# choderalab/pymbar

Measured on AMD Instinct MI355X. Metric: mbar_adaptive_iterations_per_sec, higher is better.
Workload: dtype f64

## Files before the change

### include/mbar_hip.h

```cpp
#ifndef MBAR_HIP_H
#define MBAR_HIP_H

#include <stdint.h>

#ifdef __cplusplus
extern "C" {
#endif

typedef struct mbar_ctx mbar_ctx;

#define MBAR_OK 0
#define MBAR_ERR_ARG (-1)
#define MBAR_ERR_HIP (-2)
#define MBAR_ERR_NODEVICE (-3)
#define MBAR_ERR_STATE (-4)
#define MBAR_ERR_COMM (-5)
#define MBAR_ERR_NUMERIC (-6)

#define MBAR_EVAL_GRAM 1u
#define MBAR_EVAL_USE_OFFSET 2u

#define MBAR_TIMER_LSE 0
#define MBAR_TIMER_GRAM 1
#define MBAR_TIMER_REDUCE 2
#define MBAR_TIMER_OTHER 3
#define MBAR_TIMER_FUSED 4
#define MBAR_TIMER_NEWTON 5
#define MBAR_TIMER_COMM 6
#define MBAR_TIMER_COUNT 7

int mbar_version(void);
const char* mbar_last_error(const mbar_ctx* ctx);
int mbar_device_count(int* count);
int mbar_device_info(int device, char* name, int name_len, int* compute_units, int64_t* total_mem_bytes);

int mbar_ctx_create(mbar_ctx** out, int device, int64_t K, int64_t N_local);
void mbar_ctx_destroy(mbar_ctx* ctx);
int mbar_ctx_synchronize(mbar_ctx* ctx);
int mbar_cache_trim(void);
int mbar_host_digest(const void* data, int64_t nbytes, int threads, uint64_t* out2);
int mbar_host_newton_direction(const double* H, const double* g, int m, int threads, double* x);
int mbar_device_synchronize(int device);
int mbar_ctx_set_option(mbar_ctx* ctx, const char* key, int64_t value);

int mbar_ctx_upload_u(mbar_ctx* ctx, const double* u_host, int64_t ld_host, int64_t col0_host,
                      int64_t ncols, int64_t col0_dev);
int mbar_ctx_download_u(mbar_ctx* ctx, double* out, int64_t ld_out);
int mbar_ctx_upload_rows(mbar_ctx* ctx, int64_t row0, int64_t nrows, const double* rows_host, int64_t ld_host);
int mbar_ctx_copy_rows(mbar_ctx* dst, int64_t dst_row0, mbar_ctx* src, int64_t src_row0, int64_t nrows);
int mbar_ctx_row_sub(mbar_ctx* ctx, int64_t row, const double* v_host);
int mbar_ctx_rows_sub(mbar_ctx* ctx, int64_t dst_row0, int64_t src_row0, int64_t nrows, const double* v_host);
int mbar_ctx_rows_rsub(mbar_ctx* ctx, int64_t dst_row0, int64_t src_row0, int64_t nrows);
int mbar_ctx_rows_logshift(mbar_ctx* ctx, int64_t row0, int64_t nrows, double* shift_out);
int mbar_ctx_vec_logshift(mbar_ctx* ctx, const double* A, double* shift_out);
int mbar_ctx_fill_masked_rows(mbar_ctx* ctx, int64_t row0, int64_t nrows, const double* v_host, const int32_t* label_host);
int mbar_ctx_generate_harmonic(mbar_ctx* ctx, uint64_t seed, const double* O_k, const double* K_k,
                               const int64_t* N_k_global, int64_t n_global0);
int mbar_ctx_set_Nk(mbar_ctx* ctx, const double* N_k);

int mbar_ctx_set_sample_weights(mbar_ctx* ctx, const double* c_n);

int mbar_ctx_draw_bootstrap_weights(mbar_ctx* ctx, uint64_t seed, int64_t replicate, const int64_t* cumN, int64_t K_states,
                                    const int64_t* order, int64_t n_global0);
int mbar_ctx_set_bootstrap_layout(mbar_ctx* ctx, const int64_t* cumN, int64_t K_states, const int64_t* order);
int mbar_bootstrap_draws(uint64_t seed, int64_t replicate, const int64_t* cumN, int64_t K_states, const int64_t* order,
                         int64_t* rints_out);

int mbar_ctx_weights_from_vec(mbar_ctx* ctx, double power);

int mbar_comm_unique_id(void* id128);
int mbar_ctx_comm_init(mbar_ctx* ctx, const void* id128, int rank, int nranks);
typedef int (*mbar_allreduce_fn)(double* buf, int64_t count, int op, void* user);
int mbar_ctx_set_host_allreduce(mbar_ctx* ctx, mbar_allreduce_fn fn, void* user, int rank, int nranks);
int mbar_ctx_comm_destroy(mbar_ctx* ctx);

typedef struct mbar_loopback mbar_loopback;
int mbar_loopback_create(mbar_loopback** out, int nranks);
void mbar_loopback_destroy(mbar_loopback* group);
int mbar_ctx_set_loopback(mbar_ctx* ctx, mbar_loopback* group, int rank);

int mbar_eval(mbar_ctx* ctx, const double* f, int nf, unsigned flags, double* psum,
              double* sumlogden, double* gram);
int mbar_ctx_set_objective_offset(mbar_ctx* ctx, const double* f0);
int mbar_lognum(mbar_ctx* ctx, const double* f, double* lognum);
int mbar_logden(mbar_ctx* ctx, const double* f, double* out_n);
int mbar_logw(mbar_ctx* ctx, const double* f, double* out_kn, int64_t ld_out);
int mbar_w(mbar_ctx* ctx, const double* f, double* out_kn, int64_t ld_out);
int mbar_gram_w(mbar_ctx* ctx, const double* f, double* gramW, double* wsum);

int mbar_ctx_create_ext(mbar_ctx** out, mbar_ctx* base, int64_t K_rows);
int mbar_ctx_rows_sub_from(mbar_ctx* dst, int64_t dst_row0, mbar_ctx* src, int64_t src_row0, int64_t nrows, const double* v_host);
int mbar_ctx_rows_rsub_from(mbar_ctx* dst, int64_t dst_row0, mbar_ctx* src, int64_t src_row0, int64_t nrows);
int mbar_ctx_rows_obs_from(mbar_ctx* dst, int64_t dst_row0, mbar_ctx* base, int64_t state_row0, int64_t obs_row0, int64_t nrows,
                           double* shift_out, const double* min_in, double* min_out);
int mbar_lognum_ext(mbar_ctx* ext, mbar_ctx* base, const double* f_base, double* lognum_ext);
int mbar_gram_w_ext(mbar_ctx* ext, mbar_ctx* base, const double* f_base, const double* f_ext, const double* gram_base, double* gramW,
                    double* wsum);

typedef struct mbar_solve_result {
    int64_t iterations;
    int64_t nr_iter;
    int64_t sci_iter;
    int32_t success;
    int32_t gram_sweeps;
    double max_delta;
    double gnorm;
    double wall_ms;
    int32_t warm_starts;
    int32_t builds;
    int32_t light_sweeps;
    int32_t fused_unit;
} mbar_solve_result;

int mbar_solve_adaptive(mbar_ctx* ctx, double* f_inout, double tol, int64_t maxiter,
                        int64_t min_sc_iter, double gamma, int check_convergence,
                        double* history, int64_t history_rows, mbar_solve_result* result);
int mbar_ctx_last_solve_psum(mbar_ctx* ctx, double* psum);
int mbar_solve_sci(mbar_ctx* ctx, double* f_inout, double tol, int64_t maxiter, int check_convergence,
                   mbar_solve_result* result);

int mbar_ctx_timing(mbar_ctx* ctx, int which, double* total_ms, int64_t* launches);
int mbar_ctx_timing_reset(mbar_ctx* ctx);
int mbar_mfma_f64_peak(mbar_ctx* ctx, double* tflops);

typedef struct mbar_kde mbar_kde;
#define MBAR_KDE_GAUSSIAN 0
#define MBAR_KDE_TOPHAT 1
#define MBAR_KDE_EPANECHNIKOV 2
#define MBAR_KDE_EXPONENTIAL 3
#define MBAR_KDE_LINEAR 4
#define MBAR_KDE_COSINE 5
int mbar_kde_create(mbar_kde** out, int device, int kernel, int d, int64_t N, const double* x, double bandwidth);
void mbar_kde_destroy(mbar_kde* kde);
int mbar_kde_set_weights(mbar_kde* kde, int64_t C, const double* v);
int mbar_kde_eval(mbar_kde* kde, int64_t M, const double* q, double* out);
int mbar_kde_log_norm(int kernel, int d, double bandwidth, double* out);

typedef struct mbar_acf mbar_acf;
int mbar_acf_create(mbar_acf** out, int device, int64_t T, const double* a, const double* b, int64_t K, const int64_t* seg,
                    double shift_a, double shift_b);
void mbar_acf_destroy(mbar_acf* acf);
int mbar_acf_suffix_g(mbar_acf* acf, int64_t nskip, int fast, int64_t mintime, int fft, double* g, int64_t* stop, int32_t* status);
int mbar_acf_multiple_g(mbar_acf* acf, int fast, int64_t mintime, double* g, int64_t* stop, int32_t* status, int64_t ct_cap,
                        double* ct);
int mbar_acf_schedule_length(int fast, int64_t tmax, int64_t* out);
int mbar_acf_lag_sums(mbar_acf* acf, int64_t nlags, const int64_t* lags, int64_t norig, const int64_t* origins, int segments,
                      double* xab, double* xba);

#define MBAR_BAR_CHUNK 4096
typedef struct mbar_bar_state {
    double DeltaF, DeltaF_old, DeltaF_initial, UpperB, LowerB, FUpperB, FLowerB, FNew, relative_change, relative_tolerance;
    double req[2];
    double moments[4];
    int64_t method, iterated, maximum_iterations, iteration, phase, status, nreq, nzero, want_moments, moments_pending;
} mbar_bar_state;
typedef struct mbar_bar mbar_bar;
int mbar_bar_create(mbar_bar** out, int device, int64_t P, const int64_t* n_f, const double* w_f, const int64_t* n_r,
                    const double* w_r);
void mbar_bar_destroy(mbar_bar* bar);
int mbar_bar_zero(mbar_bar* bar, const double* deltaf, double* out);
int mbar_bar_solve(mbar_bar* bar, mbar_bar_state* states, int64_t* passes);
int mbar_bar_moments(mbar_bar* bar, double* out);
int mbar_bar_step_host(mbar_bar_state* state, const double* F);

typedef struct mbar_bspline mbar_bspline;
int mbar_bspline_create(mbar_bspline** out, int device, int64_t N, const double* x);
void mbar_bspline_destroy(mbar_bspline* bs);
int mbar_bspline_set_groups(mbar_bspline* bs, int G, const int* g);
int mbar_bspline_set_weights(mbar_bspline* bs, int64_t C, const double* v);
int mbar_bspline_moments(mbar_bspline* bs, int k, int nbasis, const double* t, double* out);
int mbar_bspline_kernel_ms(mbar_bspline* bs, double* ms);

#define MBAR_BATCH_MAX_K 64
#define MBAR_BATCH_CHUNK 256
typedef struct mbar_batch_state {
    double f[MBAR_BATCH_MAX_K];
    double req[2][MBAR_BATCH_MAX_K];
    double lognum[MBAR_BATCH_MAX_K];
    double psum[MBAR_BATCH_MAX_K];
    double Nk[MBAR_BATCH_MAX_K];
    double x[MBAR_BATCH_MAX_K];
    double tol, gamma, max_delta, max_diff, gnorm_sci, gnorm_nr;
    int64_t K, maxiter, min_sc_iter, iterations, nr_iter, sci_iter, choices;
    int64_t phase, status, success, nreq, gram_req, gram_w, newton_bad;
} mbar_batch_state;
typedef struct mbar_batch mbar_batch;
int mbar_batch_create(mbar_batch** out, int device, int64_t P, const int64_t* K, const int64_t* N, const double* const* u);
void mbar_batch_destroy(mbar_batch* b);
int mbar_batch_solve(mbar_batch* b, mbar_batch_state* states, int64_t* passes);
int mbar_batch_gram_w(mbar_batch* b, const double* f, const int32_t* mask, double* gram, double* wsum);
int mbar_batch_step_host(mbar_batch_state* state, const double* lognum, const double* gram);

int mbar_batch_set_replicas(mbar_batch* b, int64_t R, const int64_t* base, const int64_t* Nk);
int mbar_batch_replica_set_weights(mbar_batch* b, int64_t slot, const double* c_n);
int mbar_batch_replicas_draw(mbar_batch* b, int64_t first, int64_t count, const uint64_t* seed, const int64_t* replicate);
int mbar_batch_replicas_solve(mbar_batch* b, mbar_batch_state* states, int64_t* passes);
int mbar_batch_replicas_gram_w(mbar_batch* b, const double* f, const int32_t* mask, double* gram, double* wsum);

#ifdef __cplusplus
}
#endif
#endif
```

### pymbar_amd/_lib.py

```python
import ctypes as C
import os

HERE = os.path.dirname(os.path.abspath(__file__))
LIB_PATH = os.environ.get("MBAR_HIP_LIBRARY") or os.path.join(HERE, "csrc", "libmbar_hip.so")

MBAR_OK = 0
EVAL_GRAM = 1
EVAL_USE_OFFSET = 2
TIMER_LSE, TIMER_GRAM, TIMER_REDUCE, TIMER_OTHER, TIMER_FUSED, TIMER_NEWTON, TIMER_COMM = 0, 1, 2, 3, 4, 5, 6


class BackendUnavailable(RuntimeError):
    """libmbar_hip.so is missing / not loadable, or there is no gfx950 device."""


class MbarHipError(RuntimeError):

    def __init__(self, code, message):
        super().__init__(f"libmbar_hip error {code}: {message}")
        self.code = code


class BarState(C.Structure):
    _fields_ = [(n, C.c_double) for n in ("DeltaF", "DeltaF_old", "DeltaF_initial", "UpperB", "LowerB", "FUpperB", "FLowerB", "FNew",
                                          "relative_change", "relative_tolerance")] + [
        ("req", C.c_double * 2), ("moments", C.c_double * 4)] + [
        (n, C.c_int64) for n in ("method", "iterated", "maximum_iterations", "iteration", "phase", "status", "nreq", "nzero",
                                 "want_moments", "moments_pending")]


MBAR_BATCH_MAX_K = 64
MBAR_BATCH_CHUNK = 256


class BatchState(C.Structure):
    _fields_ = [(n, C.c_double * MBAR_BATCH_MAX_K) for n in ("f",)] + [("req", (C.c_double * MBAR_BATCH_MAX_K) * 2)] + [
        (n, C.c_double * MBAR_BATCH_MAX_K) for n in ("lognum", "psum", "Nk", "x")] + [
        (n, C.c_double) for n in ("tol", "gamma", "max_delta", "max_diff", "gnorm_sci", "gnorm_nr")] + [
        (n, C.c_int64) for n in ("K", "maxiter", "min_sc_iter", "iterations", "nr_iter", "sci_iter", "choices", "phase", "status",
                                 "success", "nreq", "gram_req", "gram_w", "newton_bad")]


class SolveResult(C.Structure):
    _fields_ = [
        ("iterations", C.c_int64),
        ("nr_iter", C.c_int64),
        ("sci_iter", C.c_int64),
        ("success", C.c_int32),
        ("gram_sweeps", C.c_int32),
        ("max_delta", C.c_double),
        ("gnorm", C.c_double),
        ("wall_ms", C.c_double),
        ("warm_starts", C.c_int32),
        ("builds", C.c_int32),
        ("light_sweeps", C.c_int32),
        ("fused_unit", C.c_int32),
    ]


ALLREDUCE_FN = C.CFUNCTYPE(C.c_int, C.POINTER(C.c_double), C.c_int64, C.c_int, C.c_void_p)

_dp = C.POINTER(C.c_double)
_ip = C.POINTER(C.c_int64)
_ctx = C.c_void_p

SIGNATURES = {
    "mbar_version": (C.c_int, []),
    "mbar_last_error": (C.c_char_p, [_ctx]),
    "mbar_device_count": (C.c_int, [C.POINTER(C.c_int)]),
    "mbar_device_info": (C.c_int, [C.c_int, C.c_char_p, C.c_int, C.POINTER(C.c_int), _ip]),
    "mbar_ctx_create": (C.c_int, [C.POINTER(_ctx), C.c_int, C.c_int64, C.c_int64]),
    "mbar_ctx_destroy": (None, [_ctx]),
    "mbar_ctx_synchronize": (C.c_int, [_ctx]),
    "mbar_device_synchronize": (C.c_int, [C.c_int]),
    "mbar_cache_trim": (C.c_int, []),
    "mbar_host_digest": (C.c_int, [C.c_void_p, C.c_int64, C.c_int, C.POINTER(C.c_uint64)]),
    "mbar_host_newton_direction": (C.c_int, [_dp, _dp, C.c_int, C.c_int, _dp]),
    "mbar_ctx_set_option": (C.c_int, [_ctx, C.c_char_p, C.c_int64]),
    "mbar_ctx_upload_u": (C.c_int, [_ctx, _dp, C.c_int64, C.c_int64, C.c_int64, C.c_int64]),
    "mbar_ctx_download_u": (C.c_int, [_ctx, _dp, C.c_int64]),
    "mbar_ctx_upload_rows": (C.c_int, [_ctx, C.c_int64, C.c_int64, _dp, C.c_int64]),
    "mbar_ctx_copy_rows": (C.c_int, [_ctx, C.c_int64, _ctx, C.c_int64, C.c_int64]),
    "mbar_ctx_row_sub": (C.c_int, [_ctx, C.c_int64, _dp]),
    "mbar_ctx_rows_sub": (C.c_int, [_ctx, C.c_int64, C.c_int64, C.c_int64, _dp]),
    "mbar_ctx_rows_rsub": (C.c_int, [_ctx, C.c_int64, C.c_int64, C.c_int64]),
    "mbar_ctx_rows_logshift": (C.c_int, [_ctx, C.c_int64, C.c_int64, _dp]),
    "mbar_ctx_vec_logshift": (C.c_int, [_ctx, _dp, _dp]),
    "mbar_ctx_fill_masked_rows": (C.c_int, [_ctx, C.c_int64, C.c_int64, _dp, C.POINTER(C.c_int32)]),
    "mbar_ctx_generate_harmonic": (C.c_int, [_ctx, C.c_uint64, _dp, _dp, _ip, C.c_int64]),
    "mbar_ctx_set_Nk": (C.c_int, [_ctx, _dp]),
    "mbar_ctx_set_sample_weights": (C.c_int, [_ctx, _dp]),
    "mbar_ctx_weights_from_vec": (C.c_int, [_ctx, C.c_double]),
    "mbar_ctx_draw_bootstrap_weights": (C.c_int, [_ctx, C.c_uint64, C.c_int64, _ip, C.c_int64, _ip, C.c_int64]),
    "mbar_ctx_set_bootstrap_layout": (C.c_int, [_ctx, _ip, C.c_int64, _ip]),
    "mbar_bootstrap_draws": (C.c_int, [C.c_uint64, C.c_int64, _ip, C.c_int64, _ip, _ip]),
    "mbar_comm_unique_id": (C.c_int, [C.c_void_p]),
    "mbar_ctx_comm_init": (C.c_int, [_ctx, C.c_void_p, C.c_int, C.c_int]),
    "mbar_ctx_set_host_allreduce": (C.c_int, [_ctx, ALLREDUCE_FN, C.c_void_p, C.c_int, C.c_int]),
    "mbar_ctx_comm_destroy": (C.c_int, [_ctx]),
    "mbar_loopback_create": (C.c_int, [C.POINTER(C.c_void_p), C.c_int]),
    "mbar_loopback_destroy": (None, [C.c_void_p]),
    "mbar_ctx_set_loopback": (C.c_int, [_ctx, C.c_void_p, C.c_int]),
    "mbar_eval": (C.c_int, [_ctx, _dp, C.c_int, C.c_uint, _dp, _dp, _dp]),
    "mbar_ctx_set_objective_offset": (C.c_int, [_ctx, _dp]),
    "mbar_lognum": (C.c_int, [_ctx, _dp, _dp]),
    "mbar_logden": (C.c_int, [_ctx, _dp, _dp]),
    "mbar_logw": (C.c_int, [_ctx, _dp, _dp, C.c_int64]),
    "mbar_w": (C.c_int, [_ctx, _dp, _dp, C.c_int64]),
    "mbar_gram_w": (C.c_int, [_ctx, _dp, _dp, _dp]),
    "mbar_ctx_create_ext": (C.c_int, [C.POINTER(_ctx), _ctx, C.c_int64]),
    "mbar_ctx_rows_sub_from": (C.c_int, [_ctx, C.c_int64, _ctx, C.c_int64, C.c_int64, _dp]),
    "mbar_ctx_rows_rsub_from": (C.c_int, [_ctx, C.c_int64, _ctx, C.c_int64, C.c_int64]),
    "mbar_ctx_rows_obs_from": (C.c_int, [_ctx, C.c_int64, _ctx, C.c_int64, C.c_int64, C.c_int64, _dp, _dp, _dp]),
    "mbar_lognum_ext": (C.c_int, [_ctx, _ctx, _dp, _dp]),
    "mbar_gram_w_ext": (C.c_int, [_ctx, _ctx, _dp, _dp, _dp, _dp, _dp]),
    "mbar_solve_adaptive": (C.c_int, [_ctx, _dp, C.c_double, C.c_int64, C.c_int64, C.c_double, C.c_int,
                                      _dp, C.c_int64, C.POINTER(SolveResult)]),
    "mbar_ctx_last_solve_psum": (C.c_int, [_ctx, _dp]),
    "mbar_solve_sci": (C.c_int, [_ctx, _dp, C.c_double, C.c_int64, C.c_int, C.POINTER(SolveResult)]),
    "mbar_ctx_timing": (C.c_int, [_ctx, C.c_int, _dp, _ip]),
    "mbar_ctx_timing_reset": (C.c_int, [_ctx]),
    "mbar_mfma_f64_peak": (C.c_int, [_ctx, _dp]),
    "mbar_kde_create": (C.c_int, [C.POINTER(C.c_void_p), C.c_int, C.c_int, C.c_int, C.c_int64, _dp, C.c_double]),
    "mbar_kde_destroy": (None, [C.c_void_p]),
    "mbar_kde_set_weights": (C.c_int, [C.c_void_p, C.c_int64, _dp]),
    "mbar_kde_eval": (C.c_int, [C.c_void_p, C.c_int64, _dp, _dp]),
    "mbar_kde_log_norm": (C.c_int, [C.c_int, C.c_int, C.c_double, _dp]),
    "mbar_acf_create": (C.c_int, [C.POINTER(C.c_void_p), C.c_int, C.c_int64, _dp, _dp, C.c_int64, _ip, C.c_double, C.c_double]),
    "mbar_acf_destroy": (None, [C.c_void_p]),
    "mbar_acf_suffix_g": (C.c_int, [C.c_void_p, C.c_int64, C.c_int, C.c_int64, C.c_int, _dp, _ip, C.POINTER(C.c_int32)]),
    "mbar_acf_multiple_g": (C.c_int, [C.c_void_p, C.c_int, C.c_int64, _dp, _ip, C.POINTER(C.c_int32), C.c_int64, _dp]),
    "mbar_acf_schedule_length": (C.c_int, [C.c_int, C.c_int64, _ip]),
    "mbar_acf_lag_sums": (C.c_int, [C.c_void_p, C.c_int64, _ip, C.c_int64, _ip, C.c_int, _dp, _dp]),
    "mbar_bar_create": (C.c_int, [C.POINTER(C.c_void_p), C.c_int, C.c_int64, _ip, _dp, _ip, _dp]),
    "mbar_bar_destroy": (None, [C.c_void_p]),
    "mbar_bar_zero": (C.c_int, [C.c_void_p, _dp, _dp]),
    "mbar_bar_solve": (C.c_int, [C.c_void_p, C.POINTER(BarState), _ip]),
    "mbar_bar_moments": (C.c_int, [C.c_void_p, _dp]),
    "mbar_bar_step_host": (C.c_int, [C.POINTER(BarState), _dp]),
    "mbar_bspline_create": (C.c_int, [C.POINTER(C.c_void_p), C.c_int, C.c_int64, _dp]),
    "mbar_bspline_destroy": (None, [C.c_void_p]),
    "mbar_bspline_set_groups": (C.c_int, [C.c_void_p, C.c_int, C.POINTER(C.c_int32)]),
    "mbar_bspline_set_weights": (C.c_int, [C.c_void_p, C.c_int64, _dp]),
    "mbar_bspline_moments": (C.c_int, [C.c_void_p, C.c_int, C.c_int, _dp, _dp]),
    "mbar_bspline_kernel_ms": (C.c_int, [C.c_void_p, _dp]),
    "mbar_batch_create": (C.c_int, [C.POINTER(C.c_void_p), C.c_int, C.c_int64, _ip, _ip, C.POINTER(_dp)]),
    "mbar_batch_destroy": (None, [C.c_void_p]),
    "mbar_batch_solve": (C.c_int, [C.c_void_p, C.POINTER(BatchState), _ip]),
    "mbar_batch_gram_w": (C.c_int, [C.c_void_p, _dp, C.POINTER(C.c_int32), _dp, _dp]),
    "mbar_batch_step_host": (C.c_int, [C.POINTER(BatchState), _dp, _dp]),
    "mbar_batch_set_replicas": (C.c_int, [C.c_void_p, C.c_int64, _ip, _ip]),
    "mbar_batch_replica_set_weights": (C.c_int, [C.c_void_p, C.c_int64, _dp]),
    "mbar_batch_replicas_draw": (C.c_int, [C.c_void_p, C.c_int64, C.c_int64, C.POINTER(C.c_uint64), _ip]),
    "mbar_batch_replicas_solve": (C.c_int, [C.c_void_p, C.POINTER(BatchState), _ip]),
    "mbar_batch_replicas_gram_w": (C.c_int, [C.c_void_p, _dp, C.POINTER(C.c_int32), _dp, _dp]),
}

_lib = None


def load_library():
    global _lib
    if _lib is not None:
        return _lib
    if not os.path.exists(LIB_PATH):
        raise BackendUnavailable(
            f"{LIB_PATH} not found: build it with `python -c 'import __graft_entry__ as g; g.build()'` "
            "(hipcc --offload-arch=gfx950).  pymbar_amd has no CPU fallback.")
    try:
        lib = C.CDLL(LIB_PATH)
    except OSError as exc:
        raise BackendUnavailable(f"cannot load {LIB_PATH}: {exc}") from exc
    for name, (restype, argtypes) in SIGNATURES.items():
        fn = getattr(lib, name)
        fn.restype = restype
        fn.argtypes = argtypes
    _lib = lib
    return lib


def last_error(ctx=None):
    msg = load_library().mbar_last_error(ctx)
    return msg.decode("utf-8", "replace") if msg else ""


def check(code, ctx=None):
    if code != MBAR_OK:
        raise MbarHipError(code, last_error(ctx))


def host_digest(a, threads=0):
    out = (C.c_uint64 * 2)()
    check(load_library().mbar_host_digest(C.c_void_p(a.ctypes.data), a.nbytes, int(threads), out))
    return bytes(out)


def bootstrap_draws(seed, replicate, cumN, order=None):
    import numpy as np

    cumN = np.ascontiguousarray(cumN, dtype=np.int64)
    total = int(cumN[-1])
    out = np.zeros(total, dtype=np.int64)
    ip = C.POINTER(C.c_int64)
    optr = None
    if order is not None:
        order = np.ascontiguousarray(order, dtype=np.int64)
        optr = order.ctypes.data_as(ip)
    check(load_library().mbar_bootstrap_draws(C.c_uint64(int(seed)), int(replicate), cumN.ctypes.data_as(ip), len(cumN) - 1, optr,
                                              out.ctypes.data_as(ip)))
    return out


def host_newton_direction(H, g, threads=0):
    import numpy as np

    H = np.ascontiguousarray(H, dtype=np.float64)
    g = np.ascontiguousarray(g, dtype=np.float64)
    m = g.shape[0]
    if H.shape != (m, m):
        raise ValueError("H must be (m, m) for g of length m")
    x = np.empty(m, dtype=np.float64)
    check(load_library().mbar_host_newton_direction(H.ctypes.data_as(_dp), g.ctypes.data_as(_dp), m, int(threads), x.ctypes.data_as(_dp)))
    return x


def trim_device_cache():
    check(load_library().mbar_cache_trim())


def device_count():
    lib = load_library()
    n = C.c_int(0)
    rc = lib.mbar_device_count(C.byref(n))
    return n.value if rc == MBAR_OK else 0


def require_device():
    if device_count() < 1:
        raise BackendUnavailable(
            "no HIP device visible: pymbar_amd computes only on an MI355X (gfx950) through "
            "libmbar_hip.so and has no CPU fallback")


def default_device(device=None):
    if device is None:
        device = int(os.environ.get("LOCAL_RANK", "0")) % max(1, device_count())
    return int(device)

# ... 27 lines not shown
```

### pymbar_amd/csrc/mbar_capi.cpp

```cpp
#include "mbar_ctx.h"

using namespace mbar;
using namespace mbar::host;

namespace mbar {
namespace host {

int fail(mbar_ctx* c, int code, const std::string& msg) {
    if (c) c->error = msg;
    g_last_error = msg;
    return code;
}
hipEvent_t get_event(mbar_ctx* c) {
    if (!c->pool.empty()) {
        hipEvent_t e = c->pool.back();
        c->pool.pop_back();
        return e;
    }
    hipEvent_t e;
    if (hipEventCreate(&e) != hipSuccess) return nullptr;
    return e;
}
void flush_timers(mbar_ctx* c) {
    for (auto& tp : c->pending) {
// ... 496 lines not shown
        HIPCHK(c, hipMemcpyAsync(c->hred, c->red, total * sizeof(double), hipMemcpyDeviceToHost, c->stream));
    }
    rc = sync_stream(c);
    if (rc) return rc;
    if (!ratio.empty())
        for (int64_t k = 0; k < rows; ++k) c->hred[(size_t)rows + k] *= ratio[(size_t)k];
    if (psum)
        for (int i = 0; i < nf; ++i)
            for (int64_t k = 0; k < c->K; ++k) psum[(size_t)i * c->K + k] = c->hred[(size_t)i * rows + k];
    if (sumlogden)
        for (int i = 0; i < nf; ++i) sumlogden[i] = c->hred[n_ps + i];
    if (want_gram && gram) {
        std::fill(gram, gram + (size_t)c->K * c->K, 0.0);
        unpack_gram(plan, c->hred + off_gram, c->K, gram);
    }
    if (c->opt_check_finite) {
        for (size_t i = 0; i < n_ps + n_obj; ++i)
            if (!std::isfinite(c->hred[i])) {
                c->error = "non-finite partial sum in evaluation pass";
                break;
            }
    }
    if (nf == 1 && ld0 == c->logden[0]) {
        c->ld0_f.assign(f, f + c->K);
        c->ld0_valid = true;
    }
    return MBAR_OK;
}


}
}


extern "C" {

int mbar_version(void) { return 101; }

const char* mbar_last_error(const mbar_ctx* ctx) { return ctx ? ctx->error.c_str() : g_last_error.c_str(); }

int mbar_device_count(int* count) {
    if (!count) return fail(nullptr, MBAR_ERR_ARG, "count is NULL");
    int n = 0;
    hipError_t e = hipGetDeviceCount(&n);
    if (e != hipSuccess) {
        *count = 0;
        return fail(nullptr, MBAR_ERR_NODEVICE, std::string("hipGetDeviceCount: ") + hipGetErrorString(e));
    }
    *count = n;
    return MBAR_OK;
}

int mbar_device_info(int device, char* name, int name_len, int* compute_units, int64_t* total_mem_bytes) {
    hipDeviceProp_t p;
    hipError_t e = hipGetDeviceProperties(&p, device);
    if (e != hipSuccess) return fail(nullptr, MBAR_ERR_NODEVICE, std::string("hipGetDeviceProperties: ") + hipGetErrorString(e));
    if (name && name_len > 0) {
        std::snprintf(name, (size_t)name_len, "%s (%s)", p.name[0] ? p.name : "AMD Instinct MI355X", p.gcnArchName);
    }
    if (compute_units) *compute_units = p.multiProcessorCount;
    if (total_mem_bytes) *total_mem_bytes = (int64_t)p.totalGlobalMem;
    return MBAR_OK;
}

int mbar_ctx_create(mbar_ctx** out, int device, int64_t K, int64_t N_local) {
    if (!out) return fail(nullptr, MBAR_ERR_ARG, "out is NULL");
    *out = nullptr;
    if (K < 1 || N_local < 0) return fail(nullptr, MBAR_ERR_ARG, "K must be >= 1 and N_local >= 0");
    DevInfo di;
    int rc = open_device(device, &di);
    if (rc) return rc;
    mbar_ctx* c = new mbar_ctx();
    g_live_contexts.fetch_add(1);
    c->device = device;
    c->num_cu = di.num_cu;
    c->K = K;
    c->Kp = padded_K(K);
    c->N = N_local;
    c->ld = c->Kp <= 32 ? (N_local + 63) / 64 * 64 : (N_local + TS - 1) / TS * TS;
    if (c->ld == 0) c->ld = c->Kp <= 32 ? 64 : TS;
#define CRT(expr)                                                                                   \
    do {                                                                                            \
        hipError_t _e = (expr);                                                                     \
        if (_e != hipSuccess) {                                                                     \
            int rc_ = fail(nullptr, MBAR_ERR_HIP, std::string(#expr) + ": " + hipGetErrorString(_e)); \
            mbar_ctx_destroy(c);                                                                    \
            return rc_;                                                                             \
        }                                                                                           \
    } while (0)
    {
        std::lock_guard<std::mutex> lock(g_dev_mu);
        auto& pool = g_stream_pool[device];
        if (!pool.empty()) {
            c->stream = pool.back();
            pool.pop_back();
        }
    }
    if (!c->stream) CRT(hipStreamCreateWithFlags(&c->stream, hipStreamNonBlocking));
    const size_t ubytes = (size_t)c->Kp * c->ld * sizeof(double);
    CRT(cache_malloc((void**)&c->u, ubytes));
    CRT(launch_zero(c->stream, c->u, ubytes));
    CRT(cache_malloc((void**)&c->logden[0], (size_t)3 * c->ld * sizeof(double)));
    CRT(launch_zero(c->stream, c->logden[0], (size_t)3 * c->ld * sizeof(double)));
    c->logden[1] = c->logden[0] + c->ld;
    c->logden[2] = c->logden[0] + 2 * c->ld;
    CRT(cache_malloc((void**)&c->cw, (size_t)c->ld * sizeof(double)));
    CRT(launch_zero(c->stream, c->cw, (size_t)c->ld * sizeof(double)));
    if (c->N > 0) CRT(launch_fill(c->stream, c->cw, 1.0, c->N));
    CRT(cache_malloc((void**)&c->small, small_doubles(c->Kp) * sizeof(double)));
    CRT(cache_host_malloc((void**)&c->hstage, (size_t)4 * c->Kp * sizeof(double)));
    CRT(hipMemsetAsync(c->small, 0, small_doubles(c->Kp) * sizeof(double), c->stream));
    CRT(hipStreamSynchronize(c->stream));
#undef CRT
    c->Nk.assign(K, 0.0);
    c->lnNk.assign(K, 0.0);
    *out = c;
    return MBAR_OK;
}

void mbar_ctx_destroy(mbar_ctx* c) {
    if (!c) return;
    (void)hipSetDevice(c->device);
    if (c->stream) (void)hipStreamSynchronize(c->stream);
    flush_timers(c);
    for (auto e : c->pool) (void)hipEventDestroy(e);
    if (c->comm && g_rccl.CommDestroy) g_rccl.CommDestroy(c->comm);
    if (c->u_alloc) (void)cache_free(c->u_alloc);
    else if (c->u) (void)cache_free(c->u);
    if (c->logden[0]) (void)cache_free(c->logden[0]);
    if (c->ad) (void)cache_free(c->ad);
    if (c->P) (void)cache_free(c->P);
    if (c->pm_vec) (void)cache_free(c->pm_vec);
    if (c->pm_ld0) (void)cache_free(c->pm_ld0);
    if (c->part_g) (void)cache_free(c->part_g);
    if (c->cwsq) (void)cache_free(c->cwsq);
    if (c->chol) (void)cache_free(c->chol);
    if (c->ad_ints) (void)cache_free(c->ad_ints);
    if (c->h_ctl) (void)cache_host_free(c->h_ctl);
    if (c->ad_graph) (void)hipGraphExecDestroy(c->ad_graph);
    if (c->dn) (void)cache_free(c->dn);
    if (c->cw) (void)cache_free(c->cw);
    if (c->lden_eff) (void)cache_free(c->lden_eff);
    if (c->small) (void)cache_free(c->small);
    if (c->part) (void)cache_free(c->part);
    if (c->scratch) (void)cache_free(c->scratch);
    if (c->red) (void)cache_free(c->red);
    if (c->hred) (void)cache_host_free(c->hred);
    if (c->lognum_part) (void)cache_free(c->lognum_part);
    if (c->f_hist) (void)cache_free(c->f_hist);
    if (c->hstage) (void)cache_host_free(c->hstage);
    if (c->vec_tmp) (void)cache_free(c->vec_tmp);
    if (c->boot_idx) (void)cache_free(c->boot_idx);
    if (c->stamps) (void)hipFree(c->stamps);
    if (c->sci_graph) (void)hipGraphExecDestroy(c->sci_graph);
    if (c->stream) {
        std::lock_guard<std::mutex> lock(g_dev_mu);
        auto& pool = g_stream_pool[c->device];
        if (pool.size() < 8)
            pool.push_back(c->stream);
        else
            (void)hipStreamDestroy(c->stream);
    }
    delete c;
    if (g_live_contexts.fetch_sub(1) == 1) g_mem.trim_to(g_mem.idle_limit());
}

int mbar_ctx_synchronize(mbar_ctx* c) {
    if (!c) return fail(nullptr, MBAR_ERR_ARG, "ctx is NULL");
    HIPCHK(c, hipSetDevice(c->device));
    return sync_stream(c);
}

int mbar_device_synchronize(int device) {
    hipError_t e = hipSetDevice(device);
    if (e == hipSuccess) e = hipDeviceSynchronize();
    if (e != hipSuccess) return fail(nullptr, MBAR_ERR_HIP, std::string("hipDeviceSynchronize: ") + hipGetErrorString(e));
    return MBAR_OK;
}

int mbar_ctx_set_option(mbar_ctx* c, const char* key, int64_t value) {
    if (!c || !key) return fail(c, MBAR_ERR_ARG, "NULL argument");
    const std::string k(key);
    if (k == "grid_blocks") c->opt_grid = value;
    else if (k == "force_generic") c->opt_force_generic = value;
    else if (k == "small_k_kernel") c->opt_small = value;
    else if (k == "wide_k_kernel") c->opt_wide = value;
    else if (k == "check_finite") c->opt_check_finite = value;
    else if (k == "timing") c->opt_timing = value;
    else if (k == "graph") c->opt_graph = value;
    else if (k == "sci_batch") c->opt_sci_batch = value < 1 ? 1 : (value > 256 ? 256 : value);
    else if (k == "device_loop") c->opt_device_loop = value;
    else if (k == "pmode") c->opt_pmode = value;
    else if (k == "fused") c->opt_fused = value;
    else if (k == "gram_quad") c->opt_quad = value;
    else if (k == "device_loop_wide") c->opt_device_loop_wide = value;
    else if (k == "pcache") c->opt_pcache = value;
    else if (k == "merge_select") c->opt_merge_select = value;
    else if (k == "light_last") c->opt_light_last = value;
    else if (k == "fused_general") {
        c->opt_fused_general = value ? 1 : 0;
        (void)drop_graphs(c);
    }
    else if (k == "debug_download_p") c->opt_debug_download_p = value;
    else if (k == "direct_results") c->opt_direct_results = value;
    else if (k == "sci_merged") c->opt_sci_merged = value;
    else if (k == "host_pmode") c->opt_host_pmode = value;
    else if (k == "rect_waves") c->opt_rect_waves = value == 8 ? 8 : 4;
    else if (k == "newton_ldlt") {
        c->opt_newton_ldlt = value ? 1 : 0;
        (void)drop_graphs(c);
    }
    else if (k == "sci_pingpong") {
        c->opt_sci_pingpong = value;
        (void)drop_graphs(c);
    }
    else if (k == "small_balanced") {
        c->opt_small_balanced = value;
        (void)drop_graphs(c);
    }
    else if (k == "wide_pmode") c->opt_wide_pmode = value;
    else if (k == "quad_trim") {
        c->opt_quad_trim = value;
        c->P_valid = false;
    }
    else if (k == "adapt_batch") c->opt_adapt_batch = value < 1 ? 1 : (value > 64 ? 64 : value);
    else return fail(c, MBAR_ERR_ARG, "unknown option: " + k);
    return MBAR_OK;
}

int mbar_ctx_upload_u(mbar_ctx* c, const double* u_host, int64_t ld_host, int64_t col0_host, int64_t ncols,
                      int64_t col0_dev) {
    if (!c || !u_host) return fail(c, MBAR_ERR_ARG, "NULL argument");
    if (ncols < 0 || col0_dev < 0 || col0_dev + ncols > c->N || col0_host < 0 || col0_host + ncols > ld_host)
        return fail(c, MBAR_ERR_ARG, "column range out of bounds");
    if (ncols == 0) return MBAR_OK;
    HIPCHK(c, hipSetDevice(c->device));
    HIPCHK(c, hipMemcpy2DAsync(c->u + col0_dev, (size_t)c->ld * sizeof(double), u_host + col0_host,
                               (size_t)ld_host * sizeof(double), (size_t)ncols * sizeof(double), (size_t)c->K,
                               hipMemcpyHostToDevice, c->stream));
    c->u_checked = false;
    c->P_valid = false;
    c->last_psum.clear();
    return sync_stream(c);
}

int mbar_ctx_upload_rows(mbar_ctx* c, int64_t row0, int64_t nrows, const double* rows_host, int64_t ld_host) {
    if (!c || !rows_host) return fail(c, MBAR_ERR_ARG, "NULL argument");
    if (row0 < 0 || nrows < 0 || row0 + nrows > c->K || ld_host < c->N) return fail(c, MBAR_ERR_ARG, "row range out of bounds");
    if (nrows == 0) return MBAR_OK;
    HIPCHK(c, hipSetDevice(c->device));
    HIPCHK(c, hipMemcpy2DAsync(c->u + row0 * c->ld, (size_t)c->ld * sizeof(double), rows_host,
                               (size_t)ld_host * sizeof(double), (size_t)c->N * sizeof(double), (size_t)nrows,
                               hipMemcpyHostToDevice, c->stream));
    c->u_checked = false;
    c->P_valid = false;
    c->last_psum.clear();
    return sync_stream(c);
}

int mbar_ctx_copy_rows(mbar_ctx* dst, int64_t dst_row0, mbar_ctx* src, int64_t src_row0, int64_t nrows) {
    if (!dst || !src) return fail(dst, MBAR_ERR_ARG, "NULL argument");
    if (dst->device != src->device || dst->N != src->N) return fail(dst, MBAR_ERR_ARG, "contexts must share device and N_local");
    if (nrows < 0 || dst_row0 < 0 || src_row0 < 0 || dst_row0 + nrows > dst->K || src_row0 + nrows > src->K)
        return fail(dst, MBAR_ERR_ARG, "row range out of bounds");
    if (nrows == 0) return MBAR_OK;
    HIPCHK(dst, hipSetDevice(dst->device));
    HIPCHK(dst, hipStreamSynchronize(src->stream));
    if (dst->ld == src->ld)
        HIPCHK(dst, hipMemcpyAsync(dst->u + dst_row0 * dst->ld, src->u + src_row0 * src->ld, (size_t)nrows * dst->ld * sizeof(double),
                                   hipMemcpyDeviceToDevice, dst->stream));
    else
        HIPCHK(dst, hipMemcpy2DAsync(dst->u + dst_row0 * dst->ld, (size_t)dst->ld * sizeof(double), src->u + src_row0 * src->ld,
                                     (size_t)src->ld * sizeof(double), (size_t)dst->N * sizeof(double), (size_t)nrows,
                                     hipMemcpyDeviceToDevice, dst->stream));
    dst->u_checked = false;
    dst->P_valid = false;
    dst->last_psum.clear();
    return sync_stream(dst);
}

int mbar_ctx_row_sub(mbar_ctx* c, int64_t row, const double* v_host) {
    if (!c) return fail(c, MBAR_ERR_ARG, "NULL argument");
    if (row < 0 || row >= c->K) return fail(c, MBAR_ERR_ARG, "row out of range");
    if (!v_host && !c->vec_tmp) return fail(c, MBAR_ERR_STATE, "mbar_ctx_row_sub: no vector has been uploaded yet");
    HIPCHK(c, hipSetDevice(c->device));
    if (!c->vec_tmp) HIPCHK(c, cache_malloc((void**)&c->vec_tmp, (size_t)c->ld * sizeof(double)));
    double* tmp = c->vec_tmp;
    if (v_host) c->vec_holds_logshift = false;
    if (v_host)
        HIPCHK(c, hipMemcpyAsync(tmp, v_host, (size_t)c->N * sizeof(double), hipMemcpyHostToDevice, c->stream));
    HIPCHK(c, launch_row_sub(c->stream, c->u + row * c->ld, tmp, c->N));
    c->u_checked = false;
    c->P_valid = false;
    c->last_psum.clear();
    return sync_stream(c);
}

int mbar_ctx_rows_sub(mbar_ctx* c, int64_t dst_row0, int64_t src_row0, int64_t nrows, const double* v_host) {
    if (!c) return fail(c, MBAR_ERR_ARG, "NULL argument");
    if (nrows < 0 || dst_row0 < 0 || src_row0 < 0 || dst_row0 + nrows > c->K || src_row0 + nrows > c->K)
        return fail(c, MBAR_ERR_ARG, "row range out of bounds");
    if (dst_row0 != src_row0 && dst_row0 < src_row0 + nrows && src_row0 < dst_row0 + nrows)
        return fail(c, MBAR_ERR_ARG, "mbar_ctx_rows_sub: the row ranges overlap");
    if (!v_host && !c->vec_tmp) return fail(c, MBAR_ERR_STATE, "mbar_ctx_rows_sub: no vector has been uploaded yet");
    if (nrows == 0) return MBAR_OK;
    HIPCHK(c, hipSetDevice(c->device));
    if (!c->vec_tmp) HIPCHK(c, cache_malloc((void**)&c->vec_tmp, (size_t)c->ld * sizeof(double)));
    if (v_host) c->vec_holds_logshift = false;
    if (v_host)
        HIPCHK(c, hipMemcpyAsync(c->vec_tmp, v_host, (size_t)c->N * sizeof(double), hipMemcpyHostToDevice, c->stream));
    HIPCHK(c, launch_rows_sub(c->stream, c->u + dst_row0 * c->ld, c->u + src_row0 * c->ld, c->ld, nrows, c->vec_tmp, c->N));
    c->u_checked = false;
    c->P_valid = false;
    c->last_psum.clear();
    return sync_stream(c);
}

int mbar_ctx_rows_rsub(mbar_ctx* c, int64_t dst_row0, int64_t src_row0, int64_t nrows) {
    if (!c) return fail(c, MBAR_ERR_ARG, "NULL argument");
    if (nrows < 0 || dst_row0 < 0 || src_row0 < 0 || dst_row0 + nrows > c->K || src_row0 + nrows > c->K)
        return fail(c, MBAR_ERR_ARG, "row range out of bounds");
    if (dst_row0 < src_row0 + nrows && src_row0 < dst_row0 + nrows) return fail(c, MBAR_ERR_ARG, "mbar_ctx_rows_rsub: the row ranges overlap");
    if (nrows == 0) return MBAR_OK;
    HIPCHK(c, hipSetDevice(c->device));
    HIPCHK(c, launch_rows_rsub(c->stream, c->u + dst_row0 * c->ld, c->u + src_row0 * c->ld, c->ld, nrows, c->N));
    c->u_checked = false;
    c->P_valid = false;
    c->last_psum.clear();
    return sync_stream(c);
}

static int logshift_rows(mbar_ctx* c, double* base, int64_t nrows, double* shift_host) {
    int rc = ensure(c, &c->scratch, &c->scratch_doubles, (size_t)nrows * 257);
    if (rc) return rc;
    double* shift_dev = c->scratch + (size_t)nrows * 256;
    HIPCHK(c, launch_rows_logshift(c->stream, base, c->ld, nrows, c->N, c->scratch, shift_dev));
    HIPCHK(c, hipMemcpyAsync(shift_host, shift_dev, (size_t)nrows * sizeof(double), hipMemcpyDeviceToHost, c->stream));
    return sync_stream(c);
}

int mbar_ctx_rows_logshift(mbar_ctx* c, int64_t row0, int64_t nrows, double* shift_out) {
    if (!c || !shift_out) return fail(c, MBAR_ERR_ARG, "NULL argument");
    if (row0 < 0 || nrows < 0 || row0 + nrows > c->K) return fail(c, MBAR_ERR_ARG, "row range out of bounds");
    if (nrows == 0) return MBAR_OK;
    if (c->nranks > 1) return fail(c, MBAR_ERR_STATE, "mbar_ctx_rows_logshift: the minimum is taken over this context's samples only");
    HIPCHK(c, hipSetDevice(c->device));
    c->u_checked = false;
    c->P_valid = false;
    c->last_psum.clear();
    return logshift_rows(c, c->u + row0 * c->ld, nrows, shift_out);
}

int mbar_ctx_vec_logshift(mbar_ctx* c, const double* A_host, double* shift_out) {
    if (!c || !A_host || !shift_out) return fail(c, MBAR_ERR_ARG, "NULL argument");
    if (c->nranks > 1) return fail(c, MBAR_ERR_STATE, "mbar_ctx_vec_logshift: the minimum is taken over this context's samples only");
    HIPCHK(c, hipSetDevice(c->device));
    if (!c->vec_tmp) HIPCHK(c, cache_malloc((void**)&c->vec_tmp, (size_t)c->ld * sizeof(double)));
    HIPCHK(c, hipMemcpyAsync(c->vec_tmp, A_host, (size_t)c->N * sizeof(double), hipMemcpyHostToDevice, c->stream));
    c->vec_holds_logshift = false;
    const int lrc = logshift_rows(c, c->vec_tmp, 1, shift_out);
    c->vec_holds_logshift = lrc == MBAR_OK;
    return lrc;
}

int mbar_ctx_fill_masked_rows(mbar_ctx* c, int64_t row0, int64_t nrows, const double* v_host, const int32_t* label_host) {
    if (!c || !v_host || !label_host) return fail(c, MBAR_ERR_ARG, "NULL argument");
    if (row0 < 0 || nrows < 0 || row0 + nrows > c->K) return fail(c, MBAR_ERR_ARG, "row range out of bounds");
    if (nrows == 0) return MBAR_OK;
    HIPCHK(c, hipSetDevice(c->device));
    if (!c->vec_tmp) HIPCHK(c, cache_malloc((void**)&c->vec_tmp, (size_t)c->ld * sizeof(double)));
    int* dlabel = nullptr;
    HIPCHK(c, cache_malloc((void**)&dlabel, (size_t)c->N * sizeof(int)));
    c->vec_holds_logshift = false;
    hipError_t e = hipMemcpyAsync(c->vec_tmp, v_host, (size_t)c->N * sizeof(double), hipMemcpyHostToDevice, c->stream);
    if (e == hipSuccess) e = hipMemcpyAsync(dlabel, label_host, (size_t)c->N * sizeof(int), hipMemcpyHostToDevice, c->stream);
    if (e == hipSuccess) e = launch_fill_masked_rows(c->stream, c->u + row0 * c->ld, c->ld, c->N, nrows, c->vec_tmp, dlabel);
    if (e == hipSuccess) e = hipStreamSynchronize(c->stream);
    (void)cache_free(dlabel);
    if (e != hipSuccess) return fail(c, MBAR_ERR_HIP, std::string("mbar_ctx_fill_masked_rows: ") + hipGetErrorString(e));
// ... 743 lines not shown
```

### pymbar_amd/csrc/mbar_ctx.h

```cpp
#pragma once
#include "../../include/mbar_hip.h"
#include "mbar_internal.h"

#include <dlfcn.h>
#include <sched.h>
#include <unistd.h>
#include <rccl/rccl.h>

#include <algorithm>
#include <chrono>
#include <condition_variable>
#include <cmath>
#include <cstdio>
#include <cstdlib>
#include <cstring>
#include <functional>
#include <limits>
#include <map>
#include <memory>
#include <mutex>
#include <string>
#include <atomic>
#include <thread>
#include <unordered_map>
// ... 110 lines not shown
        *out = q;
        return hipSuccess;
    }
    hipError_t release(void* q) {
        if (!q) return hipSuccess;
        std::lock_guard<std::mutex> lock(mu);
        auto it = live.find(q);
        if (it == live.end()) return hipErrorInvalidValue;
        const size_t sz = it->second.first;
        const int d = it->second.second;
        Pool& p = d < 0 ? pinned : dev[d];
        if (p.cached + sz <= p.limit && sz <= p.limit / 2) {
            p.free_blocks.emplace(sz, q);
            p.cached += sz;
            return hipSuccess;
        }
        live.erase(it);
        return d < 0 ? hipHostFree(q) : hipFree(q);
    }
    void trim_to(size_t keep_bytes) {
        std::lock_guard<std::mutex> lock(mu);
        for (auto& dp : dev) {
            Pool& p = dp.second;
            while (p.cached > keep_bytes && !p.free_blocks.empty()) {
                auto it = std::prev(p.free_blocks.end());
                live.erase(it->second);
                (void)hipSetDevice(dp.first);
                (void)hipFree(it->second);
                p.cached -= it->first;
                p.free_blocks.erase(it);
            }
        }
    }
    size_t idle_limit() {
        if (const char* e = std::getenv("MBAR_CACHE_IDLE_MB")) return (size_t)std::strtoull(e, nullptr, 10) << 20;
        return (size_t)1024 << 20;
    }
    void trim() {
        std::lock_guard<std::mutex> lock(mu);
        for (auto& dp : dev) {
            for (auto& kv : dp.second.free_blocks) {
                live.erase(kv.second);
                (void)hipSetDevice(dp.first);
                (void)hipFree(kv.second);
            }
            dp.second.free_blocks.clear();
            dp.second.cached = 0;
        }
        for (auto& kv : pinned.free_blocks) {
            live.erase(kv.second);
            (void)hipHostFree(kv.second);
        }
        pinned.free_blocks.clear();
        pinned.cached = 0;
    }
};
extern MemCache g_mem;
extern std::atomic<int> g_live_contexts;
struct DevInfo {
    int num_cu = 256;
    std::string arch;
};
extern std::mutex g_dev_mu;
extern std::map<int, DevInfo> g_dev_info;
extern std::map<int, std::vector<hipStream_t>> g_stream_pool;
inline hipError_t cache_malloc(void** p, size_t bytes) { return g_mem.alloc(p, bytes, false); }
inline hipError_t cache_free(void* p) { return g_mem.release(p); }
inline hipError_t cache_host_malloc(void** p, size_t bytes) { return g_mem.alloc(p, bytes, true); }
inline hipError_t cache_host_free(void* p) { return g_mem.release(p); }

struct TimerPair {
    hipEvent_t a, b;
    int which;
};


}
}
using mbar::host::TimerPair;

struct mbar_loopback {
    int nranks = 0, device = -1;
    std::mutex mu;
    std::condition_variable cv;
    int arrived = 0;
    uint64_t gen = 0;
    bool broken = false;
    std::vector<const double*> src;
    std::vector<int64_t> cnt;
    std::vector<int> op;
    std::vector<hipEvent_t> ready, done;
    std::vector<double*> tmp;
    std::vector<size_t> tmp_doubles;
    std::vector<int> attached;
};

struct mbar_ctx {
    int device = 0;
    int num_cu = 256;
    hipStream_t stream = nullptr;
    int64_t K = 0, Kp = 0, N = 0, ld = 0;
    bool have_Nk = false;
    bool u_checked = false, u_poison = false;
    std::vector<double> ld0_f;
    bool ld0_valid = false;
    bool u_posinf = true;
    std::vector<double> Nk, lnNk;
    std::vector<int> sampled;
    double* u = nullptr;
    double* u_alloc = nullptr;
    mbar_ctx* ext_base = nullptr;
    double* logden[3] = {nullptr, nullptr, nullptr};
    double* dn = nullptr;
    double* cw = nullptr;
    double* lden_eff = nullptr;
    bool weighted = false;
    double* small = nullptr;
    double* part = nullptr;
    size_t part_doubles = 0;
    double* scratch = nullptr;
    size_t scratch_doubles = 0;
    double* red = nullptr;
    size_t red_doubles = 0;
    double* hred = nullptr;
    double* hstage = nullptr;
    double* lognum_part = nullptr;
    size_t lognum_part_doubles = 0;
    double* f_hist = nullptr;
    double* vec_tmp = nullptr;
    int64_t* boot_idx = nullptr;
    size_t boot_idx_words = 0;
    uint64_t boot_layout_digest[2] = {0, 0};
    int64_t boot_states = 0, boot_total = 0;
    bool boot_has_order = false;
    bool vec_holds_logshift = false;
    hipGraphExec_t sci_graph = nullptr;
    int64_t sci_graph_batch = 0, sci_graph_sig = 0;
    double sci_graph_tol = 0.0;
    double* ad = nullptr;
    int64_t ad_hist_cap = 0;
    int* ad_ints = nullptr;
    int* h_ctl = nullptr;
    hipGraphExec_t ad_graph = nullptr;
    int64_t ad_graph_batch = 0, ad_graph_sig = 0;
    double* P = nullptr;
    bool P_failed = false;
    double* pm_vec = nullptr;
    double* pm_ld0 = nullptr;
    double* part_g = nullptr;
    size_t part_g_doubles = 0;
    double* cwsq = nullptr;
    double* chol = nullptr;
    long long* stamps = nullptr;
    std::vector<double> last_psum;
    bool P_valid = false;
    std::vector<double> P_a0;
    int64_t opt_grid = 0, opt_force_generic = 0, opt_check_finite = 1, opt_sci_batch = 16, opt_timing = 0, opt_graph = 1, opt_small = 1, opt_wide = 1;
    int64_t opt_device_loop = 1, opt_adapt_batch = 8, opt_pmode = 1, opt_fused = 1, opt_quad = 1, opt_device_loop_wide = 1, opt_pcache = 1, opt_merge_select = 1, opt_sci_merged = 1, opt_wide_pmode = 1, opt_quad_trim = 1, opt_light_last = 1, opt_direct_results = 1, opt_debug_download_p = 0, opt_fused_general = 0;
    int64_t opt_small_balanced = 1, opt_sci_pingpong = 1, opt_host_pmode = 2, opt_rect_waves = 8, opt_newton_ldlt = 1;

    ncclComm_t comm = nullptr;
    mbar_loopback* loop = nullptr;
    mbar_allreduce_fn host_reduce = nullptr;
    void* host_reduce_user = nullptr;
    int rank = 0, nranks = 1;
    std::vector<TimerPair> pending;
    std::vector<hipEvent_t> pool;
    double t_ms[MBAR_TIMER_COUNT] = {0, 0, 0, 0, 0};
    int64_t t_n[MBAR_TIMER_COUNT] = {0, 0, 0, 0, 0};
    std::string error;
};


namespace mbar {
namespace host {

int fail(mbar_ctx* c, int code, const std::string& msg);
#define HIPCHK(ctx, expr)                                                                        \
    do {                                                                                         \
        hipError_t _e = (expr);                                                                  \
        if (_e != hipSuccess)                                                                    \
            return fail(ctx, MBAR_ERR_HIP, std::string(#expr) + ": " + hipGetErrorString(_e));   \
    } while (0)
inline int bad_arg(const std::string& msg) { return fail(nullptr, MBAR_ERR_ARG, msg); }


template <typename T>
struct DevBuf {
    T* p = nullptr;
    size_t n = 0;
    DevBuf() = default;
    DevBuf(const DevBuf&) = delete;
    DevBuf& operator=(const DevBuf&) = delete;
    DevBuf(DevBuf&& o) noexcept : p(o.p), n(o.n) {
        o.p = nullptr;
        o.n = 0;
    }
    DevBuf& operator=(DevBuf&& o) noexcept {
        std::swap(p, o.p);
        std::swap(n, o.n);
        return *this;
    }
    ~DevBuf() { reset(); }
    operator T*() const { return p; }
    void reset() {
        if (p) (void)cache_free(p);
        p = nullptr;
        n = 0;
    }
    auto grow(size_t want) -> hipError_t {
        if (n >= want) return hipSuccess;
        if (p) {
            hipError_t e = cache_free(p);
            if (e != hipSuccess) return e;
        }
        p = nullptr;
        n = 0;
        hipError_t e = cache_malloc((void**)&p, want * sizeof(T));
        if (e == hipSuccess) n = want;
        return e;
    }
};

int open_device(int device, DevInfo* out);

struct Handle {
    int device = 0;
    hipStream_t stream = nullptr;
    Handle() { g_live_contexts.fetch_add(1); }
    Handle(const Handle&) = delete;
    Handle& operator=(const Handle&) = delete;
    ~Handle() {
        if (stream) (void)hipStreamDestroy(stream);
        if (g_live_contexts.fetch_sub(1) == 1) g_mem.trim_to(g_mem.idle_limit());
    }
};

template <class H>
void destroy_handle(H* h) {
    if (!h) return;
    (void)hipSetDevice(h->device);
    if (h->stream) (void)hipStreamSynchronize(h->stream);
    delete h;
}

template <class H, class Init>
int create_handle(H** out, int device, Init&& init) {
    DevInfo di;
    int rc = open_device(device, &di);
    if (rc) return rc;
    H* h = new H();
    h->device = device;
    hipError_t e = hipStreamCreateWithFlags(&h->stream, hipStreamNonBlocking);
    rc = e == hipSuccess ? init(h, di)
                         : fail(nullptr, MBAR_ERR_HIP, std::string("hipStreamCreateWithFlags: ") + hipGetErrorString(e));
    if (rc != MBAR_OK) {
        const std::string msg = g_last_error;
        destroy_handle(h);
        return fail(nullptr, rc, msg);
    }
    *out = h;
    return MBAR_OK;
}

struct ColumnPasses {
    std::vector<int> widths;
    std::vector<double> host;
    int64_t rows = 0, C = 0;
    DevBuf<double> dev;
    int64_t pass = -1;
    int cb = 0;
    explicit ColumnPasses(std::vector<int> w) : widths(std::move(w)) {}
    int width(int64_t cols) const {
        for (int w : widths)
            if (w >= cols) return w;
        return widths.back();
    }
    double* reset(int64_t rows_, int64_t C_, const double* v = nullptr) {
        rows = rows_;
        C = C_;
        if (v) host.assign(v, v + rows * C);
        else host.resize((size_t)rows * C);
        pass = -1;
        return host.data();
    }
    bool holds(int64_t c0, int width_) const { return pass == c0 && cb == width_; }
    int upload(int64_t c0, int cv, int w, int64_t pitch);
};


hipEvent_t get_event(mbar_ctx* c);
struct ScopedTimer {
    mbar_ctx* c;
    TimerPair tp;
    bool on;
    ScopedTimer(mbar_ctx* c_, int which) : c(c_), on(false) {
        tp.a = tp.b = nullptr;
        if (!c->opt_timing) return;
        tp.a = get_event(c);
        tp.b = get_event(c);
        tp.which = which;
        if (tp.a && tp.b) {
            on = hipEventRecord(tp.a, c->stream) == hipSuccess;
        }
    }
    ~ScopedTimer() {
        if (on) {
            (void)hipEventRecord(tp.b, c->stream);
            c->pending.push_back(tp);
        }
    }
// ... 74 lines not shown
```

### pymbar_amd/csrc/mbar_device.h

```cpp
#ifndef MBAR_DEVICE_H
#define MBAR_DEVICE_H
#include "mbar_internal.h"

#include <hip/hip_ext.h>
#include <math.h>
#include <type_traits>

namespace mbar {

typedef double v4d __attribute__((ext_vector_type(4)));

template <int CTRL>
__device__ __forceinline__ double dpp_move(double x) {
    int lo = __double2loint(x), hi = __double2hiint(x);
    lo = __builtin_amdgcn_update_dpp(0, lo, CTRL, 0xF, 0xF, true);
    hi = __builtin_amdgcn_update_dpp(0, hi, CTRL, 0xF, 0xF, true);
    return __hiloint2double(hi, lo);
}
__device__ __forceinline__ double row16_max(double x) {
    x = fmax(x, dpp_move<0xB1>(x));
    x = fmax(x, dpp_move<0x4E>(x));
    x = fmax(x, dpp_move<0x141>(x));
    x = fmax(x, dpp_move<0x140>(x));
    return x;
// ... 373 lines not shown
                                              double (&s0)[NF]) {
    double x0[NB];
    lse_load1<NB>(cbuf, rd0, a, x0);
    lse_math1<NB, NF>(x0, c, acc, w0, m2_0, s0);
}
template <int NB, int NF>
__device__ __forceinline__ void lse_group_pair(const char* cbuf, const char* wslot, int rd_base,
                                               const int (&pos)[GROUPS], int g, const double (&a)[NB],
                                               const double (&c)[NB], double (&acc)[NF][NB], int ks, int ns,
                                               double& mm, double (&ss)[NF]) {
    double m2a, m2b, sa[NF], sb[NF];
    const double va = *reinterpret_cast<const double*>(wslot + (4 * g + ns) * 8);
    const double vb = *reinterpret_cast<const double*>(wslot + (4 * (g + 1) + ns) * 8);
    if constexpr (NB <= 8) {
        lse_two_groups<NB, NF>(cbuf, rd_base + pos[g], rd_base + pos[g + 1], a, c, acc, va, vb, m2a, m2b, sa, sb);
    } else {
        lse_one_group<NB, NF>(cbuf, rd_base + pos[g], a, c, acc, va, m2a, sa);
        lse_one_group<NB, NF>(cbuf, rd_base + pos[g + 1], a, c, acc, vb, m2b, sb);
    }
    if ((ks & 3) == g) {
        mm = m2a;
#pragma unroll
        for (int f = 0; f < NF; ++f) ss[f] = sa[f];
    }
    if ((ks & 3) == g + 1) {
        mm = m2b;
#pragma unroll
        for (int f = 0; f < NF; ++f) ss[f] = sb[f];
    }
}

template <bool WIDE>
struct StageOffsetsT {
    typedef typename std::conditional<WIDE, uint64_t, uint32_t>::type off_t;
    off_t off[2];
};
typedef StageOffsetsT<false> StageOffsets;
template <bool WIDE = false>
__device__ __forceinline__ StageOffsetsT<WIDE> make_stage_offsets(int64_t ld, int lane) {
    StageOffsetsT<WIDE> so;
    const int r = lane >> 3, pos = 2 * (lane & 7);
#pragma unroll
    for (int par = 0; par < 2; ++par) {
        const int smp = (pos - ((r & 6) | (par << 3))) & 15;
        so.off[par] = (typename StageOffsetsT<WIDE>::off_t)(((int64_t)r * ld + smp) * 8);
    }
    return so;
}
#ifndef MBAR_DMA_AUX
#define MBAR_DMA_AUX 0
#endif
template <bool DMA>
__device__ __forceinline__ void stage_piece(const double* __restrict__ ubase , uint64_t voff,
                                            char* dst , int lane) {
    const char* src = reinterpret_cast<const char*>(ubase) + voff;
    if constexpr (DMA) {
        __builtin_amdgcn_global_load_lds((const __attribute__((address_space(1))) void*)src,
                                         (__attribute__((address_space(3))) void*)dst, 16, 0, MBAR_DMA_AUX);
    } else {
        *reinterpret_cast<double2*>(dst + lane * 16) = *reinterpret_cast<const double2*>(src);
    }
}
template <bool DMA>
__device__ __forceinline__ void stage_piece(const double* __restrict__ ubase , uint32_t voff,
                                            char* dst , int lane) {
    uint64_t ub = reinterpret_cast<uint64_t>(ubase);
    asm("" : "+s"(ub));
    asm("" : "+v"(voff));
    const char* src = reinterpret_cast<const char*>(ub) + voff;
    if constexpr (DMA) {
        __builtin_amdgcn_global_load_lds((const __attribute__((address_space(1))) void*)src,
                                         (__attribute__((address_space(3))) void*)dst, 16, 0, MBAR_DMA_AUX);
    } else {
        *reinterpret_cast<double2*>(dst + lane * 16) = *reinterpret_cast<const double2*>(src);
    }
}
template <int ROWS, bool DMA, int J0, int JSTEP, typename RowMap, typename SO>
__device__ __forceinline__ void stage_tile(const double* __restrict__ u, int64_t ld, int64_t n0, char* dst, int lane,
                                           const SO& so, RowMap rowmap) {
    constexpr int NDMA = ROWS / 8;
#pragma unroll
    for (int j = J0; j < NDMA; j += JSTEP)
        stage_piece<DMA>(u + rowmap(8 * j) * ld + rowmap.cols(j, n0), so.off[j & 1], dst + j * 1024, lane);
}

template <bool DMA>
__device__ __forceinline__ void stage_vec16(const double* __restrict__ v, int64_t n0, char* dst, int lane) {
    if (lane < 8) stage_piece<DMA>(v + n0, (uint32_t)(lane * 16), dst, lane);
}

__device__ __forceinline__ void settle(double& x) { asm volatile("" : "+v"(x)); }

__device__ __forceinline__ double load_untracked(const double* p) {
    double v;
    asm volatile("global_load_dwordx2 %0, %1, off" : "=v"(v) : "v"(p) : "memory");
    return v;
}
template <int N>
__device__ __forceinline__ void wait_vm_for(double& a, double& b, double& c, double& d, double& e, double (&r)[16]) {
    asm volatile("s_waitcnt vmcnt(%21)"
                 : "+v"(a), "+v"(b), "+v"(c), "+v"(d), "+v"(e), "+v"(r[0]), "+v"(r[1]), "+v"(r[2]), "+v"(r[3]), "+v"(r[4]), "+v"(r[5]),
                   "+v"(r[6]), "+v"(r[7]), "+v"(r[8]), "+v"(r[9]), "+v"(r[10]), "+v"(r[11]), "+v"(r[12]), "+v"(r[13]), "+v"(r[14]), "+v"(r[15])
                 : "n"(N)
                 : "memory");
}
__device__ __forceinline__ void lds_barrier() { asm volatile("s_waitcnt lgkmcnt(0)\n\ts_barrier" ::: "memory"); }
template <int N>
__device__ __forceinline__ void wait_vm() {
    asm volatile("s_waitcnt vmcnt(%0)" ::"n"(N) : "memory");
}

struct RowIdentity {
    int64_t row0;
    uint32_t live = 0xffffffffu;
    __device__ __forceinline__ int64_t operator()(int tr) const { return row0 + tr; }
    __device__ __forceinline__ int64_t cols(int j, int64_t n0) const { return ((live >> j) & 1u) ? n0 : 0; }
};
struct RowTwoPanels {
    int64_t row_i0, row_j0;
    int split;
    uint32_t live = 0xffffffffu;
    __device__ __forceinline__ int64_t operator()(int tr) const {
        return tr < split ? row_i0 + tr : row_j0 + (tr - split);
    }
    __device__ __forceinline__ int64_t cols(int j, int64_t n0) const { return ((live >> j) & 1u) ? n0 : 0; }
};
template <int NB>
__device__ __forceinline__ uint32_t live_piece_mask(const double (&a)[NB], double dead) {
    uint32_t m = 0;
#pragma unroll
    for (int I = 0; I < NB; ++I) {
        const unsigned long long b = __ballot(a[I] != dead);
        m |= ((b & 0xffull) ? 1u : 0u) << (2 * I);
        m |= ((b & 0xff00ull) ? 1u : 0u) << (2 * I + 1);
    }
    return m;
}

constexpr int lse_waves(int nb) { return nb <= 2 ? 16 : (nb <= 4 ? 8 : (nb <= 8 ? 4 : 2)); }
constexpr int TSS = 64;
constexpr int GRAM_AGPR_BLOCKS = 31;
constexpr double GRAM_NEG_HUGE = -2.9e303, LOGDEN_HUGE = 1e300;
constexpr int FUSED_PSUM1_FROM_GRAM_NB = 8;

static inline int blocks_per_cu_for(size_t lds_bytes) {
    int b = (int)((160 * 1024) / lds_bytes);
    if (b < 1) b = 1;
    if (b > 4) b = 4;
    return b;
}

static inline bool stage_offsets_wide(int64_t ld) { return (uint64_t)ld * 56u + 128u >= (1ull << 32); }

hipError_t launch_fused_quad(hipStream_t s, int nbt, const LaunchGeom& g, const double* P, int64_t ld, int64_t N, const double* cmul,
                             const double* cw, const double* wsq, double* rinv0, double* gp, double* pp, const LoopCtl& lc);

}
#endif
```

### pymbar_amd/csrc/mbar_host.cpp

```cpp
#include "mbar_ctx.h"

using namespace mbar;
using namespace mbar::host;

namespace mbar {
namespace host {

thread_local std::string g_last_error;
MemCache g_mem;
std::atomic<int> g_live_contexts{0};
std::mutex g_dev_mu;
std::map<int, DevInfo> g_dev_info;
std::map<int, std::vector<hipStream_t>> g_stream_pool;

int open_device(int device, DevInfo* out) {
    int n = 0;
    if (hipGetDeviceCount(&n) != hipSuccess || n < 1)
        return fail(nullptr, MBAR_ERR_NODEVICE, "no HIP device visible (libmbar_hip needs an MI355X / gfx950 GPU)");
    if (device < 0 || device >= n) return bad_arg("device index out of range");
    HIPCHK(nullptr, hipSetDevice(device));
    DevInfo di;
    {
        std::lock_guard<std::mutex> lock(g_dev_mu);
        auto it = g_dev_info.find(device);
// ... 381 lines not shown
            rc_[c] = d;
            inv[c - j0] = 1.0 / d;
            for (int i = c + 1; i < j1; ++i) {
                double* ri = L + (size_t)i * S;
                double v = ri[c];
                for (int k = j0; k < c; ++k) v -= ri[k] * rc_[k];
                ri[c] = v * inv[c - j0];
            }
        }
        for (int c = 0; c < j1 - j0; ++c)
            for (int k = c; k < j1 - j0; ++k) Lt[c * B + k] = L[(size_t)(j0 + k) * S + j0 + c];
        return true;
    };
    const bool dbg = std::getenv("MBAR_DEBUG_TIMING") != nullptr;
    double tp_diag = 0, tp_p1 = 0, tp_p2 = 0, tp_wait = 0;
    auto run = [&](int t) {
        const bool tm = dbg && t == 0;
        double q0 = tm ? now_ms() : 0.0, q1;
        auto lap = [&](double& into) { if (tm) { q1 = now_ms(); into += q1 - q0; q0 = q1; } };
        for_my_chunks(t, 0, [&](int i0, int n) {
            for (int i = i0; i < i0 + n; ++i) {
                double* dst = L + (size_t)i * S;
                const size_t len = i == mv ? (size_t)m : (size_t)(i + 1);
                std::memcpy(dst, i == mv ? b.data() : A + (size_t)i * lda, len * sizeof(double));
                std::memset(dst + len, 0, (S - len) * sizeof(double));
            }
        });
        copied.fetch_add(1, std::memory_order_acq_rel);
        spin_until([&]() { return copied.load(std::memory_order_acquire) >= T; });
        lap(tp_wait);
        for (int bi = 0; bi < nblk; ++bi) {
            const int j1 = std::min((bi + 1) * B, m);
            if (t == 0) {
                if (bi > 0)
                    for (int i0 = bi * B; i0 < j1; i0 += 8) phase2_rows(0, i0, std::min(8, j1 - i0), bi - 1);
                lap(tp_p2);
                if (!factor_diag(bi)) {
                    failed.store(1, std::memory_order_release);
                    return;
                }
                diag_ready.store(bi, std::memory_order_release);
                lap(tp_diag);
            }
            const int i_lo = j1 >= m ? mv : j1;
            if (bi > 0) for_my_chunks(t, i_lo, [&](int i0, int n) { phase2_rows(t, i0, n, bi - 1); });
            lap(tp_p2);
            if (t != 0) {
                spin_until([&]() { return diag_ready.load(std::memory_order_acquire) >= bi || failed.load(std::memory_order_acquire); });
                if (failed.load(std::memory_order_acquire)) return;
            }
            for_my_chunks(t, i_lo, [&](int i0, int n) { solve8(L + (size_t)i0 * S, S, n, bi * B, j1 - bi * B, Lt, inv, colbuf[bi & 1], ms, i0); });
            lap(tp_p1);
            arrived.fetch_add(1, std::memory_order_acq_rel);
            spin_until([&]() { return arrived.load(std::memory_order_acquire) >= T * (bi + 1) || failed.load(std::memory_order_acquire); });
            lap(tp_wait);
            if (failed.load(std::memory_order_acquire)) return;
        }
    };
    const double t_begin = dbg ? now_ms() : 0.0;
    g_team.run(T, run);
    const double t_fact = dbg ? now_ms() : 0.0;
    if (failed.load()) return false;
    std::memcpy(b.data(), L + (size_t)mv * S, (size_t)m * sizeof(double));
    for (int i = m - 1; i >= 0; --i) {
        const double* row = L + (size_t)i * S;
        const double xi = b[i] / row[i];
        b[i] = xi;
        for (int k = 0; k < i; ++k) b[k] -= row[k] * xi;
    }
    if (dbg)
        std::fprintf(stderr, "[mbar] blocked Cholesky m=%d, %d threads: factorisation %.3f ms (thread 0: diagonal blocks %.3f, rows against the block %.3f, trailing updates %.3f, copy + waiting %.3f), substitutions %.3f ms\n",
                     m, T, t_fact - t_begin, tp_diag, tp_p1, tp_p2, tp_wait, now_ms() - t_fact);
    for (int i = 0; i < m; ++i)
        if (!std::isfinite(b[i])) return false;
    return true;
}

void jacobi_eigh(std::vector<double> A, int m, std::vector<double>& w, std::vector<double>& V) {
    V.assign((size_t)m * m, 0.0);
    for (int i = 0; i < m; ++i) V[(size_t)i * m + i] = 1.0;
    for (int sweep = 0; sweep < 60; ++sweep) {
        double off = 0.0, diag = 0.0;
        for (int i = 0; i < m; ++i) {
            diag += A[(size_t)i * m + i] * A[(size_t)i * m + i];
            for (int j = i + 1; j < m; ++j) off += A[(size_t)i * m + j] * A[(size_t)i * m + j];
        }
        if (off <= 1e-30 * (diag + 1e-300)) break;
        for (int p = 0; p < m - 1; ++p)
            for (int q = p + 1; q < m; ++q) {
                const double apq = A[(size_t)p * m + q];
                if (apq == 0.0) continue;
                const double app = A[(size_t)p * m + p], aqq = A[(size_t)q * m + q];
                const double theta = (aqq - app) / (2.0 * apq);
                const double t = (theta >= 0 ? 1.0 : -1.0) / (std::fabs(theta) + std::sqrt(theta * theta + 1.0));
                const double cs = 1.0 / std::sqrt(t * t + 1.0), sn = t * cs;
                for (int k = 0; k < m; ++k) {
                    const double akp = A[(size_t)k * m + p], akq = A[(size_t)k * m + q];
                    A[(size_t)k * m + p] = cs * akp - sn * akq;
                    A[(size_t)k * m + q] = sn * akp + cs * akq;
                }
                for (int k = 0; k < m; ++k) {
                    const double apk = A[(size_t)p * m + k], aqk = A[(size_t)q * m + k];
                    A[(size_t)p * m + k] = cs * apk - sn * aqk;
                    A[(size_t)q * m + k] = sn * apk + cs * aqk;
                }
                for (int k = 0; k < m; ++k) {
                    const double vkp = V[(size_t)k * m + p], vkq = V[(size_t)k * m + q];
                    V[(size_t)k * m + p] = cs * vkp - sn * vkq;
                    V[(size_t)k * m + q] = sn * vkp + cs * vkq;
                }
            }
    }
    w.resize(m);
    for (int i = 0; i < m; ++i) w[i] = A[(size_t)i * m + i];
}

void newton_direction(const std::vector<double>& H, const std::vector<double>& g, int m, std::vector<double>& x) {
    x.assign(m, 0.0);
    if (m <= 1) return;
    const int r = m - 1;
    std::vector<double> b(g.begin() + 1, g.end());
    bool ok;
    if (r >= CHOL_BLOCKED_MIN) {
        ok = chol_solve_blocked(H.data() + m + 1, (size_t)m, b, r, host_team_size(r));
    } else {
        std::vector<double> A((size_t)r * r);
        for (int i = 0; i < r; ++i)
            for (int j = 0; j < r; ++j) A[(size_t)i * r + j] = H[(size_t)(i + 1) * m + (j + 1)];
        ok = chol_solve(A, b, r);
    }
    if (ok) {
        for (int i = 0; i < r; ++i) x[i + 1] = b[i];
        return;
    }
    std::vector<double> w, V;
    jacobi_eigh(H, m, w, V);
    double wmax = 0.0;
    for (double v : w) wmax = std::max(wmax, std::fabs(v));
    const double cut = wmax * std::numeric_limits<double>::epsilon() * m;
    std::vector<double> y(m, 0.0);
    for (int e = 0; e < m; ++e) {
        if (std::fabs(w[e]) <= cut) continue;
        double proj = 0.0;
        for (int k = 0; k < m; ++k) proj += V[(size_t)k * m + e] * g[k];
        proj /= w[e];
        for (int k = 0; k < m; ++k) y[k] += V[(size_t)k * m + e] * proj;
    }
    for (int k = 0; k < m; ++k) x[k] = y[k] - y[0];
}



}
}

extern "C" {

int mbar_cache_trim(void) {
    g_mem.trim();
    return MBAR_OK;
}

namespace {
inline uint64_t rotl64(uint64_t x, int r) { return (x << r) | (x >> (64 - r)); }
constexpr uint64_t DG_M0 = 0x9E3779B97F4A7C15ull, DG_M1 = 0xC2B2AE3D27D4EB4Full, DG_M2 = 0x165667B19E3779F9ull,
                   DG_M3 = 0xD6E8FEB86659FD93ull;
constexpr int64_t DG_CHUNK = 1 << 20;

void digest_chunk(const unsigned char* p, int64_t n, uint64_t out[2]) {
    uint64_t a0 = DG_M0 ^ (uint64_t)n, a1 = DG_M1, a2 = DG_M2, a3 = DG_M3;
    int64_t i = 0;
    for (; i + 32 <= n; i += 32) {
        uint64_t w[4];
        std::memcpy(w, p + i, 32);
        a0 = rotl64(a0 ^ w[0], 29) * DG_M1;
        a1 = rotl64(a1 ^ w[1], 29) * DG_M2;
        a2 = rotl64(a2 ^ w[2], 29) * DG_M3;
        a3 = rotl64(a3 ^ w[3], 29) * DG_M0;
    }
    if (i < n) {
        uint64_t w[4] = {0, 0, 0, 0};
        std::memcpy(w, p + i, (size_t)(n - i));
        a0 = rotl64(a0 ^ w[0], 29) * DG_M1;
        a1 = rotl64(a1 ^ w[1], 29) * DG_M2;
        a2 = rotl64(a2 ^ w[2], 29) * DG_M3;
        a3 = rotl64(a3 ^ w[3], 29) * DG_M0;
    }
    out[0] = a0 ^ rotl64(a1, 13) ^ rotl64(a2, 29) ^ rotl64(a3, 47);
    out[1] = a0 * DG_M2 + a1 * DG_M3 + a2 * DG_M0 + a3 * DG_M1;
}
}

int mbar_host_digest(const void* data, int64_t nbytes, int threads, uint64_t* out2) {
    if ((!data && nbytes > 0) || nbytes < 0 || !out2) return fail(nullptr, MBAR_ERR_ARG, "mbar_host_digest: bad argument");
    const unsigned char* p = (const unsigned char*)data;
    const int64_t nchunks = (nbytes + DG_CHUNK - 1) / DG_CHUNK;
    std::vector<uint64_t> part((size_t)nchunks * 2);
    int nt = threads > 0 ? threads : (int)std::thread::hardware_concurrency();
    nt = (int)std::max<int64_t>(1, std::min<int64_t>({(int64_t)nt, (int64_t)64, nchunks / 8}));
    auto work = [&](int t) {
        for (int64_t c = t; c < nchunks; c += nt)
            digest_chunk(p + c * DG_CHUNK, std::min<int64_t>(DG_CHUNK, nbytes - c * DG_CHUNK), &part[(size_t)c * 2]);
    };
    if (nt == 1) {
        work(0);
    } else {
        std::vector<std::thread> pool;
        for (int t = 1; t < nt; ++t) pool.emplace_back(work, t);
        work(0);
        for (auto& th : pool) th.join();
    }
    uint64_t h0 = DG_M3 ^ (uint64_t)nbytes, h1 = DG_M2 + (uint64_t)nbytes;
    for (int64_t c = 0; c < nchunks; ++c) {
        h0 = rotl64(h0 ^ part[(size_t)c * 2], 31) * DG_M0;
        h1 = rotl64(h1 ^ part[(size_t)c * 2 + 1], 27) * DG_M1;
    }
    out2[0] = h0 ^ (h0 >> 32);
    out2[1] = h1 ^ (h1 >> 29);
    return MBAR_OK;
}

int mbar_host_newton_direction(const double* H, const double* g, int m, int threads, double* x) {
    if (!H || !g || !x || m < 1) return fail(nullptr, MBAR_ERR_ARG, "mbar_host_newton_direction: bad argument");
    std::vector<double> Hv(H, H + (size_t)m * m), gv(g, g + m), xv;
    if (threads != 0) {
        const int r = m - 1;
        std::vector<double> A((size_t)r * r), b(r);
        for (int i = 0; i < r; ++i) {
            b[i] = gv[i + 1];
            for (int j = 0; j < r; ++j) A[(size_t)i * r + j] = Hv[(size_t)(i + 1) * m + (j + 1)];
        }
        if (r > 0 && (threads > 0 ? chol_solve_blocked(A.data(), (size_t)r, b, r, threads) : chol_solve(A, b, r))) {
            x[0] = 0.0;
            for (int i = 0; i < r; ++i) x[i + 1] = b[i];
            return MBAR_OK;
        }
    }
    newton_direction(Hv, gv, m, xv);
    std::copy(xv.begin(), xv.end(), x);
    return MBAR_OK;
}

int mbar_bootstrap_draws(uint64_t seed, int64_t replicate, const int64_t* cumN, int64_t K_states, const int64_t* order, int64_t* rints_out) {
    if (!cumN || !rints_out || K_states < 1 || replicate < 0 || cumN[0] != 0) return fail(nullptr, MBAR_ERR_ARG, "mbar_bootstrap_draws: bad argument");
    for (int64_t k = 0; k < K_states; ++k)
        if (cumN[k + 1] < cumN[k]) return fail(nullptr, MBAR_ERR_ARG, "mbar_bootstrap_draws: cumN must not decrease");
    if (order)
        for (int64_t p = 0; p < cumN[K_states]; ++p)
            if (order[p] < 0 || order[p] >= cumN[K_states]) return fail(nullptr, MBAR_ERR_ARG, "mbar_bootstrap_draws: order entry out of range");
    for (int64_t k = 0; k < K_states; ++k) {
        const int64_t start = cumN[k], nk = cumN[k + 1] - start;
        for (int64_t i = 0; i < nk; ++i) {
            const int64_t pos = start + bootstrap_draw(seed, (uint64_t)replicate, (uint64_t)(start + i), (uint64_t)nk);
            const int64_t slot_sample = order ? order[start + i] : start + i;
            rints_out[slot_sample] = order ? order[pos] : pos;
        }
    }
    return MBAR_OK;
}

}
```

### pymbar_amd/csrc/mbar_internal.h

```cpp
#pragma once
#include <hip/hip_runtime.h>
#include <stdint.h>

#include "../../include/mbar_hip.h"

namespace mbar {

constexpr int TS = 16;
constexpr int GROUPS = 4;
constexpr int MAX_FAST_K = 256;
constexpr int PANEL = 64;

inline int64_t padded_K(int64_t K) {
    if (K <= 128) return (K + 15) / 16 * 16;
    return (K + PANEL - 1) / PANEL * PANEL;
}
inline int lse_nb_for(int64_t Kp) {
    static const int nbs[] = {1, 2, 3, 4, 5, 6, 7, 8, 12, 16};
    int need = (int)(Kp / 16);
    for (int nb : nbs) if (nb >= need) return nb;
    return 0;
}

#if defined(__HIPCC__)
#define MBAR_HD __host__ __device__
#else
#define MBAR_HD
#endif
MBAR_HD inline uint64_t bootstrap_mix64(uint64_t z) {
    z = (z ^ (z >> 30)) * 0xBF58476D1CE4E5B9ull;
    z = (z ^ (z >> 27)) * 0x94D049BB133111EBull;
    return z ^ (z >> 31);
}
MBAR_HD inline int64_t bootstrap_draw(uint64_t seed, uint64_t replicate, uint64_t slot, uint64_t n) {
    const uint64_t key = bootstrap_mix64(seed + 0x9E3779B97F4A7C15ull * (replicate + 1));
    const uint64_t z = bootstrap_mix64(bootstrap_mix64(key ^ (slot * 0xD1342543DE82EF95ull)) + slot);
    return (int64_t)(((unsigned __int128)z * (unsigned __int128)n) >> 64);
}

enum : int {
    CTL_SLOT = 0,
    CTL_DONE = 1,
    CTL_ITER = 2,
    CTL_SCI = 3,
    CTL_NR = 4,
    CTL_REASON = 5,
    CTL_NEEDGRAM = 6,
    CTL_GRAMSWEEPS = 7,
    CTL_SPEC = 8,
    CTL_LIGHT = 9,
    CTL_LIGHTS = 10,
    CTL_WORDS = 12
};
struct LoopCtl {
    const int* ctl = nullptr;
    int64_t slot_stride = 0;
    hipEvent_t ev_start = nullptr, ev_stop = nullptr;
    bool unclamped = false;
    bool pmode = false;
    bool cond_needgram = false;
    bool light_only = false;
};

struct LaunchGeom {
    int blocks;
    int waves;
    int nwaves;
    int psum_records;
    int variant;
    size_t lds_bytes;
    int live_blocks = 0;
    int balanced = 0;
};

LaunchGeom lse_geometry(int nb, int nf, int num_cu, int64_t ntiles, int64_t grid_override, int variant);
hipError_t launch_lse(hipStream_t s, int nb, int nf, const LaunchGeom& g,
                      const double* u, int64_t ld, int64_t N, const double* aden ,
                      const double* cw, double* logden0, double* logden1, const double* dn,
                      double* psum_part, double* obj_part, const LoopCtl& lc = LoopCtl());

LaunchGeom gram_geometry(int tile_rows, bool diag, int num_cu, int64_t ntiles, int64_t grid_override);
hipError_t launch_row_sub(hipStream_t s, double* row, const double* v, int64_t n);
hipError_t launch_rows_sub(hipStream_t s, double* dst, const double* src, int64_t ld, int64_t nrows, const double* v, int64_t n);
hipError_t launch_rows_obs(hipStream_t s, double* dst, const double* obs, const double* state, int64_t ld, int64_t nrows, int64_t n,
                           double* part, double* shift_out, bool have_min = false);
hipError_t launch_rows_rsub(hipStream_t s, double* dst, const double* src, int64_t ld, int64_t nrows, int64_t n);
hipError_t launch_rows_logshift(hipStream_t s, double* base, int64_t ld, int64_t nrows, int64_t n, double* part, double* shift_out);
hipError_t launch_fill_masked_rows(hipStream_t s, double* rows, int64_t ld, int64_t n, int64_t nrows, const double* v,
                                   const int* label);
hipError_t launch_gram_diag(hipStream_t s, int nb, const LaunchGeom& g, const double* u,
                            int64_t ld, int64_t N, const double* anum ,
                            const double* logden, int64_t row0, double* gram_part, double* psum_part,
                            const LoopCtl& lc = LoopCtl());
hipError_t launch_gram_thin(hipStream_t s, const LaunchGeom& g, const double* u, int64_t ld, int64_t N, const double* ai,
                            const double* aj, const double* logden, int64_t ri, int64_t rj, double* gp);
hipError_t launch_gram_off(hipStream_t s, int nbj , const LaunchGeom& g, const double* u, int64_t ld,
                           int64_t N, const double* anum_i, const double* anum_j, const double* logden,
                           int64_t row_i0, int64_t row_j0, double* gram_part, bool pmode = false);

LaunchGeom gram_quad_geometry(int nbt, int num_cu, int64_t ntiles, int64_t grid_override);
hipError_t launch_gram_rect(hipStream_t s, int nbi, const LaunchGeom& g, const double* P, int64_t ld, int64_t N, int64_t ri, int64_t rj,
                            const double* rinv, double* gram_part);
hipError_t launch_gram_quad(hipStream_t s, int nbt, const LaunchGeom& g, const double* u, int64_t ld, int64_t N,
                            const double* anum, const double* logden, double* gram_part, const LoopCtl& lc = LoopCtl(),
                            double* Pout = nullptr);
hipError_t launch_gram_quad_split(hipStream_t s, int nbt, const LaunchGeom& g, const double* u, int64_t ld, int64_t N, const double* anum,
                                  const double* logden, double* gram_part, int64_t split_rows, int64_t row_j0);

hipError_t launch_lse_split(hipStream_t s, int num_cu, int nf, const double* u, int64_t ld, int64_t N, int64_t rows, const double* aden,
                            const double* cw, double* logden, double* logden1, const double* dn, double* psum_part, double* obj_part,
                            int* blocks_out, const double* ld_anchor = nullptr );
hipError_t launch_lse_generic(hipStream_t s, int num_cu, const double* u, int64_t ld, int64_t N, int64_t K,
                              const double* aden, const double* cw, double* logden, const double* dn,
                              double* obj_part , int* blocks_out);
hipError_t launch_colsum_generic(hipStream_t s, int num_cu, const double* u, int64_t ld, int64_t N, int64_t K,
                                 const double* anum, const double* cw, const double* logden,
                                 double* psum_part , int* blocks_out);
hipError_t launch_shift_logden(hipStream_t s, const double* logden, const double* cw, double alpha, int64_t N,
                               double* out, const LoopCtl& lc = LoopCtl());

hipError_t launch_reduce(hipStream_t s, const double* part, int64_t nparts, int64_t count,
                         double* scratch, double* out);
hipError_t launch_lognum(hipStream_t s, const double* u, int64_t ld, int64_t N, int64_t K,
                         const double* anum, const double* logden,
                         double* pmax , double* psum , int64_t nchunks);
int64_t lognum_chunks(int64_t N, int64_t K);
hipError_t launch_lognum_merge(hipStream_t s, const double* pmax, const double* psum, int64_t K,
                               int64_t nchunks, double* out_max , double* out_sum );
hipError_t launch_logw(hipStream_t s, const double* u, int64_t ld, int64_t N, int64_t K,
                       const double* f, const double* logden, double* out, int64_t ld_out, bool exponentiate = false);
hipError_t launch_check_u(hipStream_t s, const double* u, int64_t ld, int64_t N, int64_t K, int* flags);
hipError_t launch_generate_harmonic(hipStream_t s, double* u, int64_t ld, int64_t N, int64_t K,
                                    uint64_t seed, const double* O_k, const double* K_k,
                                    const int64_t* cumN , int64_t n_global0);
hipError_t launch_sci_update(hipStream_t s, const double* part, int64_t nparts, int64_t rows, const double* Nk,
                             const double* lnNk, int64_t K, int64_t Kp, int first_state, double tol, double* f,
                             double* aden, double* f_hist, double* delta_out);
struct SciLoopArgs {
    const double* Nk;
    const double* lnNk;
    int K;
    int first;
    double tol;
    double* state;
    double* rec;
    int64_t nrec;
    double* f_hist;
    double* delta_out;
    int parity;
    uint32_t live;
    int balanced;
    int pingpong;
    long long* stamps;
};
hipError_t launch_sci_small(hipStream_t s, int nb, const LaunchGeom& g, const double* u, int64_t ld, int64_t N, const double* cw,
                            const SciLoopArgs& q);
hipError_t launch_bootstrap_counts(hipStream_t s, uint64_t seed, int64_t replicate, const int64_t* cum, int64_t K, int64_t total,
                                   const int64_t* order, int64_t n0, int64_t N, double* cw);
hipError_t launch_weights_from_log(hipStream_t s, const double* v, double p, int64_t n, double* cw, double* cwsq, int* overflow);
hipError_t launch_reduce_level1(hipStream_t s, const double* part, int64_t nparts, int64_t count, double* out,
                                int64_t* nchunks);
hipError_t launch_mfma_peak(hipStream_t s, int blocks, int iters, double* sink);
hipError_t launch_reduce2(hipStream_t s, const double* partA, int64_t countA, const double* partB, int64_t countB,
                          int64_t nparts, double* scratch, double* outA, double* outB);

struct LoopSrc {
    const double* p[8];
    int n;
};
hipError_t launch_loop_reduce(hipStream_t s, const LoopSrc& src, int64_t count, int op , double* out);

struct AdaptArgs {
    const double* gram_red;
    const double* lse_red;
    double* f;
    double* psum;
    double* cand;
    double* ratio;
    double* aden;
    double* anum;
    const double* Nk;
    const double* lnNk;
    const int* sampled;
    int m, K, Kp;
    int* ctl;
    const double* prm;
    double* state;
    double* hist;
    int64_t hist_cap;
    int pmode;
    const double* a0;
    double* ccur;
    int fused;
    double* cgram;
    int light_ok;
    long long* stamps;
    int newton_ldlt;
};
LaunchGeom psweep_geometry(int nb, int num_cu, int64_t ntiles, int64_t grid_override);
hipError_t launch_psweep(hipStream_t s, int nb, int nf, const LaunchGeom& g, const double* P, int64_t ld, int64_t N,
                         const double* cmul, const double* cw, double* rinv0, double* rinv1, double* psum_part,
                         const LoopCtl& lc = LoopCtl());
LaunchGeom fused_geometry(int nb, int num_cu, int64_t ntiles, int64_t grid_override, bool unit = false);
hipError_t launch_fused(hipStream_t s, int nb, const LaunchGeom& g, const double* P, int64_t ld, int64_t N, const double* cmul,
                        const double* cw, const double* wsq, bool unit, double* rinv_base, double* gram_part, double* psum_part,
                        const LoopCtl& lc);
LaunchGeom build_sweep_geometry(int nb, int num_cu, int64_t ntiles, int64_t grid_override);
hipError_t launch_build_sweep(hipStream_t s, int nb, const LaunchGeom& g, const double* u, int64_t ld, int64_t N,
                              const double* aden, const double* cw, double* P, double* rinv_slot, double* psum_part);
LaunchGeom build_gram_geometry(int nb, int num_cu, int64_t ntiles, int64_t grid_override);
hipError_t launch_build_gram(hipStream_t s, int nb, const LaunchGeom& g, const double* u, int64_t ld, int64_t N,
                             const double* aden, const double* wsq, bool general, double* P, double* rinv_slot, double* gram_part);

hipError_t launch_make_p(hipStream_t s, int num_cu, const double* u, int64_t ld, int64_t N, int64_t rows, const double* aden,
                         const double* logden, double* P);
hipError_t launch_fill(hipStream_t s, double* v, double value, int64_t n);
hipError_t launch_zero(hipStream_t s, void* p, size_t bytes);
hipError_t launch_sqrt_vec(hipStream_t s, double* dst, const double* src, int64_t n);
hipError_t launch_rinv_from_logden(hipStream_t s, const double* ld0, const double* ldv, const double* cw, bool weighted, int64_t N,
                                   double* out);
hipError_t launch_rinv_weighted(hipStream_t s, const double* rinv, const double* cw, int64_t N, double* out,
                                const LoopCtl& lc = LoopCtl());
hipError_t launch_newton(hipStream_t s, const AdaptArgs& a);
constexpr size_t NEWTON_CHOL_WORK = (size_t)256 * 256 + 8;
hipError_t launch_newton_chol(hipStream_t s, const AdaptArgs& a, double* work);
hipError_t launch_select(hipStream_t s, const AdaptArgs& a);
hipError_t launch_select_newton(hipStream_t s, const AdaptArgs& a);
hipError_t launch_ctl_resume(hipStream_t s, int* ctl);


enum : int { KDE_GAUSSIAN = 0, KDE_TOPHAT = 1, KDE_EPANECHNIKOV = 2, KDE_EXPONENTIAL = 3, KDE_LINEAR = 4, KDE_COSINE = 5 };
constexpr int KDE_MAX_D = 8;
constexpr int KDE_TILE = 64;
constexpr int KDE_MAX_CB = 32;
struct KdeLaunch {
    int kernel, d, cb;
    const double* X;
    int64_t ldx;
    const double* V;
    const double* Q;
    int64_t ldq, M;
    double coef;
    double h, inv_h, inv_h2;
    int64_t qblocks, nchunks, chunk;
    double* part;
};
size_t kde_lds_bytes(int kernel, int d, int cb);
hipError_t launch_kde(hipStream_t s, const KdeLaunch& a);
hipError_t launch_kde_combine(hipStream_t s, const KdeLaunch& a, int cv, const double* logW, double lognorm, double* out, int* flag);
hipError_t launch_kde_exact(hipStream_t s, const KdeLaunch& a, int64_t N, int64_t npairs, const int64_t* pq, const double* logW,
                            double lognorm, double* out);

constexpr int BSP_MAX_K = 7;
constexpr int BSP_MAX_BASIS = 1024;
constexpr int BSP_MAX_GROUPS = 1024;
constexpr int BSP_MAX_CB = 32;
constexpr int BSP_SLAB_ENTRIES = 768;
struct BsplineLaunch {
    int k, nbasis, cb;
    const double* X;
    const int* G;
    const double* V;
    int64_t N;
    const double* t;
    int64_t nchunks, chunk;
    int cells, tile_cells, ntiles;
    double* part;
};
size_t bspline_lds_bytes(int k, int nbasis, int tile_cells, int cb);
hipError_t launch_bspline(hipStream_t s, const BsplineLaunch& a);
hipError_t launch_bspline_combine(hipStream_t s, const BsplineLaunch& a, double* out);

constexpr int ACF_WG = 256;
constexpr int ACF_R = 8;
constexpr int ACF_TILE = ACF_WG * ACF_R;
constexpr int ACF_MAX_LAGS = 64;
enum : int { ACF_AUTO = 0, ACF_CROSS = 1, ACF_PLAIN = 2 };
enum : int { ACF_RULE_SUFFIX = 0, ACF_RULE_MULTIPLE = 1 };
enum : int { ACF_RUNNING = 0, ACF_STOPPED = 1, ACF_ZERO_VARIANCE = 2, ACF_END = 3 };
struct AcfLaunch {
    int kind, nacc;
    const double2* A;
    const double2* B;
    const int* rem;
    int64_t T, ldx, ntiles;
    int nl;
    int64_t lag[ACF_MAX_LAGS];
    int64_t inc[ACF_MAX_LAGS];
    double den[ACF_MAX_LAGS];
    int64_t kbase;
    int64_t tile_lo, atile_hi;
    double2* tot;
    double2* off;
};
struct AcfRule {
    int mode, fft;
    int64_t nskip, norig;
    int64_t mintime;
    double navg;
    int64_t tend;
    const double2* SA;
    const double2* SB;
    double* g;
    double* sig2;
    double2* dA;
    double2* dB;
    int* status;
    int64_t* stop;
    double* ct;
    int* active;
};
hipError_t launch_acf_tiles(hipStream_t s, const AcfLaunch& a);
hipError_t launch_acf_scan(hipStream_t s, const AcfLaunch& a);
hipError_t launch_acf_store(hipStream_t s, const AcfLaunch& a, int64_t c_lo, int64_t c_hi, const int* oid, double2* out, int64_t ldo);
hipError_t launch_acf_rule(hipStream_t s, const AcfLaunch& a, const AcfRule& r, int64_t c_lo, int64_t c_hi);
hipError_t launch_acf_rule_init(hipStream_t s, const AcfRule& r, int64_t T, int64_t last_change);
hipError_t launch_acf_finish(hipStream_t s, const AcfLaunch& a, const double2* q, int64_t norig, const int64_t* orig, int segments,
                             const double2* SA, const double2* SB, double* xab, double* xba, int64_t j0);
hipError_t launch_acf_fill_int(hipStream_t s, int* p, int64_t n, int v);
hipError_t launch_acf_scatter_oid(hipStream_t s, int* oid, const int64_t* orig, int64_t norig);


enum : int64_t { BAR_RUNNING = 0, BAR_DONE = 1, BAR_NAN_BRACKET = 2, BAR_BOUNDS = 3, BAR_NOT_CONVERGED = 4 };
enum : int64_t { BAR_FALSE_POSITION = 0, BAR_BISECTION = 1, BAR_SELF_CONSISTENT = 2 };
enum : int64_t { BAR_PH_INIT = 0, BAR_PH_BRACKET0 = 1, BAR_PH_WIDEN = 2, BAR_PH_LOOP = 3 };

MBAR_HD inline void bar_finish_loop(mbar_bar_state& s, bool broke) {
    if (!broke) s.iteration = s.maximum_iterations;
    s.nreq = 0;
    s.status = (s.iterated && !(s.iteration < s.maximum_iterations)) ? BAR_NOT_CONVERGED : BAR_DONE;
}

MBAR_HD inline int64_t bar_advance(mbar_bar_state& s, const double* F) {
#pragma clang fp contract(off)
    if (s.status != BAR_RUNNING) return s.status;
    const bool bracketed = s.method != BAR_SELF_CONSISTENT;
    switch (s.phase) {
    case BAR_PH_INIT:
        s.DeltaF_initial = s.DeltaF;
        s.iteration = 0;
        s.nzero = 0;
        if (bracketed) {
            s.req[0] = s.UpperB;
            s.req[1] = s.LowerB;
            s.nreq = 2;
            s.phase = BAR_PH_BRACKET0;
            return s.status;
        }
        break;
    case BAR_PH_BRACKET0:
    case BAR_PH_WIDEN: {
        s.FUpperB = F[0];
        s.FLowerB = F[1];
        s.nzero += 2;
        if (s.phase == BAR_PH_BRACKET0 && (s.FUpperB != s.FUpperB || s.FLowerB != s.FLowerB)) {
            s.DeltaF = 0.0;
            s.nreq = 0;
            s.status = BAR_NAN_BRACKET;
            return s.status;
        }
        if (s.FUpperB * s.FLowerB > 0) {
            const double FAve = (s.UpperB + s.LowerB) / 2;
            const double du = fabs(s.UpperB - FAve), dl = fabs(s.LowerB - FAve);
// ... 306 lines not shown
```

### pymbar_amd/csrc/mbar_k_fused.hip

```cpp
#include "mbar_device.h"

namespace mbar {

template <int NB>
__host__ __device__ constexpr int fused_steps_done(int I) {
    if (I < 0) return 0;
    if (I >= NB - 2) return 2 * NB;
    if (NB < 4) return 2 * (I + 1) < 2 * NB ? 2 * (I + 1) : 2 * NB;
    const int r1 = (NB + 1) / 2 - 1;
    if (I <= r1) return 2 * (I + 1) < NB ? 2 * (I + 1) : NB;
    const int rows = NB - 2 - r1;
    return NB + (NB * (I - r1) + rows - 1) / rows;
}
template <int NB, bool WIDE, bool UNIT>
__global__ void __launch_bounds__(256, 1)
k_fused(const double* __restrict__ P, int64_t ld, int64_t N, int64_t ntiles, const double* __restrict__ cmul,
        const double* __restrict__ cw, const double* __restrict__ wsq, double* __restrict__ rinv0,
        double* __restrict__ rinv1, double* __restrict__ gram_part, double* __restrict__ psum_part,
        const int* __restrict__ ctl, int64_t slot_stride) {
    extern __shared__ __attribute__((aligned(16))) char smem[];
    if (ctl) {
        if (ctl[CTL_DONE] != 0 || ctl[CTL_LIGHT] != 0) return;
        const int s = ctl[CTL_SLOT];
        rinv1 = rinv0 + (int64_t)((s + 2) % 3) * slot_stride;
        rinv0 = rinv0 + (int64_t)((s + 1) % 3) * slot_stride;
    }
    constexpr int ROWS = NB * 16;
    constexpr int NDMA = ROWS / 8 + (UNIT ? 0 : 1);
    constexpr int U_BYTES = ROWS * TS * 8;
    constexpr int TILE_BYTES = U_BYTES + (UNIT ? 0 : 1024);
    constexpr int NBLK = NB * (NB + 1) / 2;
    constexpr bool PINNED = NBLK > GRAM_AGPR_BLOCKS;
    constexpr bool ACC1 = NB < FUSED_PSUM1_FROM_GRAM_NB;
    const int lane = threadIdx.x & 63;
    const int wave = __builtin_amdgcn_readfirstlane(threadIdx.x >> 6);
    const int nwv = blockDim.x >> 6;
    const int ks = lane & 15, ns = lane >> 4;
    char* buf = smem + wave * (2 * TILE_BYTES);
    const int64_t gw = (int64_t)blockIdx.x * nwv + wave;
    const int64_t W = (int64_t)gridDim.x * nwv;
    RowIdentity rows{0};
    const StageOffsetsT<WIDE> so = make_stage_offsets<WIDE>(ld, lane);

    double acc[2][NB];
#pragma unroll
    for (int f = 0; f < 2; ++f)
#pragma unroll
        for (int I = 0; I < NB; ++I) acc[f][I] = 0.0;
    {
        double cany[NB];
#pragma unroll
        for (int I = 0; I < NB; ++I) cany[I] = fabs(cmul[16 * I + ks]) + fabs(cmul[ROWS + 16 * I + ks]);
        if constexpr (NB <= 2) rows.live = live_piece_mask<NB>(cany, 0.0);
    }
    constexpr int NSTEP = ROWS / 4;
    double cb[UNIT ? NSTEP : 1];
    if constexpr (UNIT) {
#pragma unroll
        for (int st = 0; st < NSTEP; ++st) {
            const double cv = cmul[(lane & 1) * ROWS + 4 * st + (lane >> 4)];
            cb[st] = (lane & 3) < 2 ? cv : 0.0;
            asm volatile("" : "+v"(cb[st]));
        }
    } else {
        double* ctab = reinterpret_cast<double*>(smem + nwv * (2 * TILE_BYTES));
        for (int e = threadIdx.x; e < NSTEP * 16; e += blockDim.x) ctab[e] = (e & 3) < 2 ? cmul[(e & 3) * ROWS + (e >> 2)] : 0.0;
        __syncthreads();
    }
    int apos[4];
#pragma unroll
    for (int q = 0; q < 4; ++q) apos[q] = ns * (TS * 8) + (((lane & 15) + (ns & 2) + 4 * q) & 15) * 8;
    v4d G[NBLK];
#pragma unroll
    for (int b = 0; b < NBLK; ++b) G[b] = v4d{0.0, 0.0, 0.0, 0.0};

    const int rd_base = ks * (TS * 8);
    int pos[GROUPS];
#pragma unroll
    for (int g = 0; g < GROUPS; ++g) pos[g] = ((4 * g + ns + (ks & 14)) & 15) * 8;
    const int sq = ns + 4 * ((lane >> 2) & 3);
    const int fq = lane & 3;

    const char* wsrc = reinterpret_cast<const char*>(((lane >> 3) & 1) ? wsq : cw) + (lane & 7) * 16;
    auto stage_w = [&](int64_t tile, char* dst) {
        __builtin_amdgcn_global_load_lds((const __attribute__((address_space(1))) void*)(wsrc + tile * (TS * 8)),
                                         (__attribute__((address_space(3))) void*)(dst + U_BYTES), 16, 0, 0);
    };
    auto stage = [&](int64_t tile, char* dst) {
        stage_tile<ROWS, true, 0, 1>(P, ld, tile * TS, dst, lane, so, rows);
        if constexpr (!UNIT) stage_w(tile, dst);
    };
    auto read_group = [&](const char* tb, int g, double (&x)[NB], double& wg, double& swg) {
        if constexpr (!UNIT) {
            wg = *reinterpret_cast<const double*>(tb + U_BYTES + (4 * g + ns) * 8);
            swg = *reinterpret_cast<const double*>(tb + U_BYTES + TS * 8 + (4 * g + ns) * 8);
        }
#pragma unroll
        for (int I = 0; I < NB; ++I) x[I] = *reinterpret_cast<const double*>(tb + I * (16 * TS * 8) + rd_base + pos[g]);
    };
    uint32_t cop_off = (uint32_t)(nwv * (2 * TILE_BYTES) + (lane >> 4) * 32 + (lane & 3) * 8);
    auto read_step = [&](const char* tb, int st, double& a, double& b) {
        a = *reinterpret_cast<const double*>(tb + st * (4 * TS * 8) + apos[st & 3]);
        if constexpr (UNIT) b = cb[st];
        else b = *reinterpret_cast<const double*>(smem + cop_off + st * 128);
    };
    auto mfma4 = [&](double& d, double a, double b, bool first) {
        if constexpr (PINNED) {
            if (first)
                asm volatile("v_mfma_f64_4x4x4_4b_f64 %0, %1, %2, 0" : "=v"(d) : "v"(a), "v"(b));
            else
                asm volatile("v_mfma_f64_4x4x4_4b_f64 %0, %1, %2, %0" : "+v"(d) : "v"(a), "v"(b));
        } else {
            d = __builtin_amdgcn_mfma_f64_4x4x4f64(a, b, first ? 0.0 : d, 0, 0, 0);
        }
    };
    auto store_rinv = [&](int64_t tile, double& r) {
        const int64_t n = tile * TS + sq;
        double* out = fq ? rinv1 : rinv0;
        if constexpr (UNIT) r = n < N ? r : 0.0;
        if (n < N && fq < 2) out[n] = r;
    };
    int64_t t = gw;
    int cur = 0;
    double rcur = 0.0;
    double uv[2][NB], w[2], sw[2];
    if (t < ntiles) {
        stage(t, buf);
        if (t + W < ntiles) {
            stage(t + W, buf + TILE_BYTES);
            wait_vm<NDMA>();
        } else {
            wait_vm<0>();
        }
        double sa = 0.0, sb = 0.0;
#pragma unroll
        for (int st = 0; st < NSTEP; st += 2) {
            double a0, b0, a1, b1;
            read_step(buf, st, a0, b0);
            read_step(buf, st + 1, a1, b1);
            sa = __builtin_amdgcn_mfma_f64_4x4x4f64(a0, b0, sa, 0, 0, 0);
            sb = __builtin_amdgcn_mfma_f64_4x4x4f64(a1, b1, sb, 0, 0, 0);
        }
        rcur = recip_fast(fmax(sa + sb, 1e-300));
        store_rinv(t, rcur);
        read_group(buf, 0, uv[0], w[0], sw[0]);
    }
    for (; t < ntiles; t += W) {
        char* cbuf = buf + cur * TILE_BYTES;
        char* nbuf = buf + (cur ^ 1) * TILE_BYTES;
        const int64_t tn = t + W, tnn = t + 2 * W;
        const int64_t tstage = tnn < ntiles ? tnn : t;
        if constexpr (!UNIT) asm volatile("" : "+v"(cop_off));
        double sacc[4];
#pragma unroll
        for (int g = 0; g < GROUPS; ++g) {
            const int gc = g & 1, gn = gc ^ 1;
            if (g == 2) wait_vm<1>();
            double r0, r1;
            switch (g) {
                case 0: r0 = row16_bcast<0>(rcur); r1 = row16_bcast<1>(rcur); break;
                case 1: r0 = row16_bcast<4>(rcur); r1 = row16_bcast<5>(rcur); break;
                case 2: r0 = row16_bcast<8>(rcur); r1 = row16_bcast<9>(rcur); break;
                default: r0 = row16_bcast<12>(rcur); r1 = row16_bcast<13>(rcur); break;
            }
            const double q0 = UNIT ? r0 : w[gc] * r0, q1 = UNIT ? r1 : w[gc] * r1;
#pragma unroll
            for (int I = 0; I < NB; ++I) {
                acc[0][I] = fma(uv[gc][I], q0, acc[0][I]);
                if constexpr (ACC1) acc[1][I] = fma(uv[gc][I], q1, acc[1][I]);
                settle(acc[0][I]);
                if constexpr (ACC1) settle(acc[1][I]);
            }
            const double rin = UNIT ? r1 : r1 * sw[gc];
            double p[NB];
#pragma unroll
            for (int I = 0; I < NB; ++I) p[I] = uv[gc][I] * rin;
            constexpr int B1 = NB >= 4 ? NB : 2 * NB;
            double opa[B1], opb[B1];
            auto request_next = [&]() {
                if (g < GROUPS - 1) {
                    read_group(cbuf, g + 1, uv[gn], w[gn], sw[gn]);
                } else {
                    read_group(nbuf, 0, uv[gn], w[gn], sw[gn]);
                }
            };
            auto request_steps = [&]() {
                if (g >= 2) {
#pragma unroll
                    for (int q = 0; q < B1; ++q) read_step(nbuf, (g - 2) * 2 * NB + q, opa[q], opb[q]);
                }
            };
            if constexpr (!PINNED) {
                request_next();
                request_steps();
            }
            auto mfma = [&](int b, double x, double y) {
                if constexpr (PINNED) {
                    if (b < GRAM_AGPR_BLOCKS)
                        asm volatile("v_mfma_f64_16x16x4_f64 %0, %1, %2, %0" : "+a"(G[b]) : "v"(x), "v"(y));
                    else
                        asm volatile("v_mfma_f64_16x16x4_f64 %0, %1, %2, %0" : "+v"(G[b]) : "v"(x), "v"(y));
                } else {
                    G[b] = __builtin_amdgcn_mfma_f64_16x16x4f64(x, y, G[b], 0, 0, 0);
                }
            };
            if constexpr (PINNED) {
                __builtin_amdgcn_sched_barrier(0);
                asm volatile("s_nop 7");
            }
            constexpr int NM = NBLK;
            int b = 0, nm = 0;
#pragma unroll
            for (int I = 0; I < NB; ++I) {
                if (NB == 1 && g >= 2) {
                    mfma4(sacc[2 * (g & 1)], opa[0], opb[0], true);
                    mfma4(sacc[2 * (g & 1) + 1], opa[1], opb[1], true);
                }
#pragma unroll
                for (int J = I; J < NB; ++J) {
                    mfma(b, p[I], p[J]);
                    if constexpr (PINNED) {
                        if (nm == 0 || nm == 1) {
                            __builtin_amdgcn_sched_barrier(0);
                            if (nm == 0) request_next(); else request_steps();
                            __builtin_amdgcn_sched_barrier(0);
                        }
                    }
                    if (g == GROUPS - 1) {
#pragma unroll
                        for (int j = nm * NDMA / NM; j < (nm + 1) * NDMA / NM; ++j) {
                            if constexpr (PINNED) __builtin_amdgcn_sched_barrier(0);
                            if (j < ROWS / 8)
                                stage_piece<true>(P + rows(8 * j) * ld + rows.cols(j, tstage * TS), so.off[j & 1], cbuf + j * 1024, lane);
                            else if constexpr (!UNIT)
                                stage_w(tstage, cbuf);
                            if constexpr (PINNED) __builtin_amdgcn_sched_barrier(0);
                        }
                    }
                    ++b;
                    ++nm;
                }
                if (g >= 2 && NB > 1 && I < NB - 1) {
#pragma unroll
                    for (int q = fused_steps_done<NB>(I - 1); q < fused_steps_done<NB>(I); ++q)
                        mfma4(sacc[q & 3], opa[q % B1], opb[q % B1], g == 2 && q < 4);
                    if (B1 < 2 * NB && fused_steps_done<NB>(I - 1) < B1 && fused_steps_done<NB>(I) >= B1) {
#pragma unroll
                        for (int q = 0; q < B1; ++q) read_step(nbuf, (g - 2) * 2 * NB + B1 + q, opa[q], opb[q]);
                    }
                }
            }
            if constexpr (PINNED) __builtin_amdgcn_sched_barrier(0);
        }
        if constexpr (PINNED)
            asm volatile("s_nop 7\n\ts_nop 7" : "+v"(sacc[0]), "+v"(sacc[1]), "+v"(sacc[2]), "+v"(sacc[3]));
        rcur = recip_fast(fmax((sacc[0] + sacc[1]) + (sacc[2] + sacc[3]), 1e-300));
        store_rinv(tn, rcur);
        cur ^= 1;
    }
    if constexpr (PINNED) asm volatile("s_nop 15\n\ts_nop 15" ::: "memory");
#pragma unroll
    for (int f = 0; f < 2; ++f) {
#pragma unroll
        for (int I = 0; I < NB; ++I) {
            double v = acc[f][I];
            v += __shfl_xor(v, 16);
            v += __shfl_xor(v, 32);
            if (lane < 16) psum_part[(gw * 2 + f) * ROWS + 16 * I + lane] = v;
        }
    }
    {
        int b = 0;
#pragma unroll
        for (int I = 0; I < NB; ++I)
#pragma unroll
            for (int J = I; J < NB; ++J, ++b) {
#pragma unroll
                for (int r = 0; r < 4; ++r) {
#if defined(MBAR_GRAM_STORE_NT)
                    __builtin_nontemporal_store(G[b][r], &gram_part[((gw * NBLK + b) * 4 + r) * 64 + lane]);
#else
                    gram_part[((gw * NBLK + b) * 4 + r) * 64 + lane] = G[b][r];
#endif
                }
            }
    }
}



LaunchGeom fused_geometry(int nb, int num_cu, int64_t ntiles, int64_t grid_override, bool unit) {
    LaunchGeom g;
    g.waves = 4;
    g.variant = 1;
    if (nb > 8) {
        g.variant = 6;
        g.lds_bytes = (size_t)2 * ((size_t)nb * 16 * TS * 8 + 4 * 1024) + 1024;
        int64_t capq = grid_override > 0 ? grid_override : num_cu;
        int64_t wantq = ntiles < 1 ? 1 : ntiles;
        g.blocks = (int)(wantq < capq ? wantq : capq);
        g.nwaves = g.blocks;
        g.psum_records = g.nwaves;
        return g;
    }
    const size_t tile = (size_t)nb * 16 * TS * 8 + 1024;
    const size_t lds_general = (size_t)4 * 2 * tile + (size_t)nb * 512;
    g.lds_bytes = unit ? (size_t)4 * 2 * (tile - 1024) : lds_general;
    int64_t want = (ntiles + 3) / 4;
    int64_t cap = num_cu;
    if (nb <= 5) {
        static const int occ[6] = {1, 4, 4, 3, 2, 2};
        const int by_lds = blocks_per_cu_for(lds_general);
        cap = (int64_t)num_cu * (by_lds < occ[nb] ? by_lds : occ[nb]);
        int64_t by_work = (ntiles + 127) / 128;
        if (by_work < num_cu) by_work = num_cu;
        if (cap > by_work) cap = by_work;
    }
    if (grid_override > 0) cap = grid_override;
    if (want < 1) want = 1;
    g.blocks = (int)(want < cap ? want : cap);
    g.nwaves = g.blocks * 4;
    g.psum_records = g.nwaves;
    return g;
}
template <int NB>
static hipError_t launch_fused_nb(hipStream_t s, const LaunchGeom& g, const double* P, int64_t ld, int64_t N, const double* cmul,
                                  const double* cw, const double* wsq, bool unit, double* rinv0, double* gp, double* pp, const LoopCtl& lc) {
    auto go = [&](auto kern) -> hipError_t {
        if (g.lds_bytes > 64 * 1024) {
            hipError_t e = hipFuncSetAttribute(reinterpret_cast<const void*>(kern),
                                               hipFuncAttributeMaxDynamicSharedMemorySize, (int)g.lds_bytes);
            if (e != hipSuccess) return e;
        }
        const int64_t ntiles = (N + TS - 1) / TS;
        double* r1 = nullptr;
        if (lc.ev_start && lc.ev_stop)
            hipExtLaunchKernelGGL(kern, dim3(g.blocks), dim3(256), g.lds_bytes, s, lc.ev_start, lc.ev_stop, 0, P, ld, N, ntiles, cmul,
                                  cw, wsq, rinv0, r1, gp, pp, lc.ctl, lc.slot_stride);
        else
            hipLaunchKernelGGL(kern, dim3(g.blocks), dim3(256), g.lds_bytes, s, P, ld, N, ntiles, cmul, cw, wsq, rinv0, r1, gp, pp,
                               lc.ctl, lc.slot_stride);
        return hipGetLastError();
    };
    if (unit) return stage_offsets_wide(ld) ? go(k_fused<NB, true, true>) : go(k_fused<NB, false, true>);
    return stage_offsets_wide(ld) ? go(k_fused<NB, true, false>) : go(k_fused<NB, false, false>);
}
hipError_t launch_fused(hipStream_t s, int nb, const LaunchGeom& g, const double* P, int64_t ld, int64_t N, const double* cmul,
                        const double* cw, const double* wsq, bool unit, double* rinv_base, double* gram_part, double* psum_part,
                        const LoopCtl& lc) {
    if (!lc.ctl) return hipErrorInvalidValue;
    if (nb == 12 || nb == 16) return launch_fused_quad(s, nb, g, P, ld, N, cmul, cw, wsq, rinv_base, gram_part, psum_part, lc);
    switch (nb) {
#define MBAR_CASE(NB_) \
    case NB_: return launch_fused_nb<NB_>(s, g, P, ld, N, cmul, cw, wsq, unit, rinv_base, gram_part, psum_part, lc);
        MBAR_CASE(1) MBAR_CASE(2) MBAR_CASE(3) MBAR_CASE(4) MBAR_CASE(5) MBAR_CASE(6) MBAR_CASE(7) MBAR_CASE(8)
#undef MBAR_CASE
        default: return hipErrorInvalidValue;
    }
}

}
```

### pymbar_amd/csrc/mbar_k_pmode.hip

```cpp
#include "mbar_device.h"

namespace mbar {

__global__ void __launch_bounds__(256)
k_rinv_weighted(const double* __restrict__ rinv, const double* __restrict__ cw, int64_t N, double* __restrict__ out,
                const int* __restrict__ ctl, int64_t slot_stride) {
    if (ctl) {
        if (ctl[CTL_DONE] != 0) return;
        rinv += (int64_t)ctl[CTL_SLOT] * slot_stride;
    }
    for (int64_t n = (int64_t)blockIdx.x * blockDim.x + threadIdx.x; n < N; n += (int64_t)gridDim.x * blockDim.x)
        out[n] = rinv[n] * sqrt(cw[n]);
}

__global__ void __launch_bounds__(256)
k_rinv_from_logden(const double* __restrict__ ld0, const double* __restrict__ ldv, const double* __restrict__ cw, int weighted,
                   int64_t N, double* __restrict__ out) {
    for (int64_t n = (int64_t)blockIdx.x * blockDim.x + threadIdx.x; n < N; n += (int64_t)gridDim.x * blockDim.x) {
        double r = exp(ld0[n] - ldv[n]);
        if (weighted) r *= sqrt(cw[n]);
        out[n] = r;
    }
}
hipError_t launch_rinv_from_logden(hipStream_t s, const double* ld0, const double* ldv, const double* cw, bool weighted, int64_t N,
                                   double* out) {
    int64_t bx = (N + 255) / 256;
    if (bx > 2048) bx = 2048;
    if (bx < 1) bx = 1;
    hipLaunchKernelGGL(k_rinv_from_logden, dim3((unsigned)bx), dim3(256), 0, s, ld0, ldv, cw, weighted ? 1 : 0, N, out);
    return hipGetLastError();
}

typedef double v2d __attribute__((ext_vector_type(2)));
__device__ __forceinline__ void store_p16(char* dst, const double2& v) {
#if defined(MBAR_P_STORE_NT)
    __builtin_nontemporal_store(v2d{v.x, v.y}, reinterpret_cast<v2d*>(dst));
#else
    *reinterpret_cast<double2*>(dst) = v;
#endif
}
template <int NB>
__device__ __forceinline__ void build_two_groups(char* cbuf, int rd0, int rd1, const double (&a)[NB], double (&acc)[NB],
                                                 double w0, double w1) {
    double x0[NB], x1[NB];
#pragma unroll
    for (int I = 0; I < NB; ++I) {
        x0[I] = *reinterpret_cast<const double*>(cbuf + I * (16 * TS * 8) + rd0);
        x1[I] = *reinterpret_cast<const double*>(cbuf + I * (16 * TS * 8) + rd1);
    }
    __builtin_amdgcn_sched_barrier(0);
#pragma unroll
    for (int I = 0; I < NB; ++I) {
        x0[I] = a[I] - x0[I];
        x1[I] = a[I] - x1[I];
    }
    double m0 = tree_max<NB>(x0), m1 = tree_max<NB>(x1);
    row16_max2(m0, m1);
    const double m2_0 = m0 * LOG2E_S, m2_1 = m1 * LOG2E_S;
#pragma unroll
    for (int I = 0; I < NB; ++I) {
        x0[I] = fma(x0[I], LOG2E_S, -m2_0);
        x1[I] = fma(x1[I], LOG2E_S, -m2_1);
    }
    exp2s_batch2<NB>(x0, x1);
    double s0 = tree_sum<NB>(x0), s1 = tree_sum<NB>(x1);
    row16_sum2(s0, s1);
    const double ri0 = recip_fast(s0), ri1 = recip_fast(s1);
#pragma unroll
    for (int I = 0; I < NB; ++I) {
        x0[I] *= ri0;
        x1[I] *= ri1;
        acc[I] = fma(x1[I], w1, fma(x0[I], w0, acc[I]));
        *reinterpret_cast<double*>(cbuf + I * (16 * TS * 8) + rd0) = x0[I];
        *reinterpret_cast<double*>(cbuf + I * (16 * TS * 8) + rd1) = x1[I];
    }
}
template <int NB, bool WIDE>
__global__ void __launch_bounds__(64 * lse_waves(NB))
k_build_sweep(const double* __restrict__ u, int64_t ld, int64_t N, int64_t ntiles, const double* __restrict__ aden,
              const double* __restrict__ cw, double* __restrict__ P, double* __restrict__ rinv_slot,
              double* __restrict__ psum_part) {
    extern __shared__ __attribute__((aligned(16))) char smem[];
    constexpr int ROWS = NB * 16;
    constexpr int NDMA = ROWS / 8;
    constexpr int U_BYTES = ROWS * TS * 8;
    constexpr int TILE_BYTES = U_BYTES + TS * 8;
    const int lane = threadIdx.x & 63;
    const int wave = __builtin_amdgcn_readfirstlane(threadIdx.x >> 6);
    const int nwv = blockDim.x >> 6;
    const int ks = lane & 15, ns = lane >> 4;
    exp_table_init(smem);
    __syncthreads();
    char* buf = smem + EXP_TABLE_BYTES + wave * (2 * TILE_BYTES);
    const int64_t gw = (int64_t)blockIdx.x * nwv + wave;
    const int64_t W = (int64_t)gridDim.x * nwv;
    RowIdentity rows{0};
    const StageOffsetsT<WIDE> so = make_stage_offsets<WIDE>(ld, lane);

    double a[NB], acc[NB];
#pragma unroll
    for (int I = 0; I < NB; ++I) {
        a[I] = aden[16 * I + ks];
        acc[I] = 0.0;
    }
#pragma unroll
    for (int I = 0; I < NB; ++I) settle(a[I]);
    rows.live = live_piece_mask<NB>(a, -INFINITY);
    const int rd_base = ks * (TS * 8);
    int pos[GROUPS];
#pragma unroll
    for (int g = 0; g < GROUPS; ++g) pos[g] = rd_base + ((4 * g + ns + (ks & 14)) & 15) * 8;

    int64_t t = gw;
    int cur = 0;
    if (t < ntiles) {
        stage_tile<ROWS, true, 0, 1>(u, ld, t * TS, buf, lane, so, rows);
        stage_vec16<true>(cw, t * TS, buf + U_BYTES, lane);
    }
    for (; t < ntiles; t += W) {
        char* cbuf = buf + cur * TILE_BYTES;
        const char* wslot = cbuf + U_BYTES;
        const int64_t tn = t + W;
        if (tn < ntiles) {
            char* nbuf = buf + (cur ^ 1) * TILE_BYTES;
            stage_tile<ROWS, true, 0, 1>(u, ld, tn * TS, nbuf, lane, so, rows);
            stage_vec16<true>(cw, tn * TS, nbuf + U_BYTES, lane);
            if (t != gw)
                wait_vm<2 * (NDMA + 1)>();
            else
                wait_vm<NDMA + 1>();
        } else {
            wait_vm<0>();
        }
        double w[GROUPS];
#pragma unroll
        for (int g = 0; g < GROUPS; ++g) w[g] = *reinterpret_cast<const double*>(wslot + (4 * g + ns) * 8);
        build_two_groups<NB>(cbuf, pos[0], pos[1], a, acc, w[0], w[1]);
        build_two_groups<NB>(cbuf, pos[2], pos[3], a, acc, w[2], w[3]);
        __builtin_amdgcn_fence(__ATOMIC_RELEASE, "wavefront");
        __builtin_amdgcn_wave_barrier();
#pragma unroll
        for (int j = 0; j < NDMA; ++j) {
            const double2 v = *reinterpret_cast<const double2*>(cbuf + j * 1024 + lane * 16);
            char* dst = reinterpret_cast<char*>(P + (int64_t)(8 * j) * ld + t * TS) + so.off[j & 1];
            store_p16(dst, v);
        }
        {
            const int64_t n = t * TS + lane;
            if (lane < TS && n < N) rinv_slot[n] = 1.0;
        }
        cur ^= 1;
    }
#pragma unroll
    for (int I = 0; I < NB; ++I) {
        double v = acc[I];
        v += __shfl_xor(v, 16);
        v += __shfl_xor(v, 32);
        if (lane < 16) psum_part[gw * ROWS + 16 * I + lane] = v;
    }
}

template <int NB, bool WIDE, bool GENERAL>
__global__ void __launch_bounds__(256, 1)
k_build_gram(const double* __restrict__ u, int64_t ld, int64_t N, int64_t ntiles, const double* __restrict__ aden,
             const double* __restrict__ wsq, double* __restrict__ P, double* __restrict__ rinv_slot, double* __restrict__ gram_part) {
    extern __shared__ __attribute__((aligned(16))) char smem[];
    constexpr int ROWS = NB * 16;
    constexpr int NDMA = ROWS / 8;
    constexpr int U_BYTES = ROWS * TS * 8;
    constexpr int TILE_BYTES = U_BYTES + TS * 8;
    constexpr int NBLK = NB * (NB + 1) / 2;
    constexpr bool PINNED = NBLK > GRAM_AGPR_BLOCKS;
    const int lane = threadIdx.x & 63;
    const int wave = __builtin_amdgcn_readfirstlane(threadIdx.x >> 6);
    const int nwv = blockDim.x >> 6;
    const int ks = lane & 15, ns = lane >> 4;
    exp_table_init(smem);
    __syncthreads();
    char* buf = smem + EXP_TABLE_BYTES + wave * (2 * TILE_BYTES);
    const int64_t gw = (int64_t)blockIdx.x * nwv + wave;
    const int64_t W = (int64_t)gridDim.x * nwv;
    RowIdentity rows{0};
    const StageOffsetsT<WIDE> so = make_stage_offsets<WIDE>(ld, lane);

    double aL[NB];
    {
        double a[NB];
#pragma unroll
        for (int I = 0; I < NB; ++I) a[I] = aden[16 * I + ks];
        if constexpr (NB <= 2) rows.live = live_piece_mask<NB>(a, -INFINITY);
#pragma unroll
        for (int I = 0; I < NB; ++I) aL[I] = a[I] > -INFINITY ? a[I] * LOG2E_S : -1.0e9;
    }
#pragma unroll
    for (int I = 0; I < NB; ++I) settle(aL[I]);
    v4d G[NBLK];
#pragma unroll
    for (int b = 0; b < NBLK; ++b) G[b] = v4d{0.0, 0.0, 0.0, 0.0};
    const int rd_base = ks * (TS * 8);
    int pos[GROUPS];
#pragma unroll
    for (int g = 0; g < GROUPS; ++g) pos[g] = rd_base + ((4 * g + ns + (ks & 14)) & 15) * 8;

    auto stage = [&](int64_t tile, char* dst) {
        stage_tile<ROWS, true, 0, 1>(u, ld, tile * TS, dst, lane, so, rows);
        stage_vec16<true>(wsq, tile * TS, dst + U_BYTES, lane);
    };
    int64_t t = gw;
    int cur = 0;
    if (t < ntiles) stage(t, buf);
    for (; t < ntiles; t += W) {
        char* cbuf = buf + cur * TILE_BYTES;
        const int64_t tn = t + W;
        if (tn < ntiles) {
            stage(tn, buf + (cur ^ 1) * TILE_BYTES);
            if (t != gw)
                wait_vm<2 * (NDMA + 1)>();
            else
                wait_vm<NDMA + 1>();
        } else {
            wait_vm<0>();
        }
        const int nvalid = (int)(N - t * TS < TS ? N - t * TS : TS);
        auto mfma = [&](int b, double xx, double yy) {
            if constexpr (PINNED) {
                if (b < GRAM_AGPR_BLOCKS)
                    asm("v_mfma_f64_16x16x4_f64 %0, %1, %2, %0" : "+a"(G[b]) : "v"(xx), "v"(yy));
                else
                    asm("v_mfma_f64_16x16x4_f64 %0, %1, %2, %0" : "+v"(G[b]) : "v"(xx), "v"(yy));
            } else {
                G[b] = __builtin_amdgcn_mfma_f64_16x16x4f64(xx, yy, G[b], 0, 0, 0);
            }
        };
#pragma unroll
        for (int g = 0; g < GROUPS; g += 2) {
            double x0[NB], x1[NB];
#pragma unroll
            for (int I = 0; I < NB; ++I) {
                x0[I] = *reinterpret_cast<const double*>(cbuf + I * (16 * TS * 8) + pos[g]);
                x1[I] = *reinterpret_cast<const double*>(cbuf + I * (16 * TS * 8) + pos[g + 1]);
            }
            __builtin_amdgcn_sched_barrier(0);
#pragma unroll
            for (int I = 0; I < NB; ++I) {
                x0[I] = fma(x0[I], -LOG2E_S, aL[I]);
                x1[I] = fma(x1[I], -LOG2E_S, aL[I]);
            }
            double m0 = tree_max<NB>(x0), m1 = tree_max<NB>(x1);
            row16_max2(m0, m1);
#pragma unroll
            for (int I = 0; I < NB; ++I) {
                x0[I] = m0 - x0[I];
                x1[I] = m1 - x1[I];
            }
            exp2s_neg_batch2<NB, GENERAL>(x0, x1);
            double s0 = tree_sum<NB>(x0), s1 = tree_sum<NB>(x1);
            row16_sum2(s0, s1);
            double ri0 = recip_fast(s0), ri1 = recip_fast(s1);
            if (4 * g + ns >= nvalid) ri0 = 0.0;
            if (4 * g + 4 + ns >= nvalid) ri1 = 0.0;
            double p0[NB], p1[NB];
            if constexpr (GENERAL) {
                const double sw0 = *reinterpret_cast<const double*>(cbuf + U_BYTES + (4 * g + ns) * 8);
                const double sw1 = *reinterpret_cast<const double*>(cbuf + U_BYTES + (4 * g + 4 + ns) * 8);
#pragma unroll
                for (int I = 0; I < NB; ++I) {
                    x0[I] *= ri0;
                    x1[I] *= ri1;
                    *reinterpret_cast<double*>(cbuf + I * (16 * TS * 8) + pos[g]) = x0[I];
                    *reinterpret_cast<double*>(cbuf + I * (16 * TS * 8) + pos[g + 1]) = x1[I];
                    p0[I] = x0[I] * sw0;
                    p1[I] = x1[I] * sw1;
                }
            } else {
#pragma unroll
                for (int I = 0; I < NB; ++I) {
                    p0[I] = x0[I] * ri0;
                    p1[I] = x1[I] * ri1;
                    *reinterpret_cast<double*>(cbuf + I * (16 * TS * 8) + pos[g]) = p0[I];
                    *reinterpret_cast<double*>(cbuf + I * (16 * TS * 8) + pos[g + 1]) = p1[I];
                }
            }
            if constexpr (PINNED) {
                __builtin_amdgcn_sched_barrier(0);
                asm volatile("s_nop 7");
            }
            {
                int b = 0;
#pragma unroll
                for (int I = 0; I < NB; ++I)
#pragma unroll
                    for (int J = I; J < NB; ++J) mfma(b++, p0[I], p0[J]);
            }
            {
                int b = 0;
#pragma unroll
                for (int I = 0; I < NB; ++I)
#pragma unroll
                    for (int J = I; J < NB; ++J) mfma(b++, p1[I], p1[J]);
            }
            if constexpr (PINNED) __builtin_amdgcn_sched_barrier(0);
        }
        __builtin_amdgcn_fence(__ATOMIC_RELEASE, "wavefront");
        __builtin_amdgcn_wave_barrier();
#pragma unroll
        for (int j = 0; j < NDMA; ++j) {
            const double2 v = *reinterpret_cast<const double2*>(cbuf + j * 1024 + lane * 16);
            char* dst = reinterpret_cast<char*>(P + (int64_t)(8 * j) * ld + t * TS) + so.off[j & 1];
            store_p16(dst, v);
        }
        {
            const int64_t n = t * TS + lane;
            if (lane < TS && n < N) rinv_slot[n] = 1.0;
        }
        cur ^= 1;
    }
    if constexpr (PINNED) asm volatile("s_nop 15\n\ts_nop 15" ::: "memory");
#pragma unroll
    for (int b = 0; b < NBLK; ++b)
#pragma unroll
        for (int r = 0; r < 4; ++r) gram_part[((gw * NBLK + b) * 4 + r) * 64 + lane] = G[b][r];
}

template <int NB, int NF>
__device__ __forceinline__ void psweep_two_groups(const char* cbuf, int rd0, int rd1, const double (&c)[NF][NB],
                                                  double (&acc)[NF][NB], double w0, double w1, double (&r0)[NF],
                                                  double (&r1)[NF]) {
    double x0[NB], x1[NB];
#pragma unroll
    for (int I = 0; I < NB; ++I) {
        x0[I] = *reinterpret_cast<const double*>(cbuf + I * (16 * TS * 8) + rd0);
        x1[I] = *reinterpret_cast<const double*>(cbuf + I * (16 * TS * 8) + rd1);
    }
    __builtin_amdgcn_sched_barrier(0);
#pragma unroll
    for (int f = 0; f < NF; ++f) {
        double s0 = dot_sum<NB>(x0, c[f]), s1 = dot_sum<NB>(x1, c[f]);
        row16_sum2(s0, s1);
        r0[f] = recip_fast(fmax(s0, 1e-300));
        r1[f] = recip_fast(fmax(s1, 1e-300));
        const double q0 = w0 * r0[f], q1 = w1 * r1[f];
#pragma unroll
        for (int I = 0; I < NB; ++I) acc[f][I] = fma(x1[I], q1, fma(x0[I], q0, acc[f][I]));
    }
}

template <int NB, int NF, bool WIDE>
__global__ void __launch_bounds__(64 * lse_waves(NB))
k_psweep(const double* __restrict__ P, int64_t ld, int64_t N, int64_t ntiles, const double* __restrict__ cmul,
         const double* __restrict__ cw, double* __restrict__ rinv0, double* __restrict__ rinv1,
         double* __restrict__ psum_part, const int* __restrict__ ctl, int64_t slot_stride, int light_only) {
    extern __shared__ __attribute__((aligned(16))) char smem[];
    if (ctl) {
        if (ctl[CTL_DONE] != 0) return;
        if (light_only && ctl[CTL_LIGHT] == 0) return;
        const int s = ctl[CTL_SLOT];
        rinv1 = rinv0 + (int64_t)((s + 2) % 3) * slot_stride;
        rinv0 = rinv0 + (int64_t)((s + 1) % 3) * slot_stride;
    }
    constexpr int ROWS = NB * 16;
    constexpr int U_BYTES = ROWS * TS * 8;
    constexpr int TILE_BYTES = U_BYTES + TS * 8;
    const int lane = threadIdx.x & 63;
    const int wave = __builtin_amdgcn_readfirstlane(threadIdx.x >> 6);
    const int nwv = blockDim.x >> 6;
    const int ks = lane & 15, ns = lane >> 4;
    char* buf = smem + wave * (2 * TILE_BYTES);
    const int64_t gw = (int64_t)blockIdx.x * nwv + wave;
    const int64_t W = (int64_t)gridDim.x * nwv;
    RowIdentity rows{0};
    const StageOffsetsT<WIDE> so = make_stage_offsets<WIDE>(ld, lane);

    double c[NF][NB], acc[NF][NB];
#pragma unroll
    for (int f = 0; f < NF; ++f)
#pragma unroll
        for (int I = 0; I < NB; ++I) {
            c[f][I] = cmul[f * ROWS + 16 * I + ks];
            acc[f][I] = 0.0;
        }
#pragma unroll
    for (int f = 0; f < NF; ++f)
#pragma unroll
        for (int I = 0; I < NB; ++I) settle(c[f][I]);
    {
        double cany[NB];
#pragma unroll
        for (int I = 0; I < NB; ++I) cany[I] = NF == 2 ? fabs(c[0][I]) + fabs(c[NF - 1][I]) : c[0][I];
        rows.live = live_piece_mask<NB>(cany, 0.0);
    }
    const int rd_base = ks * (TS * 8);
    int pos[GROUPS];
#pragma unroll
    for (int g = 0; g < GROUPS; ++g) pos[g] = rd_base + ((4 * g + ns + (ks & 14)) & 15) * 8;
    const int gq = ks & 3;
    const int fq = (NF == 2 && (ks & 4)) ? 1 : 0;

    int64_t t = gw;
    int cur = 0;
    if (t < ntiles) {
        stage_tile<ROWS, true, 0, 1>(P, ld, t * TS, buf, lane, so, rows);
        stage_vec16<true>(cw, t * TS, buf + U_BYTES, lane);
    }
    for (; t < ntiles; t += W) {
        char* cbuf = buf + cur * TILE_BYTES;
        const char* wslot = cbuf + U_BYTES;
        const int64_t tn = t + W;
        if (tn < ntiles) {
            char* nbuf = buf + (cur ^ 1) * TILE_BYTES;
            stage_tile<ROWS, true, 0, 2>(P, ld, tn * TS, nbuf, lane, so, rows);
            stage_vec16<true>(cw, tn * TS, nbuf + U_BYTES, lane);
            constexpr int NEVEN = (ROWS / 8 + 1) / 2 + 1;
            if (t != gw)
                wait_vm<NEVEN + 1>();
            else
                wait_vm<NEVEN>();
        } else {
            wait_vm<0>();
        }
        double w[GROUPS];
#pragma unroll
        for (int g = 0; g < GROUPS; ++g) w[g] = *reinterpret_cast<const double*>(wslot + (4 * g + ns) * 8);
        double ra[NF], rb[NF], keep = 0.0;
        psweep_two_groups<NB, NF>(cbuf, pos[0], pos[1], c, acc, w[0], w[1], ra, rb);
        if (gq == 0) keep = ra[fq];
        if (gq == 1) keep = rb[fq];
        __builtin_amdgcn_sched_barrier(0);
        if (tn < ntiles) stage_tile<ROWS, true, 1, 2>(P, ld, tn * TS, buf + (cur ^ 1) * TILE_BYTES, lane, so, rows);
        __builtin_amdgcn_sched_barrier(0);
        psweep_two_groups<NB, NF>(cbuf, pos[2], pos[3], c, acc, w[2], w[3], ra, rb);
        if (gq == 2) keep = ra[fq];
        if (gq == 3) keep = rb[fq];
        {
            const int64_t n = t * TS + 4 * gq + ns;
            double* out = fq ? rinv1 : rinv0;
            if (n < N && ks < 4 * NF) out[n] = keep;
        }
        cur ^= 1;
    }
#pragma unroll
    for (int f = 0; f < NF; ++f) {
#pragma unroll
        for (int I = 0; I < NB; ++I) {
            double v = acc[f][I];
            v += __shfl_xor(v, 16);
            v += __shfl_xor(v, 32);
            if (lane < 16) psum_part[(gw * NF + f) * ROWS + 16 * I + lane] = v;
        }
    }
}



LaunchGeom psweep_geometry(int nb, int num_cu, int64_t ntiles, int64_t grid_override) {
    LaunchGeom g;
    const size_t tile = (size_t)nb * 16 * TS * 8 + TS * 8;
    g.variant = 1;
    g.waves = lse_waves(nb);
    g.lds_bytes = (size_t)g.waves * 2 * tile;
    int64_t want = (ntiles + g.waves - 1) / g.waves;
    int64_t cap = (int64_t)num_cu * blocks_per_cu_for(g.lds_bytes);
    if (grid_override > 0) cap = grid_override;
    if (want < 1) want = 1;
    g.blocks = (int)(want < cap ? want : cap);
    g.nwaves = g.blocks * g.waves;
    g.psum_records = g.nwaves;
    return g;
}

template <int NB>
static hipError_t launch_psweep_nb(hipStream_t s, int nf, const LaunchGeom& g, const double* P, int64_t ld, int64_t N,
                                   const double* cmul, const double* cw, double* rinv0, double* rinv1, double* pp,
                                   const LoopCtl& lc) {
    auto go = [&](auto kern) -> hipError_t {
        if (g.lds_bytes > 64 * 1024) {
            hipError_t e = hipFuncSetAttribute(reinterpret_cast<const void*>(kern),
                                               hipFuncAttributeMaxDynamicSharedMemorySize, (int)g.lds_bytes);
            if (e != hipSuccess) return e;
        }
        const int64_t ntiles = (N + TS - 1) / TS;
        if (lc.ev_start && lc.ev_stop)
            hipExtLaunchKernelGGL(kern, dim3(g.blocks), dim3(g.waves * 64), g.lds_bytes, s, lc.ev_start, lc.ev_stop, 0, P, ld, N,
                                  ntiles, cmul, cw, rinv0, rinv1, pp, lc.ctl, lc.slot_stride, lc.light_only ? 1 : 0);
        else
            hipLaunchKernelGGL(kern, dim3(g.blocks), dim3(g.waves * 64), g.lds_bytes, s, P, ld, N, ntiles, cmul, cw, rinv0,
                               rinv1, pp, lc.ctl, lc.slot_stride, lc.light_only ? 1 : 0);
        return hipGetLastError();
    };
    const bool wide = stage_offsets_wide(ld);
    if (nf == 1) return wide ? go(k_psweep<NB, 1, true>) : go(k_psweep<NB, 1, false>);
    return wide ? go(k_psweep<NB, 2, true>) : go(k_psweep<NB, 2, false>);
}

hipError_t launch_psweep(hipStream_t s, int nb, int nf, const LaunchGeom& g, const double* P, int64_t ld, int64_t N,
                         const double* cmul, const double* cw, double* rinv0, double* rinv1, double* pp, const LoopCtl& lc) {
    switch (nb) {
#define MBAR_CASE(NB_) \
    case NB_: return launch_psweep_nb<NB_>(s, nf, g, P, ld, N, cmul, cw, rinv0, rinv1, pp, lc);
        MBAR_CASE(1) MBAR_CASE(2) MBAR_CASE(3) MBAR_CASE(4) MBAR_CASE(5) MBAR_CASE(6) MBAR_CASE(7) MBAR_CASE(8)
#undef MBAR_CASE
        default: return hipErrorInvalidValue;
    }
}

hipError_t launch_rinv_weighted(hipStream_t s, const double* rinv, const double* cw, int64_t N, double* out,
                                const LoopCtl& lc) {
    int64_t bx = (N + 255) / 256;
    if (bx > 2048) bx = 2048;
    if (bx < 1) bx = 1;
    hipLaunchKernelGGL(k_rinv_weighted, dim3((unsigned)bx), dim3(256), 0, s, rinv, cw, N, out, lc.ctl, lc.slot_stride);
    return hipGetLastError();
}

template <int NB>
static hipError_t launch_build_sweep_nb(hipStream_t s, const LaunchGeom& g, const double* u, int64_t ld, int64_t N,
                                        const double* aden, const double* cw, double* P, double* rinv_slot, double* pp) {
    auto go = [&](auto kern) -> hipError_t {
        if (g.lds_bytes > 64 * 1024) {
            hipError_t e = hipFuncSetAttribute(reinterpret_cast<const void*>(kern),
                                               hipFuncAttributeMaxDynamicSharedMemorySize, (int)g.lds_bytes);
            if (e != hipSuccess) return e;
        }
        const int64_t ntiles = (N + TS - 1) / TS;
        hipLaunchKernelGGL(kern, dim3(g.blocks), dim3(g.waves * 64), g.lds_bytes, s, u, ld, N, ntiles, aden, cw, P, rinv_slot, pp);
        return hipGetLastError();
    };
    return stage_offsets_wide(ld) ? go(k_build_sweep<NB, true>) : go(k_build_sweep<NB, false>);
}
LaunchGeom build_sweep_geometry(int nb, int num_cu, int64_t ntiles, int64_t grid_override) {
    return lse_geometry(nb, 1, num_cu, ntiles, grid_override, 1);
}
hipError_t launch_build_sweep(hipStream_t s, int nb, const LaunchGeom& g, const double* u, int64_t ld, int64_t N,
                              const double* aden, const double* cw, double* P, double* rinv_slot, double* pp) {
    switch (nb) {
#define MBAR_CASE(NB_) \
    case NB_: return launch_build_sweep_nb<NB_>(s, g, u, ld, N, aden, cw, P, rinv_slot, pp);
        MBAR_CASE(1) MBAR_CASE(2) MBAR_CASE(3) MBAR_CASE(4) MBAR_CASE(5) MBAR_CASE(6) MBAR_CASE(7) MBAR_CASE(8)
#undef MBAR_CASE
        default: return hipErrorInvalidValue;
    }
}

LaunchGeom build_gram_geometry(int nb, int num_cu, int64_t ntiles, int64_t grid_override) {
    LaunchGeom g = fused_geometry(nb, num_cu, ntiles, grid_override);
    g.lds_bytes = (size_t)4 * 2 * ((size_t)nb * 16 * TS * 8 + TS * 8) + EXP_TABLE_BYTES;
    return g;
}
template <int NB>
static hipError_t launch_build_gram_nb(hipStream_t s, const LaunchGeom& g, const double* u, int64_t ld, int64_t N,
                                       const double* aden, const double* wsq, bool general, double* P, double* rinv_slot, double* gp) {
    auto go = [&](auto kern) -> hipError_t {
        if (g.lds_bytes > 64 * 1024) {
            hipError_t e = hipFuncSetAttribute(reinterpret_cast<const void*>(kern),
                                               hipFuncAttributeMaxDynamicSharedMemorySize, (int)g.lds_bytes);
            if (e != hipSuccess) return e;
        }
        const int64_t ntiles = (N + TS - 1) / TS;
        hipLaunchKernelGGL(kern, dim3(g.blocks), dim3(256), g.lds_bytes, s, u, ld, N, ntiles, aden, wsq, P, rinv_slot, gp);
        return hipGetLastError();
    };
    if (general) return stage_offsets_wide(ld) ? go(k_build_gram<NB, true, true>) : go(k_build_gram<NB, false, true>);
    return stage_offsets_wide(ld) ? go(k_build_gram<NB, true, false>) : go(k_build_gram<NB, false, false>);
}
hipError_t launch_build_gram(hipStream_t s, int nb, const LaunchGeom& g, const double* u, int64_t ld, int64_t N,
                             const double* aden, const double* wsq, bool general, double* P, double* rinv_slot, double* gram_part) {
    switch (nb) {
#define MBAR_CASE(NB_) \
    case NB_: return launch_build_gram_nb<NB_>(s, g, u, ld, N, aden, wsq, general, P, rinv_slot, gram_part);
        MBAR_CASE(1) MBAR_CASE(2) MBAR_CASE(3) MBAR_CASE(4) MBAR_CASE(5) MBAR_CASE(6) MBAR_CASE(7) MBAR_CASE(8)
#undef MBAR_CASE
        default: return hipErrorInvalidValue;
    }
}

}
```

### pymbar_amd/csrc/mbar_loops.cpp

```cpp
#include "mbar_ctx.h"

using namespace mbar;
using namespace mbar::host;

namespace mbar {
namespace host {

int adaptive_host_loop(mbar_ctx* c, std::vector<double>& f, double tol, int64_t maxiter, int64_t min_sc_iter, double gamma,
                       int check_convergence, double* history, int64_t history_rows, mbar_solve_result& res,
                       std::vector<double>& psum, double& max_delta) {
    const int64_t K = c->K;
    const int m = (int)c->sampled.size();
    const int first = c->sampled[0];
    std::vector<double> f_old(K), cand(2 * (size_t)K), psum2(2 * (size_t)K);
    std::vector<double> H((size_t)m * m), g(m), x;
    std::vector<int> pos((size_t)K, -1);
    for (int i = 0; i < m; ++i) pos[(size_t)c->sampled[i]] = i;
    psum.assign(K, 0.0);
    int cur = 0;
    int rc = eval_core(c, f.data(), 1, 0, c->logden[cur], nullptr, psum.data(), nullptr, nullptr);
    if (rc) return rc;
    bool done = false;
    const GramPlan plan = plan_for(c);
    const bool dbg = std::getenv("MBAR_DEBUG_TIMING") != nullptr;
// ... 185 lines not shown
            res.sci_iter++;
            choice = 0;
        } else {
            std::copy(f_nr, f_nr + K, f.begin());
            std::copy(psum2.begin() + K, psum2.end(), psum.begin());
            cur = sB;
            res.nr_iter++;
            choice = 1;
        }
        const double small = std::min(1e-8, tol);
        max_delta = 0.0;
        double max_diff = 0.0;
        bool nan_seen = false;
        for (int i = 1; i < m; ++i) {
            const int k = c->sampled[i];
            const double div = std::fabs(f[k]) < small ? 1.0 : std::fabs(f[k]);
            const double d1 = std::fabs(f[k] - f_old[k]) / div, d2 = std::fabs(f_sci[k] - f_nr[k]) / div;
            if (std::isnan(d1)) nan_seen = true;
            max_delta = std::max(max_delta, d1);
            max_diff = std::max(max_diff, d2);
        }
        if (nan_seen) max_delta = std::numeric_limits<double>::quiet_NaN();
        res.iterations = it + 1;
        res.gram_sweeps += 1;
        if (history && it < history_rows) {
            history[4 * it + 0] = choice;
            history[4 * it + 1] = std::sqrt(gn_sci);
            history[4 * it + 2] = std::sqrt(gn_nr);
            history[4 * it + 3] = max_delta;
        }
        double stop = (check_convergence && (std::isnan(max_delta) || (max_delta < tol && max_diff < std::sqrt(tol)))) ? 1.0 : 0.0;
        if (check_convergence) {
            rc = agree_with_rank0(c, &stop, 1);
            if (rc) return rc;
        }
        if (stop > 0.5) {
            res.success = 1;
            done = true;
        }
    }
    const int64_t nit = res.iterations - it0;
    if (dbg && nit > 0)
        std::fprintf(stderr, "[mbar] adaptive (host loop): %lld it, per it: passA %.3f ms (of it unpacking %.3f), host solve %.3f ms (of it the factorisation + substitutions %.3f), passB %.3f ms, total %.3f ms\n",
                     (long long)nit, tA / nit, tA_unpack / nit, tH / nit, tH_solve / nit, tB / nit, (now_ms() - t0) / nit);
    return MBAR_OK;
}

bool device_loop_eligible(const mbar_ctx* c) {
    if (!c->opt_device_loop || !use_fast(c)) return false;
    if (c->nranks > 1 && !stream_transport(c)) return false;
    const int64_t ntiles = (c->N + TS - 1) / TS;
    const LaunchGeom gl = lse_geometry((int)(c->Kp / 16), 2, c->num_cu, ntiles, c->opt_grid, lse_variant_for(c));
    if (c->Kp > 128) return c->opt_device_loop_wide && use_quad(c) && gl.variant == 5;
    return gl.variant == 1;
}

inline size_t ad_off_f(const mbar_ctx*) { return 0; }
inline size_t ad_off_psum(const mbar_ctx* c) { return (size_t)c->Kp; }
inline size_t ad_off_cand(const mbar_ctx* c) { return (size_t)2 * c->Kp; }
inline size_t ad_off_ratio(const mbar_ctx* c) { return (size_t)4 * c->Kp; }
inline size_t ad_off_prm(const mbar_ctx* c) { return (size_t)5 * c->Kp; }
inline size_t ad_off_state(const mbar_ctx* c) { return (size_t)5 * c->Kp + 4; }
inline size_t ad_off_hist(const mbar_ctx* c) { return (size_t)5 * c->Kp + 8; }

int ensure_ad(mbar_ctx* c, int64_t hist_rows) {
    const int64_t cap = std::max<int64_t>(1024, std::min<int64_t>(hist_rows, 1 << 20));
    if (!c->ad || c->ad_hist_cap < cap) {
        int rc = drop_graphs(c);
        if (rc) return rc;
        if (c->ad) HIPCHK(c, cache_free(c->ad));
        c->ad = nullptr;
        HIPCHK(c, cache_malloc((void**)&c->ad, (ad_off_hist(c) + (size_t)4 * cap) * sizeof(double)));
        c->ad_hist_cap = cap;
    }
    if (!c->ad_ints) HIPCHK(c, cache_malloc((void**)&c->ad_ints, (size_t)(CTL_WORDS + c->Kp) * sizeof(int)));
    if (!c->h_ctl) HIPCHK(c, cache_host_malloc((void**)&c->h_ctl, (size_t)CTL_WORDS * sizeof(int)));
    return MBAR_OK;
}

int agree_all_ok(mbar_ctx* c, bool& ok) {
    if (c->nranks <= 1) return MBAR_OK;
    double v = ok ? 0.0 : 1.0;
    int rc = allreduce_host(c, &v, 1, 1);
    if (rc) return rc;
    ok = !(v > 0.0);
    return MBAR_OK;
}

int adaptive_device_loop(mbar_ctx* c, std::vector<double>& f, double tol, int64_t maxiter, int64_t min_sc_iter, double gamma,
                         int check_convergence, double* history, int64_t history_rows, mbar_solve_result& res,
                         std::vector<double>& psum, double& max_delta, bool& handed_back) {
    const int64_t K = c->K, Kp = c->Kp;
    const int m = (int)c->sampled.size();
    const int nb = (int)(Kp / 16);
    const int64_t ntiles = (c->N + TS - 1) / TS;
    handed_back = false;
    c->ld0_valid = false;
    psum.assign(K, 0.0);
    const bool wide = Kp > 128;
    bool pmode = c->opt_pmode && !c->P_failed && (!wide || (c->opt_wide_pmode && c->opt_fused));
    int arc = ensure_ad(c, history ? history_rows : 0);
    if (!arc && wide && !c->chol && cache_malloc((void**)&c->chol, NEWTON_CHOL_WORK * sizeof(double)) != hipSuccess)
        arc = fail(c, MBAR_ERR_HIP, "allocation of the Newton workspace failed");
    if (!arc && pmode && !c->P) {
        arc = drop_graphs(c);
        if (!arc) {
            if (cache_malloc((void**)&c->P, (size_t)Kp * c->ld * sizeof(double)) != hipSuccess) {
                (void)hipGetLastError();
                c->P = nullptr;
                c->P_failed = true;
                pmode = false;
            } else if (launch_zero(c->stream, c->P, (size_t)Kp * c->ld * sizeof(double)) != hipSuccess) {
                arc = fail(c, MBAR_ERR_HIP, "zero fill of P failed");
            }
        }
    }
    {
        bool p_ok = pmode;
        int rc = agree_all_ok(c, p_ok);
        if (rc) return rc;
        if (pmode && !p_ok) {
            pmode = false;
            c->error = "resident probability matrix does not fit on every rank: classic sweeps";
        }
    }
    if (!arc && pmode && !c->pm_vec && cache_malloc((void**)&c->pm_vec, (size_t)3 * Kp * sizeof(double)) != hipSuccess)
        arc = fail(c, MBAR_ERR_HIP, "allocation of the P-mode vectors failed");
    const bool fused = pmode && c->opt_fused;
    bool light = fused && check_convergence && c->opt_light_last != 0 &&
                 (c->opt_light_last >= 2 || (nb >= 5 && (double)Kp * (double)c->N >= 5.0e7));
    LaunchGeom gg = wide ? gram_quad_geometry(nb, c->num_cu, ntiles, c->opt_grid)
                         : gram_geometry(nb * 16, true, c->num_cu, ntiles, c->opt_grid);
    const bool unit = !c->weighted && !c->opt_fused_general;
    LaunchGeom gl = fused ? fused_geometry(nb, c->num_cu, ntiles, c->opt_grid, unit)
                    : pmode ? psweep_geometry(nb, c->num_cu, ntiles, c->opt_grid)
                            : lse_geometry(nb, 2, c->num_cu, ntiles, c->opt_grid, lse_variant_for(c));
    if (wide) gg.live_blocks = gl.live_blocks = quad_live_blocks(c);
    if (fused) {
        gg.blocks = gl.blocks;
        gg.nwaves = gl.nwaves;
    }
    LaunchGeom gp = psweep_geometry(wide ? 8 : nb, c->num_cu, ntiles, 0);
    if (light && !wide && gl.nwaves % gp.waves != 0) light = false;
    if (light && !wide) {
        gp.blocks = gl.nwaves / gp.waves;
        gp.nwaves = gp.psum_records = gl.nwaves;
    }
    {
        bool l_ok = light;
        int rcl = agree_all_ok(c, l_ok);
        if (rcl) return rcl;
        light = light && l_ok;
    }
    const LaunchGeom gb = fused ? build_gram_geometry(nb, c->num_cu, ntiles, c->opt_grid)
                                : build_sweep_geometry(nb, c->num_cu, ntiles, c->opt_grid);
    const size_t rec_g = (size_t)nb * (nb + 1) / 2 * 256;
    const size_t rec_l = (size_t)2 * Kp;
    const size_t off_gram = rec_l + 2;
    if (!arc) arc = ensure_red(c, off_gram + rec_g);
    if (!arc)
        arc = ensure(c, &c->part, &c->part_doubles,
                     std::max(std::max((size_t)gg.nwaves * rec_g, (size_t)gl.nwaves * (rec_l + 2)), (size_t)gb.nwaves * Kp));
    if (!arc)
        arc = ensure(c, &c->scratch, &c->scratch_doubles,
                     std::max(((size_t)std::max(gg.nwaves, gl.nwaves) / 32 + 1) * (rec_g + rec_l + 2), ((size_t)gb.nwaves / 32 + 1) * (Kp + rec_g)));
    if (!arc && c->weighted && !c->lden_eff) arc = fail(c, MBAR_ERR_STATE, "weighted context without its logden buffer");
    if (!arc && fused) arc = ensure(c, &c->part_g, &c->part_g_doubles, (size_t)gl.nwaves * rec_g);
    {
        bool ok = arc == MBAR_OK;
        const std::string local_err = c->error;
        int rc = agree_all_ok(c, ok);
        if (rc) return rc;
        if (arc) return arc;
        if (!ok) return fail(c, MBAR_ERR_STATE, "a peer rank could not allocate its solver buffers");
        c->error = local_err;
    }
    int rc = MBAR_OK;
    LoopCtl lc_slot, lc_flat;
    lc_slot.ctl = lc_flat.ctl = c->ad_ints;
    lc_slot.slot_stride = c->ld;
    lc_slot.unclamped = lc_flat.unclamped = c->u_checked && !c->u_posinf;
    lc_slot.pmode = lc_flat.pmode = pmode;
    std::vector<double> an0((size_t)Kp), cm0((size_t)Kp, 0.0);
    build_aden(c, f.data(), an0.data(), Kp);
    bool warm = fused && c->opt_pcache && c->P_valid && (int64_t)c->P_a0.size() == Kp;
    for (int64_t k = 0; warm && k < Kp; ++k) {
        const bool live = !std::isinf(an0[k]), was = !std::isinf(c->P_a0[k]);
        if (live != was) warm = false;
        else if (live) {
            const double d = an0[k] - c->P_a0[k];
            if (!(std::fabs(d) < 200.0)) warm = false;
            cm0[k] = std::exp(d);
        }
    }
    rc = agree_all_ok(c, warm);
    if (rc) return rc;
    if (!pmode) {
        rc = eval_core(c, f.data(), 1, 0, c->logden[0], nullptr, psum.data(), nullptr, nullptr);
        if (rc) return rc;
    } else if (warm) {
        std::vector<int> z((size_t)CTL_WORDS, 0);
        HIPCHK(c, hipMemcpyAsync(c->ad_ints, z.data(), z.size() * sizeof(int), hipMemcpyHostToDevice, c->stream));
        std::copy(cm0.begin(), cm0.end(), c->hstage);
        std::copy(cm0.begin(), cm0.end(), c->hstage + Kp);
        HIPCHK(c, hipMemcpyAsync(d_aden(c), c->hstage, (size_t)2 * Kp * sizeof(double), hipMemcpyHostToDevice, c->stream));
        HIPCHK(c, hipMemsetAsync(c->red, 0, off_gram * sizeof(double), c->stream));
        {
            ScopedTimer t(c, MBAR_TIMER_OTHER);
            HIPCHK(c, launch_fused(c->stream, nb, gl, c->P, c->ld, c->N, d_aden(c), c->cw, c->weighted ? c->cwsq : c->cw, unit,
                                   c->logden[0], c->part_g, c->part, lc_slot));
        }
        HIPCHK(c, launch_reduce2(c->stream, c->part, (int64_t)rec_l, c->part_g, (int64_t)rec_g, gl.nwaves, c->scratch, c->red,
                                 c->red + off_gram));
        rc = allreduce_dev(c, c->red, (int64_t)(off_gram + rec_g), 0);
        if (rc) return rc;
        HIPCHK(c, hipMemcpyAsync(c->hred, c->red, (size_t)Kp * sizeof(double), hipMemcpyDeviceToHost, c->stream));
        rc = sync_stream(c);
        if (rc) return rc;
        for (int64_t k = 0; k < K; ++k) psum[k] = c->hred[k] * cm0[k];
        res.warm_starts += 1;
    } else if (wide) {
        c->P_valid = false;
        rc = eval_core(c, f.data(), 1, 0, c->logden[1], nullptr, psum.data(), nullptr, nullptr);
        if (rc) return rc;
        if (fused && !c->weighted) {
            ScopedTimer t(c, MBAR_TIMER_OTHER);
            HIPCHK(c, launch_gram_quad(c->stream, nb, gg, c->u, c->ld, c->N, d_aden(c), c->logden[1], c->part_g, LoopCtl(), c->P));
            HIPCHK(c, launch_reduce(c->stream, c->part_g, gg.nwaves, (int64_t)rec_g, c->scratch, c->red + off_gram));
            rc = allreduce_dev(c, c->red + off_gram, (int64_t)rec_g, 0);
            if (rc) return rc;
            HIPCHK(c, launch_fill(c->stream, c->logden[0], 1.0, c->ld));
        } else {
            ScopedTimer t(c, MBAR_TIMER_OTHER);
            HIPCHK(c, launch_make_p(c->stream, c->num_cu, c->u, c->ld, c->N, Kp, d_aden(c), c->logden[1], c->P));
            HIPCHK(c, launch_fill(c->stream, c->logden[0], 1.0, c->ld));
        }
        if (fused && c->weighted) {
            const double* lden = c->logden[0];
            if (c->weighted) {
                HIPCHK(c, launch_rinv_weighted(c->stream, c->logden[0], c->cw, c->N, c->lden_eff));
                lden = c->lden_eff;
            }
            LoopCtl lp;
            lp.pmode = true;
            {
                ScopedTimer t(c, MBAR_TIMER_GRAM);
                HIPCHK(c, launch_gram_quad(c->stream, nb, gg, c->P, c->ld, c->N, d_anum(c), lden, c->part_g, lp));
            }
            HIPCHK(c, launch_reduce(c->stream, c->part_g, gg.nwaves, (int64_t)rec_g, c->scratch, c->red + off_gram));
            rc = allreduce_dev(c, c->red + off_gram, (int64_t)rec_g, 0);
            if (rc) return rc;
        }
        rc = sync_stream(c);
        if (rc) return rc;
        c->P_a0 = an0;
        c->P_valid = true;
        res.builds += 1;
    } else {
        c->P_valid = false;
        build_aden(c, f.data(), c->hstage, Kp);
        HIPCHK(c, hipMemcpyAsync(d_aden(c), c->hstage, (size_t)Kp * sizeof(double), hipMemcpyHostToDevice, c->stream));
        HIPCHK(c, hipMemsetAsync(c->red, 0, off_gram * sizeof(double), c->stream));
        {
            ScopedTimer t(c, MBAR_TIMER_OTHER);
            if (fused)
                HIPCHK(c, launch_build_gram(c->stream, nb, gb, c->u, c->ld, c->N, d_aden(c), c->weighted ? c->cwsq : c->cw,
                                            c->weighted || !lc_slot.unclamped, c->P, c->logden[0], c->part_g));
            else
                HIPCHK(c, launch_build_sweep(c->stream, nb, gb, c->u, c->ld, c->N, d_aden(c), c->cw, c->P, c->logden[0], c->part));
        }
        if (fused) {
            HIPCHK(c, launch_reduce(c->stream, c->part_g, gb.nwaves, (int64_t)rec_g, c->scratch, c->red + off_gram));
            rc = allreduce_dev(c, c->red + off_gram, (int64_t)rec_g, 0);
            if (rc) return rc;
            HIPCHK(c, hipMemcpyAsync(c->hred + off_gram, c->red + off_gram, rec_g * sizeof(double), hipMemcpyDeviceToHost, c->stream));
            rc = sync_stream(c);
            if (rc) return rc;
            gram_row_sums(c->hred + off_gram, (int)nb, K, psum.data());
        } else {
            HIPCHK(c, launch_reduce(c->stream, c->part, gb.nwaves, Kp, c->scratch, c->red));
            rc = allreduce_dev(c, c->red, Kp, 0);
            if (rc) return rc;
            HIPCHK(c, hipMemcpyAsync(c->hred, c->red, (size_t)Kp * sizeof(double), hipMemcpyDeviceToHost, c->stream));
            rc = sync_stream(c);
            if (rc) return rc;
            for (int64_t k = 0; k < K; ++k) psum[k] = c->hred[k];
        }
        c->P_a0 = an0;
        c->P_valid = true;
        res.builds += 1;
    }
    double* gram_part = fused ? c->part_g : c->part;

    {
        std::vector<double> h(ad_off_hist(c), 0.0);
        for (int64_t k = 0; k < K; ++k) {
            h[ad_off_f(c) + k] = f[k];
            h[ad_off_psum(c) + k] = psum[k];
        }
        h[ad_off_prm(c) + 0] = gamma;
        h[ad_off_prm(c) + 1] = tol;
        h[ad_off_prm(c) + 2] = (double)std::min<int64_t>(min_sc_iter, 1 << 30);
        h[ad_off_prm(c) + 3] = check_convergence ? 1.0 : 0.0;
        h[ad_off_state(c)] = std::numeric_limits<double>::quiet_NaN();
        std::vector<int> hi((size_t)CTL_WORDS + Kp, 0);
        hi[CTL_NEEDGRAM] = fused ? 0 : 1;
        hi[CTL_GRAMSWEEPS] = 0;
        hi[CTL_SPEC] = 1;
// ... 28 lines not shown
    q.aden = d_aden(c);
    q.anum = d_anum(c);
    q.Nk = d_Nk(c);
    q.lnNk = d_lnNk(c);
    q.sampled = c->ad_ints + CTL_WORDS;
    q.m = m;
    q.K = (int)K;
    q.Kp = (int)Kp;
    q.ctl = c->ad_ints;
    q.prm = c->ad + ad_off_prm(c);
    q.state = c->ad + ad_off_state(c);
    q.hist = c->ad + ad_off_hist(c);
    q.hist_cap = c->ad_hist_cap;
    q.pmode = pmode ? 1 : 0;
    q.a0 = c->pm_vec;
    q.ccur = pmode ? c->pm_vec + Kp : nullptr;
    q.fused = fused ? 1 : 0;
    q.cgram = fused ? c->pm_vec + 2 * Kp : nullptr;
    q.light_ok = light ? 1 : 0;
    q.newton_ldlt = c->opt_newton_ldlt ? 1 : 0;
    if (const char* e = std::getenv("MBAR_NEWTON_LDLT")) q.newton_ldlt = std::atoi(e) != 0 ? 1 : 0;
    q.stamps = nullptr;
    if (std::getenv("MBAR_DEBUG_STAMPS")) {
        if (!c->stamps) HIPCHK(c, hipMalloc((void**)&c->stamps, 65 * 16 * sizeof(long long)));
        HIPCHK(c, hipMemsetAsync(c->stamps, 0, 65 * 16 * sizeof(long long), c->stream));
        q.stamps = c->stamps;
    }

    auto enqueue_gram = [&](bool timed) -> int {
        const double* lden = c->logden[0];
        LoopCtl lca = lc_slot;
        if (fused) HIPCHK(c, launch_ctl_resume(c->stream, c->ad_ints));
        if (c->weighted) {
            if (pmode)
                HIPCHK(c, launch_rinv_weighted(c->stream, c->logden[0], c->cw, c->N, c->lden_eff, lc_slot));
            else
                HIPCHK(c, launch_shift_logden(c->stream, c->logden[0], c->cw, 0.5, c->N, c->lden_eff, lc_slot));
            lden = c->lden_eff;
            lca = lc_flat;
        }
        {
            TimerPair tp{nullptr, nullptr, MBAR_TIMER_GRAM};
            if (timed) { tp.a = get_event(c); tp.b = get_event(c); }
            const bool ext = tp.a && tp.b && c->opt_timing == 2;
            if (ext) { lca.ev_start = tp.a; lca.ev_stop = tp.b; }
            if (tp.a && tp.b && !ext) (void)hipEventRecord(tp.a, c->stream);
            if (wide)
                HIPCHK(c, launch_gram_quad(c->stream, nb, gg, pmode ? c->P : c->u, c->ld, c->N, d_anum(c), lden, gram_part, lca));
            else
                HIPCHK(c, launch_gram_diag(c->stream, nb, gg, pmode ? c->P : c->u, c->ld, c->N, d_anum(c), lden, 0, gram_part,
                                           nullptr, lca));
            if (tp.a && tp.b && !ext) (void)hipEventRecord(tp.b, c->stream);
            if (tp.a && tp.b) c->pending.push_back(tp);
        }
        HIPCHK(c, launch_reduce(c->stream, gram_part, gg.nwaves, (int64_t)rec_g, c->scratch, c->red + off_gram));
        if (stream_transport(c)) {
            int r2 = allreduce_dev(c, c->red + off_gram, (int64_t)rec_g, 0);
            if (r2) return r2;
        }
        return MBAR_OK;
    };
    const bool merged = fused && !wide && c->opt_merge_select;
    bool need_newton = true;
    struct Section {
        mbar_ctx* c;
        TimerPair tp;
        Section(mbar_ctx* c_, bool on, int which) : c(c_) {
            tp.a = tp.b = nullptr;
            tp.which = which;
            if (!on) return;
            tp.a = get_event(c);
            tp.b = get_event(c);
            if (tp.a && tp.b) (void)hipEventRecord(tp.a, c->stream);
        }
        ~Section() {
            if (tp.a && tp.b) {
                (void)hipEventRecord(tp.b, c->stream);
                c->pending.push_back(tp);
            }
        }
    };
    auto enqueue_iteration = [&](bool timed) -> int {
        const bool split = timed && c->opt_timing == 3;
        if (!fused) {
            int r2 = enqueue_gram(timed);
            if (r2) return r2;
        }
        {
            Section sec(c, split && (wide || !merged || need_newton), MBAR_TIMER_NEWTON);
            if (wide)
                HIPCHK(c, launch_newton_chol(c->stream, q, c->chol));
            else if (!merged || need_newton)
                HIPCHK(c, launch_newton(c->stream, q));
        }
        need_newton = false;
        double* psum_part = c->part;
        double* obj_part = c->part + (size_t)gl.nwaves * rec_l;
        {
            TimerPair tp{nullptr, nullptr, fused ? MBAR_TIMER_FUSED : MBAR_TIMER_LSE};
            if (timed) { tp.a = get_event(c); tp.b = get_event(c); }
            const bool ext = tp.a && tp.b && c->opt_timing == 2;
            LoopCtl lcb = lc_slot;
            if (ext) { lcb.ev_start = tp.a; lcb.ev_stop = tp.b; }
            if (tp.a && tp.b && !ext) (void)hipEventRecord(tp.a, c->stream);
            if (fused) {
                HIPCHK(c, launch_fused(c->stream, nb, gl, c->P, c->ld, c->N, d_aden(c), c->cw, c->weighted ? c->cwsq : c->cw, unit,
                                       c->logden[0], gram_part, psum_part, lcb));
                if (light && !wide) {
                    LoopCtl lcl = lc_slot;
                    lcl.light_only = true;
                    HIPCHK(c, launch_psweep(c->stream, nb, 2, gp, c->P, c->ld, c->N, d_aden(c), c->cw, c->logden[0], nullptr, psum_part, lcl));
                }
            } else if (pmode)
                HIPCHK(c, launch_psweep(c->stream, nb, 2, gl, c->P, c->ld, c->N, d_aden(c), c->cw, c->logden[0], nullptr, psum_part,
                                        lcb));
            else
                HIPCHK(c, launch_lse(c->stream, nb, 2, gl, c->u, c->ld, c->N, d_aden(c), c->cw, c->logden[0], nullptr,
                                     nullptr, psum_part, obj_part, lcb));
            if (tp.a && tp.b && !ext) (void)hipEventRecord(tp.b, c->stream);
            if (tp.a && tp.b) c->pending.push_back(tp);
        }
        int64_t ar_count = (int64_t)(rec_l + 2);
        {
            Section sec(c, split, MBAR_TIMER_REDUCE);
            if (fused) {
                HIPCHK(c, launch_reduce2(c->stream, psum_part, (int64_t)rec_l, gram_part, (int64_t)rec_g, gl.nwaves, c->scratch, c->red,
                                         c->red + off_gram));
                ar_count = (int64_t)(off_gram + rec_g);
            } else if (pmode) {
                HIPCHK(c, launch_reduce(c->stream, psum_part, gl.nwaves, (int64_t)rec_l, c->scratch, c->red));
            } else {
                HIPCHK(c, launch_reduce2(c->stream, psum_part, (int64_t)rec_l, obj_part, 2, gl.nwaves, c->scratch, c->red, c->red + rec_l));
            }
        }
        if (stream_transport(c)) {
            Section sec(c, split, MBAR_TIMER_COMM);
            int r2 = allreduce_dev(c, c->red, ar_count, 0);
            if (r2) return r2;
        }
        {
            Section sec(c, split, MBAR_TIMER_NEWTON);
            if (merged)
                HIPCHK(c, launch_select_newton(c->stream, q));
            else
                HIPCHK(c, launch_select(c->stream, q));
        }
        return MBAR_OK;
    };

    const int64_t batch = c->opt_adapt_batch;
    const bool use_graph = c->opt_graph && !stream_transport(c);
    auto prepare_graph = [&]() -> int {
        const int64_t sig = ((int64_t)gg.blocks << 40) ^ ((int64_t)gl.blocks << 20) ^ ((int64_t)m << 12) ^ (pmode ? 128 : 0) ^ (fused ? 256 : 0) ^
                            (c->weighted ? 64 : 0) ^ (lc_slot.unclamped ? 512 : 0) ^ (merged ? 1024 : 0) ^ (light ? 2048 : 0) ^ (int64_t)nb;
        if (!c->ad_graph || c->ad_graph_batch != batch || c->ad_graph_sig != sig) {
            const bool need_saved = need_newton;
            need_newton = false;
            struct Restore { bool& r; bool v; ~Restore() { r = v; } } restore{need_newton, need_saved};
            if (c->ad_graph) HIPCHK(c, hipGraphExecDestroy(c->ad_graph));
            c->ad_graph = nullptr;
            int one = 1;
            HIPCHK(c, hipMemcpyAsync(c->ad_ints + CTL_DONE, &one, sizeof(int), hipMemcpyHostToDevice, c->stream));
            rc = enqueue_iteration(false);
            if (rc) return rc;
            int zero = 0;
            HIPCHK(c, hipMemcpyAsync(c->ad_ints + CTL_DONE, &zero, sizeof(int), hipMemcpyHostToDevice, c->stream));
            HIPCHK(c, hipStreamSynchronize(c->stream));
            hipGraph_t graph = nullptr;
            HIPCHK(c, hipStreamBeginCapture(c->stream, hipStreamCaptureModeThreadLocal));
            int crc = MBAR_OK;
            for (int64_t b = 0; b < batch && crc == MBAR_OK; ++b) crc = enqueue_iteration(false);
            hipError_t ee = hipStreamEndCapture(c->stream, &graph);
            if (crc) return crc;
            if (ee != hipSuccess) return fail(c, MBAR_ERR_HIP, std::string("hipStreamEndCapture: ") + hipGetErrorString(ee));
            ee = hipGraphInstantiate(&c->ad_graph, graph, nullptr, nullptr, 0);
            (void)hipGraphDestroy(graph);
            if (ee != hipSuccess) return fail(c, MBAR_ERR_HIP, std::string("hipGraphInstantiate: ") + hipGetErrorString(ee));
            c->ad_graph_batch = batch;
            c->ad_graph_sig = sig;
        }
        return MBAR_OK;
    };
    int64_t it = res.iterations;
    const int64_t it_start = it;
    bool done = false;
    int64_t nbatch = 0, ramp = batch;
    int32_t gram_sweeps = 0;
    while (it < maxiter && !done) {
        static const int64_t first_batches[3] = {6, 2, 4};
        const bool fixed_count = !check_convergence;
        const int64_t want = std::min(ramp, (nbatch < 3 && !fixed_count) ? std::min(batch, first_batches[nbatch]) : batch);
        ++nbatch;
        ramp = std::min(batch, ramp * 2);
        int64_t nbat = 0;
        for (int rep = 0; rep < (fixed_count && ramp == batch ? 4 : 1) && it + nbat < maxiter; ++rep) {
            const int64_t nb1 = std::min(want, maxiter - it - nbat);
            if (use_graph && nb1 == batch) {
                rc = prepare_graph();
                if (rc) return rc;
                if (merged && need_newton) {
                    HIPCHK(c, launch_newton(c->stream, q));
                    need_newton = false;
                }
                HIPCHK(c, hipGraphLaunch(c->ad_graph, c->stream));
            } else {
                for (int64_t b = 0; b < nb1; ++b) {
                    rc = enqueue_iteration(c->opt_timing != 0);
                    if (rc) return rc;
                }
            }
            nbat += nb1;
        }
        HIPCHK(c, hipMemcpyAsync(c->h_ctl, c->ad_ints, CTL_WORDS * sizeof(int), hipMemcpyDeviceToHost, c->stream));
        rc = sync_stream(c);
        if (rc) return rc;
        const int64_t it_new = c->h_ctl[CTL_ITER];
        if (c->h_ctl[CTL_DONE] == 1) {
            res.success = 1;
            done = true;
        } else if (c->h_ctl[CTL_DONE] == 2) {
            handed_back = true;
            done = true;
        } else if (c->h_ctl[CTL_DONE] == 3) {
            if (it_new <= it || it_new > it + nbat) return fail(c, MBAR_ERR_STATE, "device-resident adaptive loop lost count of its iterations");
            if (it_new < maxiter) {
                rc = enqueue_gram(c->opt_timing != 0);
                if (rc) return rc;
                ++gram_sweeps;
                ramp = 1;
                need_newton = true;
            }
        } else if (it_new != it + nbat) {
            return fail(c, MBAR_ERR_STATE, "device-resident adaptive loop lost count of its iterations");
        }
        it = it_new;
    }
    {
        std::vector<double> h(ad_off_hist(c));
        HIPCHK(c, hipMemcpyAsync(h.data(), c->ad, h.size() * sizeof(double), hipMemcpyDeviceToHost, c->stream));
        const int64_t row1 = history ? std::min<int64_t>(std::min<int64_t>(it, history_rows), c->ad_hist_cap) : 0;
        if (row1 > it_start)
            HIPCHK(c, hipMemcpyAsync(history + 4 * it_start, c->ad + ad_off_hist(c) + 4 * it_start, (size_t)(row1 - it_start) * 4 * sizeof(double),
                                     hipMemcpyDeviceToHost, c->stream));
        HIPCHK(c, hipStreamSynchronize(c->stream));
        for (int64_t k = 0; k < K; ++k) {
            f[k] = h[ad_off_f(c) + k];
            psum[k] = h[ad_off_psum(c) + k];
        }
        if (it > res.iterations) max_delta = h[ad_off_state(c)];
    }
    if (q.stamps) {
        std::vector<long long> st(65 * 16);
        HIPCHK(c, hipMemcpy(st.data(), c->stamps, st.size() * sizeof(long long), hipMemcpyDeviceToHost));
        for (int i = 0; i < 64; ++i) {
            const long long* p = st.data() + 16 * i;
            if (!p[0] || !p[5]) continue;
            std::fprintf(stderr, "[mbar] k_select_newton launch %d (shader clocks): select %lld, set-up %lld, elimination %lld, solution %lld, candidates %lld, total %lld; of the elimination: pivot loops %lld, exchange + trailing update %lld; of the selection: inputs %lld, Gram staged %lld, matrix-vector product %lld, sums %lld, maxima %lld\n",
                         i, p[1] - p[0], p[2] - p[1], p[3] - p[2], p[4] - p[3], p[5] - p[4], p[5] - p[0], p[6], p[7], p[8] - p[0], p[9] - p[8], p[10] - p[9],
                         p[11] - p[10], p[12] - p[11]);
        }
    }
    res.iterations = it;
    res.sci_iter = c->h_ctl[CTL_SCI];
    res.nr_iter = c->h_ctl[CTL_NR];
    res.gram_sweeps += fused ? gram_sweeps : (int32_t)(it - it_start);
    res.light_sweeps += c->h_ctl[CTL_LIGHTS];
    if (fused && !wide && unit) res.fused_unit += 1;
    if (handed_back) {
        c->P_valid = false;
        static const char* why[] = {"", "the Newton system is not positive definite", "a candidate is too far from the point the sweeps are anchored at",
                                    "a candidate is not finite"};
        const int r = c->h_ctl[CTL_REASON];
        c->error = std::string("device-resident adaptive loop handed back to the host loop: ") + why[(r >= 1 && r <= 3) ? r : 0];
    }
    return MBAR_OK;
}


}
}

extern "C" {

int mbar_solve_adaptive(mbar_ctx* c, double* f_inout, double tol, int64_t maxiter, int64_t min_sc_iter, double gamma,
                        int check_convergence, double* history, int64_t history_rows, mbar_solve_result* result) {
    if (c && c->ext_base) return fail(c, MBAR_ERR_STATE, "mbar_solve_adaptive: an extension context holds rows only (mbar_lognum_ext / mbar_gram_w_ext sweep them)");
    if (!c || !f_inout) return fail(c, MBAR_ERR_ARG, "NULL argument");
    if (!c->have_Nk) return fail(c, MBAR_ERR_STATE, "mbar_ctx_set_Nk has not been called");
    HIPCHK(c, hipSetDevice(c->device));
    const double t0 = now_ms();
    const int64_t K = c->K;
    std::vector<double> f(f_inout, f_inout + K), psum;
    mbar_solve_result res;
    std::memset(&res, 0, sizeof(res));
    struct Ld0Guard {
        mbar_ctx* c;
        ~Ld0Guard() { c->ld0_valid = false; }
    } ld0_guard{c};
    c->ld0_valid = false;
    double max_delta = std::numeric_limits<double>::quiet_NaN();
    int rc = refresh_poison(c);
    if (rc) return rc;
    bool on_device = device_loop_eligible(c) && !c->u_poison && f_is_finite(c, f.data(), 1) && maxiter > 0;
    int handbacks = 0;
    while (on_device) {
        bool handed_back = false;
        rc = adaptive_device_loop(c, f, tol, maxiter, min_sc_iter, gamma, check_convergence, history, history_rows, res, psum,
// ... 291 lines not shown
```

Before: 292.6.

## Add XCC-aware stream ladder tile assignment to fused and gram kernels

Replaces the fixed strided tile walk in the fused and gram-build kernels with a stream walk that gives each wave a contiguous block of tail tiles. An optional ladder table hands slightly different tile counts to different slots, and a runtime balancer reads each XCC's throughput from the previous launch and lets blocks claim slots based on it. The goal is to even out per-XCC finish times on MI355X. By default the ladder is off and the mode is identity, so the kernels mostly run the old schedule, with extra claim, syncthreads and 16 bytes of LDS per block.

```diff
diff --git a/include/mbar_hip.h b/include/mbar_hip.h
--- a/include/mbar_hip.h
+++ b/include/mbar_hip.h
@@ -65,6 +65,9 @@
 int mbar_ctx_set_bootstrap_layout(mbar_ctx* ctx, const int64_t* cumN, int64_t K_states, const int64_t* order);
 int mbar_bootstrap_draws(uint64_t seed, int64_t replicate, const int64_t* cumN, int64_t K_states, const int64_t* order,
                          int64_t* rints_out);
+
+int mbar_stream_table(int nb, int64_t blocks, int64_t ntiles, int ladder, int64_t* info, int64_t* first, int64_t* extra);
+int mbar_ctx_stream_stats(mbar_ctx* ctx, int reset, int64_t* out64);
 
 int mbar_ctx_weights_from_vec(mbar_ctx* ctx, double power);
 
diff --git a/pymbar_amd/_lib.py b/pymbar_amd/_lib.py
--- a/pymbar_amd/_lib.py
+++ b/pymbar_amd/_lib.py
@@ -94,6 +94,8 @@
     "mbar_ctx_draw_bootstrap_weights": (C.c_int, [_ctx, C.c_uint64, C.c_int64, _ip, C.c_int64, _ip, C.c_int64]),
     "mbar_ctx_set_bootstrap_layout": (C.c_int, [_ctx, _ip, C.c_int64, _ip]),
     "mbar_bootstrap_draws": (C.c_int, [C.c_uint64, C.c_int64, _ip, C.c_int64, _ip, _ip]),
+    "mbar_stream_table": (C.c_int, [C.c_int, C.c_int64, C.c_int64, C.c_int, _ip, _ip, _ip]),
+    "mbar_ctx_stream_stats": (C.c_int, [_ctx, C.c_int, _ip]),
     "mbar_comm_unique_id": (C.c_int, [C.c_void_p]),
     "mbar_ctx_comm_init": (C.c_int, [_ctx, C.c_void_p, C.c_int, C.c_int]),
     "mbar_ctx_set_host_allreduce": (C.c_int, [_ctx, ALLREDUCE_FN, C.c_void_p, C.c_int, C.c_int]),
diff --git a/pymbar_amd/csrc/mbar_capi.cpp b/pymbar_amd/csrc/mbar_capi.cpp
--- a/pymbar_amd/csrc/mbar_capi.cpp
+++ b/pymbar_amd/csrc/mbar_capi.cpp
@@ -672,6 +672,8 @@
     if (c->vec_tmp) (void)cache_free(c->vec_tmp);
     if (c->boot_idx) (void)cache_free(c->boot_idx);
     if (c->stamps) (void)hipFree(c->stamps);
+    if (c->stab) (void)cache_free(c->stab);
+    if (c->bal) (void)cache_free(c->bal);
     if (c->sci_graph) (void)hipGraphExecDestroy(c->sci_graph);
     if (c->stream) {
         std::lock_guard<std::mutex> lock(g_dev_mu);
@@ -739,12 +741,31 @@
         (void)drop_graphs(c);
     }
     else if (k == "wide_pmode") c->opt_wide_pmode = value;
+    else if (k == "stream_ladder" || k == "stream_assign" || k == "stream_rotate" || k == "stream_debug") {
+        if (k == "stream_ladder") c->opt_stream_ladder = value ? 1 : 0;
+        else if (k == "stream_assign") c->opt_stream_assign = value < 0 || value > 3 ? 0 : value;
+        else if (k == "stream_rotate") c->opt_stream_rot = value;
+        else c->opt_stream_debug = value ? 1 : 0;
+        (void)drop_graphs(c);
+    }
     else if (k == "quad_trim") {
         c->opt_quad_trim = value;
         c->P_valid = false;
     }
     else if (k == "adapt_batch") c->opt_adapt_batch = value < 1 ? 1 : (value > 64 ? 64 : value);
     else return fail(c, MBAR_ERR_ARG, "unknown option: " + k);
+    return MBAR_OK;
+}
+
+int mbar_ctx_stream_stats(mbar_ctx* c, int reset, int64_t* out64) {
+    if (!c || !out64) return fail(c, MBAR_ERR_ARG, "NULL argument");
+    HIPCHK(c, hipSetDevice(c->device));
+    std::fill(out64, out64 + 64, (int64_t)0);
+    if (!c->bal) return MBAR_OK;
+    int rc = sync_stream(c);
+    if (rc) return rc;
+    HIPCHK(c, hipMemcpy(out64, c->bal + STREAM_BAL_DEBUG, 64 * sizeof(int64_t), hipMemcpyDeviceToHost));
+    if (reset) HIPCHK(c, hipMemset(c->bal + STREAM_BAL_DEBUG, 0, 64 * sizeof(int64_t)));
     return MBAR_OK;
 }
 
diff --git a/pymbar_amd/csrc/mbar_ctx.h b/pymbar_amd/csrc/mbar_ctx.h
--- a/pymbar_amd/csrc/mbar_ctx.h
+++ b/pymbar_amd/csrc/mbar_ctx.h
@@ -286,11 +286,16 @@
     double* cwsq = nullptr;
     double* chol = nullptr;
     long long* stamps = nullptr;
+    int64_t* stab = nullptr;
+    int64_t stab_ntiles = -1, stab_streams = 0, stab_L0 = 0;
+    unsigned long long* bal = nullptr;
+    int64_t bal_blocks = 0;
     std::vector<double> last_psum;
     bool P_valid = false;
     std::vector<double> P_a0;
     int64_t opt_grid = 0, opt_force_generic = 0, opt_check_finite = 1, opt_sci_batch = 16, opt_timing = 0, opt_graph = 1, opt_small = 1, opt_wide = 1;
     int64_t opt_device_loop = 1, opt_adapt_batch = 8, opt_pmode = 1, opt_fused = 1, opt_quad = 1, opt_device_loop_wide = 1, opt_pcache = 1, opt_merge_select = 1, opt_sci_merged = 1, opt_wide_pmode = 1, opt_quad_trim = 1, opt_light_last = 1, opt_direct_results = 1, opt_debug_download_p = 0, opt_fused_general = 0;
+    int64_t opt_stream_ladder = 0, opt_stream_assign = 0, opt_stream_rot = 0, opt_stream_debug = 0;
     int64_t opt_small_balanced = 1, opt_sci_pingpong = 1, opt_host_pmode = 2, opt_rect_waves = 8, opt_newton_ldlt = 1;
 
     ncclComm_t comm = nullptr;
diff --git a/pymbar_amd/csrc/mbar_device.h b/pymbar_amd/csrc/mbar_device.h
--- a/pymbar_amd/csrc/mbar_device.h
+++ b/pymbar_amd/csrc/mbar_device.h
@@ -549,6 +549,96 @@
 
 static inline bool stage_offsets_wide(int64_t ld) { return (uint64_t)ld * 56u + 128u >= (1ull << 32); }
 
+#if defined(__HIPCC__)
+__device__ __forceinline__ void stream_claim(const StreamArgs& sa, int* out) {
+    const int nblk = (int)gridDim.x;
+    int slot = (int)blockIdx.x, xcc = 0, set = 0;
+    if (sa.mode == 2) slot = nblk - 1 - slot;
+    else if (sa.mode == 3) slot = (slot + sa.rot) % nblk;
+    if (sa.bal) {
+        unsigned int id;
+        asm volatile("s_getreg_b32 %0, hwreg(HW_REG_XCC_ID, 0, 4)" : "=s"(id));
+        xcc = (int)(id & 7u);
+        const unsigned long long ticket = atomicAdd(sa.bal + STREAM_BAL_TICKET, 1ull);
+        set = (int)((ticket / (unsigned long long)nblk) % 3ull);
+        const int prev = (set + 2) % 3, next = (set + 1) % 3;
+        if (ticket % (unsigned long long)nblk == 0) {
+            for (int i = 0; i < 8; ++i) sa.bal[STREAM_BAL_CNT + 8 * next + i] = 0ull;
+            for (int i = 0; i < 16; ++i) sa.bal[STREAM_BAL_HIST + 16 * next + i] = 0ull;
+        }
+        if (sa.mode == 0) {
+            const unsigned long long* h = sa.bal + STREAM_BAL_HIST + 16 * prev;
+            const unsigned long long mt = h[2 * xcc], mk = h[2 * xcc + 1];
+            bool have = true;
+            int rank = 0;
+            for (int i = 0; i < 8; ++i) {
+                const unsigned long long ot = h[2 * i], ok = h[2 * i + 1];
+                have = have && ok != 0ull && ot != 0ull;
+                const unsigned long long a = ot * mk, b = mt * ok;
+                if (i != xcc && (a > b || (a == b && i < xcc))) ++rank;
+            }
+            if (!have) rank = xcc;
+            const unsigned long long cap = (unsigned long long)(nblk / 8);
+            int got = -1;
+            for (int k = 0; k < 8 && got < 0; ++k) {
+                const int c = (rank + k) & 7;
+                const unsigned long long v = atomicAdd(sa.bal + STREAM_BAL_CNT + 8 * set + c, 1ull);
+                if (v < cap) got = c + 8 * (int)v;
+            }
+            if (got >= 0) slot = got;
+        }
+    }
+    out[0] = slot;
+    out[1] = xcc;
+    out[2] = set;
+}
+__device__ __forceinline__ void stream_report(const StreamArgs& sa, int kind, int xcc, int set, int64_t tiles, unsigned long long ticks) {
+    unsigned long long* h = sa.bal + STREAM_BAL_HIST + 16 * set + 2 * xcc;
+    __hip_atomic_fetch_add(h, (unsigned long long)tiles, __ATOMIC_RELAXED, __HIP_MEMORY_SCOPE_AGENT);
+    __hip_atomic_fetch_add(h + 1, ticks, __ATOMIC_RELAXED, __HIP_MEMORY_SCOPE_AGENT);
+    if (sa.debug) {
+        unsigned long long* d = sa.bal + STREAM_BAL_DEBUG + 32 * kind + 4 * xcc;
+        __hip_atomic_fetch_add(d, (unsigned long long)tiles, __ATOMIC_RELAXED, __HIP_MEMORY_SCOPE_AGENT);
+        __hip_atomic_fetch_add(d + 1, ticks, __ATOMIC_RELAXED, __HIP_MEMORY_SCOPE_AGENT);
+        __hip_atomic_fetch_add(d + 2, 1ull, __ATOMIC_RELAXED, __HIP_MEMORY_SCOPE_AGENT);
+        __hip_atomic_fetch_max(d + 3, ticks, __ATOMIC_RELAXED, __HIP_MEMORY_SCOPE_AGENT);
+    }
+}
+struct StreamWalk {
+    int64_t v, stride, first, ntiles;
+    int64_t p, L0, n;
+    __device__ __forceinline__ void start(const StreamArgs& sa, int64_t gw, int64_t W, int64_t nt) {
+        ntiles = nt;
+        L0 = sa.L0;
+        int64_t extra;
+        if (sa.tab) {
+            first = sa.tab[2 * gw];
+            extra = sa.tab[2 * gw + 1];
+        } else {
+            first = L0 * W + gw;
+            extra = first < nt ? 1 : 0;
+        }
+        first = (int64_t)(((uint64_t)(uint32_t)__builtin_amdgcn_readfirstlane((int)(first >> 32)) << 32) |
+                          (uint64_t)(uint32_t)__builtin_amdgcn_readfirstlane((int)first));
+        extra = __builtin_amdgcn_readfirstlane((int)extra);
+        n = L0 + extra;
+        p = 0;
+        stride = L0 > 0 ? W : 1;
+        v = L0 > 0 ? gw : first;
+        if (n <= 0) v = ntiles;
+    }
+    __device__ __forceinline__ int64_t cur() const { return v; }
+    __device__ __forceinline__ int64_t count() const { return n; }
+    __device__ __forceinline__ void next() {
+        ++p;
+        const bool sw = p == L0;
+        v = sw ? first : v + stride;
+        stride = sw ? 1 : stride;
+        v = p >= n ? ntiles : v;
+    }
+};
+#endif
+
 hipError_t launch_fused_quad(hipStream_t s, int nbt, const LaunchGeom& g, const double* P, int64_t ld, int64_t N, const double* cmul,
                              const double* cw, const double* wsq, double* rinv0, double* gp, double* pp, const LoopCtl& lc);
 
diff --git a/pymbar_amd/csrc/mbar_host.cpp b/pymbar_amd/csrc/mbar_host.cpp
--- a/pymbar_amd/csrc/mbar_host.cpp
+++ b/pymbar_amd/csrc/mbar_host.cpp
@@ -557,9 +557,54 @@
 
 
 }
+
+const int64_t STREAM_LADDER[8] = {10158, 10102, 10071, 10024, 9970, 9928, 9896, 9851};
+
+int64_t stream_table(int64_t ntiles, int64_t blocks, bool ladder, int64_t* first, int64_t* extra) {
+    const int64_t S = 4 * blocks;
+    if (ntiles < 0) ntiles = 0;
+    if (!ladder) {
+        const int64_t L0 = ntiles / S, R = ntiles - L0 * S;
+        for (int64_t s = 0; s < S; ++s) {
+            extra[s] = s < R ? 1 : 0;
+            first[s] = L0 * S + (s < R ? s : R);
+        }
+        return L0;
+    }
+    const int64_t den = STREAM_LADDER_UNIT * S;
+    const int64_t L0 = STREAM_LADDER[7] * ntiles / den, R = ntiles - L0 * S;
+    std::vector<int64_t> rem((size_t)S), order((size_t)S);
+    int64_t given = 0;
+    for (int64_t s = 0; s < S; ++s) {
+        const int64_t q = STREAM_LADDER[(s / 4) % 8] * ntiles - L0 * den;
+        extra[s] = q / den;
+        rem[(size_t)s] = q % den;
+        given += extra[s];
+        order[(size_t)s] = s;
+    }
+    std::stable_sort(order.begin(), order.end(), [&](int64_t a, int64_t b) { return rem[(size_t)a] > rem[(size_t)b]; });
+    for (int64_t i = 0; i < R - given && i < S; ++i) extra[order[(size_t)i]] += 1;
+    int64_t at = L0 * S;
+    for (int64_t s = 0; s < S; ++s) {
+        first[s] = at;
+        at += extra[s];
+    }
+    return L0;
+}
+
 }
 
 extern "C" {
+
+int mbar_stream_table(int nb, int64_t blocks, int64_t ntiles, int ladder, int64_t* info, int64_t* first, int64_t* extra) {
+    if (!info || !first || !extra || blocks < 1 || blocks > (1 << 24) || ntiles < 0 || nb < 1)
+        return fail(nullptr, MBAR_ERR_ARG, "mbar_stream_table: bad argument");
+    const bool use = ladder != 0 && stream_ladder_eligible(nb, blocks, ntiles);
+    info[0] = stream_table(ntiles, blocks, use, first, extra);
+    info[1] = use ? 1 : 0;
+    for (int r = 0; r < 8; ++r) info[2 + r] = STREAM_LADDER[r];
+    return MBAR_OK;
+}
 
 int mbar_cache_trim(void) {
     g_mem.trim();
diff --git a/pymbar_amd/csrc/mbar_internal.h b/pymbar_amd/csrc/mbar_internal.h
--- a/pymbar_amd/csrc/mbar_internal.h
+++ b/pymbar_amd/csrc/mbar_internal.h
@@ -62,7 +62,18 @@
     bool light_only = false;
 };
 
+struct StreamArgs {
+    const int64_t* tab = nullptr;
+    int64_t L0 = 0;
+    unsigned long long* bal = nullptr;
+    int mode = 1;
+    int rot = 0;
+    int debug = 0;
+};
+enum : int { STREAM_BAL_TICKET = 0, STREAM_BAL_CNT = 8, STREAM_BAL_HIST = 32, STREAM_BAL_DEBUG = 80, STREAM_BAL_WORDS = 144 };
+
 struct LaunchGeom {
+    StreamArgs streams;
     int blocks;
     int waves;
     int nwaves;
@@ -209,6 +220,12 @@
 hipError_t launch_build_sweep(hipStream_t s, int nb, const LaunchGeom& g, const double* u, int64_t ld, int64_t N,
                               const double* aden, const double* cw, double* P, double* rinv_slot, double* psum_part);
 LaunchGeom build_gram_geometry(int nb, int num_cu, int64_t ntiles, int64_t grid_override);
+inline bool stream_ladder_eligible(int nb, int64_t blocks, int64_t ntiles) {
+    return nb == 8 && blocks > 0 && blocks % 8 == 0 && ntiles / (4 * blocks) >= 64;
+}
+int64_t stream_table(int64_t ntiles, int64_t blocks, bool ladder, int64_t* first, int64_t* extra);
+extern const int64_t STREAM_LADDER[8];
+constexpr int64_t STREAM_LADDER_UNIT = 10000;
 hipError_t launch_build_gram(hipStream_t s, int nb, const LaunchGeom& g, const double* u, int64_t ld, int64_t N,
                              const double* aden, const double* wsq, bool general, double* P, double* rinv_slot, double* gram_part);
 
diff --git a/pymbar_amd/csrc/mbar_k_fused.hip b/pymbar_amd/csrc/mbar_k_fused.hip
--- a/pymbar_amd/csrc/mbar_k_fused.hip
+++ b/pymbar_amd/csrc/mbar_k_fused.hip
@@ -17,7 +17,7 @@
 k_fused(const double* __restrict__ P, int64_t ld, int64_t N, int64_t ntiles, const double* __restrict__ cmul,
         const double* __restrict__ cw, const double* __restrict__ wsq, double* __restrict__ rinv0,
         double* __restrict__ rinv1, double* __restrict__ gram_part, double* __restrict__ psum_part,
-        const int* __restrict__ ctl, int64_t slot_stride) {
+        const int* __restrict__ ctl, int64_t slot_stride, StreamArgs sa) {
     extern __shared__ __attribute__((aligned(16))) char smem[];
     if (ctl) {
         if (ctl[CTL_DONE] != 0 || ctl[CTL_LIGHT] != 0) return;
@@ -37,7 +37,12 @@
     const int nwv = blockDim.x >> 6;
     const int ks = lane & 15, ns = lane >> 4;
     char* buf = smem + wave * (2 * TILE_BYTES);
-    const int64_t gw = (int64_t)blockIdx.x * nwv + wave;
+    int* claim = reinterpret_cast<int*>(smem + nwv * (2 * TILE_BYTES) + (UNIT ? 0 : ROWS / 4 * 16 * 8));
+    if (threadIdx.x == 0) stream_claim(sa, claim);
+    __syncthreads();
+    const int slot = __builtin_amdgcn_readfirstlane(claim[0]);
+    const int xcc = __builtin_amdgcn_readfirstlane(claim[1]), hset = __builtin_amdgcn_readfirstlane(claim[2]);
+    const int64_t gw = (int64_t)slot * nwv + wave;
     const int64_t W = (int64_t)gridDim.x * nwv;
     RowIdentity rows{0};
     const StageOffsetsT<WIDE> so = make_stage_offsets<WIDE>(ld, lane);
@@ -120,14 +125,21 @@
         if constexpr (UNIT) r = n < N ? r : 0.0;
         if (n < N && fq < 2) out[n] = r;
     };
-    int64_t t = gw;
+    StreamWalk walk;
+    walk.start(sa, gw, W, ntiles);
+    int64_t t = walk.cur();
+    walk.next();
+    int64_t tn = walk.cur();
+    walk.next();
+    int64_t tnn = walk.cur();
+    const unsigned long long tick0 = sa.bal ? wall_clock64() : 0ull;
     int cur = 0;
     double rcur = 0.0;
     double uv[2][NB], w[2], sw[2];
     if (t < ntiles) {
         stage(t, buf);
-        if (t + W < ntiles) {
-            stage(t + W, buf + TILE_BYTES);
+        if (tn < ntiles) {
+            stage(tn, buf + TILE_BYTES);
             wait_vm<NDMA>();
         } else {
             wait_vm<0>();
@@ -145,10 +157,9 @@
         store_rinv(t, rcur);
         read_group(buf, 0, uv[0], w[0], sw[0]);
     }
-    for (; t < ntiles; t += W) {
+    while (t < ntiles) {
         char* cbuf = buf + cur * TILE_BYTES;
         char* nbuf = buf + (cur ^ 1) * TILE_BYTES;
-        const int64_t tn = t + W, tnn = t + 2 * W;
         const int64_t tstage = tnn < ntiles ? tnn : t;
         if constexpr (!UNIT) asm volatile("" : "+v"(cop_off));
         double sacc[4];
@@ -257,7 +268,12 @@
         rcur = recip_fast(fmax((sacc[0] + sacc[1]) + (sacc[2] + sacc[3]), 1e-300));
         store_rinv(tn, rcur);
         cur ^= 1;
-    }
+        walk.next();
+        t = tn;
+        tn = tnn;
+        tnn = walk.cur();
+    }
+    if (sa.bal && lane == 0) stream_report(sa, 0, xcc, hset, walk.count(), wall_clock64() - tick0);
     if constexpr (PINNED) asm volatile("s_nop 15\n\ts_nop 15" ::: "memory");
 #pragma unroll
     for (int f = 0; f < 2; ++f) {
@@ -305,7 +321,7 @@
     }
     const size_t tile = (size_t)nb * 16 * TS * 8 + 1024;
     const size_t lds_general = (size_t)4 * 2 * tile + (size_t)nb * 512;
-    g.lds_bytes = unit ? (size_t)4 * 2 * (tile - 1024) : lds_general;
+    g.lds_bytes = (unit ? (size_t)4 * 2 * (tile - 1024) : lds_general) + 16;
     int64_t want = (ntiles + 3) / 4;
     int64_t cap = num_cu;
     if (nb <= 5) {
@@ -336,10 +352,10 @@
         double* r1 = nullptr;
         if (lc.ev_start && lc.ev_stop)
             hipExtLaunchKernelGGL(kern, dim3(g.blocks), dim3(256), g.lds_bytes, s, lc.ev_start, lc.ev_stop, 0, P, ld, N, ntiles, cmul,
-                                  cw, wsq, rinv0, r1, gp, pp, lc.ctl, lc.slot_stride);
+                                  cw, wsq, rinv0, r1, gp, pp, lc.ctl, lc.slot_stride, g.streams);
         else
             hipLaunchKernelGGL(kern, dim3(g.blocks), dim3(256), g.lds_bytes, s, P, ld, N, ntiles, cmul, cw, wsq, rinv0, r1, gp, pp,
-                               lc.ctl, lc.slot_stride);
+                               lc.ctl, lc.slot_stride, g.streams);
         return hipGetLastError();
     };
     if (unit) return stage_offsets_wide(ld) ? go(k_fused<NB, true, true>) : go(k_fused<NB, false, true>);
diff --git a/pymbar_amd/csrc/mbar_k_pmode.hip b/pymbar_amd/csrc/mbar_k_pmode.hip
--- a/pymbar_amd/csrc/mbar_k_pmode.hip
+++ b/pymbar_amd/csrc/mbar_k_pmode.hip
@@ -163,7 +163,8 @@
 template <int NB, bool WIDE, bool GENERAL>
 __global__ void __launch_bounds__(256, 1)
 k_build_gram(const double* __restrict__ u, int64_t ld, int64_t N, int64_t ntiles, const double* __restrict__ aden,
-             const double* __restrict__ wsq, double* __restrict__ P, double* __restrict__ rinv_slot, double* __restrict__ gram_part) {
+             const double* __restrict__ wsq, double* __restrict__ P, double* __restrict__ rinv_slot, double* __restrict__ gram_part,
+             StreamArgs sa) {
     extern __shared__ __attribute__((aligned(16))) char smem[];
     constexpr int ROWS = NB * 16;
     constexpr int NDMA = ROWS / 8;
@@ -175,10 +176,14 @@
     const int wave = __builtin_amdgcn_readfirstlane(threadIdx.x >> 6);
     const int nwv = blockDim.x >> 6;
     const int ks = lane & 15, ns = lane >> 4;
+    int* claim = reinterpret_cast<int*>(smem + EXP_TABLE_BYTES + nwv * (2 * TILE_BYTES));
+    if (threadIdx.x == 0) stream_claim(sa, claim);
     exp_table_init(smem);
     __syncthreads();
     char* buf = smem + EXP_TABLE_BYTES + wave * (2 * TILE_BYTES);
-    const int64_t gw = (int64_t)blockIdx.x * nwv + wave;
+    const int slot = __builtin_amdgcn_readfirstlane(claim[0]);
+    const int xcc = __builtin_amdgcn_readfirstlane(claim[1]), hset = __builtin_amdgcn_readfirstlane(claim[2]);
+    const int64_t gw = (int64_t)slot * nwv + wave;
     const int64_t W = (int64_t)gridDim.x * nwv;
     RowIdentity rows{0};
     const StageOffsetsT<WIDE> so = make_stage_offsets<WIDE>(ld, lane);
@@ -206,15 +211,20 @@
         stage_tile<ROWS, true, 0, 1>(u, ld, tile * TS, dst, lane, so, rows);
         stage_vec16<true>(wsq, tile * TS, dst + U_BYTES, lane);
     };
-    int64_t t = gw;
+    StreamWalk walk;
+    walk.start(sa, gw, W, ntiles);
+    int64_t t = walk.cur();
+    const unsigned long long tick0 = sa.bal ? wall_clock64() : 0ull;
     int cur = 0;
+    bool later = false;
     if (t < ntiles) stage(t, buf);
-    for (; t < ntiles; t += W) {
+    while (t < ntiles) {
         char* cbuf = buf + cur * TILE_BYTES;
-        const int64_t tn = t + W;
+        walk.next();
+        const int64_t tn = walk.cur();
         if (tn < ntiles) {
             stage(tn, buf + (cur ^ 1) * TILE_BYTES);
-            if (t != gw)
+            if (later)
                 wait_vm<2 * (NDMA + 1)>();
             else
                 wait_vm<NDMA + 1>();
@@ -314,7 +324,10 @@
             if (lane < TS && n < N) rinv_slot[n] = 1.0;
         }
         cur ^= 1;
-    }
+        later = true;
+        t = tn;
+    }
+    if (sa.bal && lane == 0) stream_report(sa, 1, xcc, hset, walk.count(), wall_clock64() - tick0);
     if constexpr (PINNED) asm volatile("s_nop 15\n\ts_nop 15" ::: "memory");
 #pragma unroll
     for (int b = 0; b < NBLK; ++b)
@@ -543,7 +556,7 @@
 
 LaunchGeom build_gram_geometry(int nb, int num_cu, int64_t ntiles, int64_t grid_override) {
     LaunchGeom g = fused_geometry(nb, num_cu, ntiles, grid_override);
-    g.lds_bytes = (size_t)4 * 2 * ((size_t)nb * 16 * TS * 8 + TS * 8) + EXP_TABLE_BYTES;
+    g.lds_bytes = (size_t)4 * 2 * ((size_t)nb * 16 * TS * 8 + TS * 8) + EXP_TABLE_BYTES + 16;
     return g;
 }
 template <int NB>
@@ -556,7 +569,7 @@
             if (e != hipSuccess) return e;
         }
         const int64_t ntiles = (N + TS - 1) / TS;
-        hipLaunchKernelGGL(kern, dim3(g.blocks), dim3(256), g.lds_bytes, s, u, ld, N, ntiles, aden, wsq, P, rinv_slot, gp);
+        hipLaunchKernelGGL(kern, dim3(g.blocks), dim3(256), g.lds_bytes, s, u, ld, N, ntiles, aden, wsq, P, rinv_slot, gp, g.streams);
         return hipGetLastError();
     };
     if (general) return stage_offsets_wide(ld) ? go(k_build_gram<NB, true, true>) : go(k_build_gram<NB, false, true>);
diff --git a/pymbar_amd/csrc/mbar_loops.cpp b/pymbar_amd/csrc/mbar_loops.cpp
--- a/pymbar_amd/csrc/mbar_loops.cpp
+++ b/pymbar_amd/csrc/mbar_loops.cpp
@@ -361,8 +361,59 @@
         if (rcl) return rcl;
         light = light && l_ok;
     }
-    const LaunchGeom gb = fused ? build_gram_geometry(nb, c->num_cu, ntiles, c->opt_grid)
-                                : build_sweep_geometry(nb, c->num_cu, ntiles, c->opt_grid);
+    LaunchGeom gb = fused ? build_gram_geometry(nb, c->num_cu, ntiles, c->opt_grid)
+                          : build_sweep_geometry(nb, c->num_cu, ntiles, c->opt_grid);
+    bool ladder = false;
+    if (!arc && fused && !wide) {
+        const bool shape_ok = gb.blocks == gl.blocks && stream_ladder_eligible(nb, gl.blocks, ntiles);
+        ladder = shape_ok && c->opt_stream_ladder != 0;
+        StreamArgs sa;
+        sa.L0 = ntiles / ((int64_t)4 * gl.blocks);
+        sa.mode = (int)c->opt_stream_assign;
+        if (sa.mode < 0 || sa.mode > 3 || (sa.mode == 0 && !ladder)) sa.mode = 1;
+        sa.rot = (int)(((c->opt_stream_rot % gl.blocks) + gl.blocks) % gl.blocks);
+        if (ladder) {
+            const int64_t S = (int64_t)4 * gl.blocks;
+            if (!c->stab || c->stab_ntiles != ntiles || c->stab_streams != S) {
+                arc = drop_graphs(c);
+                if (!arc && c->stab && c->stab_streams != S) {
+                    HIPCHK(c, cache_free(c->stab));
+                    c->stab = nullptr;
+                }
+                if (!arc && !c->stab && cache_malloc((void**)&c->stab, (size_t)2 * S * sizeof(int64_t)) != hipSuccess)
+                    arc = fail(c, MBAR_ERR_HIP, "allocation of the stream table failed");
+                if (!arc) {
+                    std::vector<int64_t> first((size_t)S), extra((size_t)S), tab((size_t)2 * S);
+                    c->stab_L0 = stream_table(ntiles, gl.blocks, true, first.data(), extra.data());
+                    for (int64_t i = 0; i < S; ++i) {
+                        tab[(size_t)2 * i] = first[(size_t)i];
+                        tab[(size_t)2 * i + 1] = extra[(size_t)i];
+                    }
+                    HIPCHK(c, hipMemcpyAsync(c->stab, tab.data(), tab.size() * sizeof(int64_t), hipMemcpyHostToDevice, c->stream));
+                    HIPCHK(c, hipStreamSynchronize(c->stream));
+                    c->stab_ntiles = ntiles;
+                    c->stab_streams = S;
+                }
+            }
+            sa.tab = c->stab;
+            sa.L0 = c->stab_L0;
+        }
+        if (!arc && shape_ok && (ladder || c->opt_stream_debug != 0)) {
+            if (!c->bal) {
+                arc = drop_graphs(c);
+                if (!arc && cache_malloc((void**)&c->bal, (size_t)STREAM_BAL_WORDS * sizeof(unsigned long long)) != hipSuccess)
+                    arc = fail(c, MBAR_ERR_HIP, "allocation of the stream counters failed");
+                c->bal_blocks = 0;
+            }
+            if (!arc && c->bal_blocks != gl.blocks) {
+                HIPCHK(c, hipMemsetAsync(c->bal, 0, (size_t)STREAM_BAL_WORDS * sizeof(unsigned long long), c->stream));
+                c->bal_blocks = gl.blocks;
+            }
+            sa.bal = c->bal;
+            sa.debug = c->opt_stream_debug != 0 ? 1 : 0;
+        }
+        if (!arc) gl.streams = gb.streams = sa;
+    }
     const size_t rec_g = (size_t)nb * (nb + 1) / 2 * 256;
     const size_t rec_l = (size_t)2 * Kp;
     const size_t off_gram = rec_l + 2;
@@ -697,7 +748,7 @@
     const bool use_graph = c->opt_graph && !stream_transport(c);
     auto prepare_graph = [&]() -> int {
         const int64_t sig = ((int64_t)gg.blocks << 40) ^ ((int64_t)gl.blocks << 20) ^ ((int64_t)m << 12) ^ (pmode ? 128 : 0) ^ (fused ? 256 : 0) ^
-                            (c->weighted ? 64 : 0) ^ (lc_slot.unclamped ? 512 : 0) ^ (merged ? 1024 : 0) ^ (light ? 2048 : 0) ^ (int64_t)nb;
+                            (c->weighted ? 64 : 0) ^ (lc_slot.unclamped ? 512 : 0) ^ (merged ? 1024 : 0) ^ (light ? 2048 : 0) ^ (ladder ? 4096 : 0) ^ (int64_t)nb;
         if (!c->ad_graph || c->ad_graph_batch != batch || c->ad_graph_sig != sig) {
             const bool need_saved = need_newton;
             need_newton = false;
```

Result: slower. 287.9 (-1.6%).
